# feixue94/sfd2

Measured on AMD Instinct MI355X. Metric: images/sec extract+match (1600x1200, n4096), higher is better.
Workload: dtype f16c

## Files before the change

sfd2_amd/_lib.py:

```python
import ctypes
import os

import numpy as np

_HERE = os.path.dirname(os.path.abspath(__file__))
LIB_PATH = os.path.join(_HERE, "libsfd2hip.so")


def use_library(path):
    global LIB_PATH, _lib
    if _lib is not None:
        raise RuntimeError("use_library() must be called before the library is first loaded")
    LIB_PATH = os.path.abspath(path)

FLAG_ASYNC = 1
FLAG_NO_STABILITY = 2
FLAG_IMG_NORMALISED = 4
FLAG_IMG_U8_HWC = 8
FLAG_IMG_BGR = 16
FLAG_IMG_U8_X = 32
FLAG_MATCH_OUT16 = 64
FLAG_DESC_STORE64 = 128
MATCH_HLOC, MATCH_ITLOC_NNM, MATCH_ITLOC_NNR = 0, 1, 2
DT_F32, DT_F64, DT_F16 = 0, 1, 2
# ... 197 lines not shown
                           "There is no CPU fallback.")
    lib = ctypes.CDLL(LIB_PATH)
    vp, ci, cf, i64 = ctypes.c_void_p, ctypes.c_int, ctypes.c_float, ctypes.c_int64
    pi = ctypes.POINTER(ctypes.c_int)
    lib.sfd2_version.restype = ci
    lib.sfd2_last_error.restype = ctypes.c_char_p
    lib.sfd2_ctx_create.argtypes = [ci, ctypes.POINTER(vp)]
    lib.sfd2_ctx_destroy.argtypes = [vp]
    lib.sfd2_ctx_destroy.restype = None
    lib.sfd2_get_stream.argtypes = [vp]
    lib.sfd2_get_stream.restype = vp
    lib.sfd2_load_weights.argtypes = [vp, ctypes.POINTER(Sfd2Tensor), ci]
    lib.sfd2_det.argtypes = [vp, vp, ci, ci, ci, ci, vp, vp, vp, ci, pi, pi, pi, pi]
    lib.sfd2_extract.argtypes = [vp, vp, ci, ci, ci, cf, ci, ci, vp, vp, vp, ci, i64, pi]
    lib.sfd2_extract_count.argtypes = [vp, pi]
    lib.sfd2_extract_multiscale.argtypes = [vp, vp, ci, ci, ci, vp, ci, cf, ci, ci, vp, vp, vp, ci, i64, pi]
    lib.sfd2_extract_spp.argtypes = [vp, vp, ci, ci, ci, cf, ci, vp, vp, vp, i64, pi, vp, vp]
    lib.sfd2_nms_fast.argtypes = [vp, vp, ci, ci, cf, ci, vp]
    lib.sfd2_extract_spp_levels.argtypes = [vp, vp, ci, ci, ci, ci, vp, vp, vp, cf, ci, vp, vp, vp, i64, vp]
    lib.sfd2_simple_nms.argtypes = [vp, vp, ci, ci, ci, vp]
    lib.sfd2_select_keypoints.argtypes = [vp, vp, ci, ci, cf, ci, ci, ci, vp, vp, i64, pi]
    lib.sfd2_sample_descriptors.argtypes = [vp, vp, ci, ci, ci, ci, vp, ci, vp]
    lib.sfd2_heatmap.argtypes = [vp, vp, ci, ci, vp, ci, ci, ci, ci, vp]
    lib.sfd2_debug_activation.argtypes = [vp, ctypes.c_char_p, vp, i64, pi, pi, pi]
    lib.sfd2_match.argtypes = [vp, vp, ci, vp, ci, ci, ci, ci, ci, ctypes.POINTER(MatchConf), vp, vp, ci]
    lib.sfd2_match_segments.argtypes = [vp, vp, ci, vp, ci, ci, ci, ci, ci, ci, vp, vp, ctypes.POINTER(MatchConf), vp, vp, ci]
    lib.sfd2_match_batch.argtypes = [vp, ctypes.POINTER(DescSet), ctypes.POINTER(DescSet), ci, ci,
                                     ctypes.POINTER(MatchConf), vp, vp, ci, ci]
    lib.sfd2_get_timings.argtypes = [vp, ctypes.POINTER(Timings)]
    lib.sfd2_sync.argtypes = [vp]
    lib.sfd2_set_precision.argtypes = [vp, ci]
    lib.sfd2_set_option.argtypes = [vp, ctypes.c_char_p, ci]
    lib.sfd2_get_option.argtypes = [vp, ctypes.c_char_p, pi]
    lib.sfd2_device_pci_bus_id.argtypes = [ci, ctypes.c_char_p, ci, pi]
    lib.sfd2_preprocess.argtypes = [vp, vp, ci, ci, ci, ci, ci, ci, vp]
    lib.sfd2_extract_match.argtypes = [vp, vp, ci, ci, cf, ci, ci, vp, vp, vp, ctypes.POINTER(DescSet), ci, ci,
                                       ctypes.POINTER(MatchConf), vp, vp]
    lib.sfd2_set_profiling.argtypes = [vp, ci]
    lib.sfd2_set_profile_filter.argtypes = [vp, ctypes.c_char_p]
    lib.sfd2_get_layer_timings.argtypes = [vp, ctypes.POINTER(LayerTiming), ci, pi]
    lib.sfd2_get_range_status.argtypes = [vp, ctypes.POINTER(RangeStatus), ci]
    lib.sfd2_range_tensor_name.argtypes = [ci]
    lib.sfd2_range_tensor_name.restype = ctypes.c_char_p
    lib.sfd2_calibrate_range.argtypes = [vp, vp, ci, ci, ci, ci]
    lib.sfd2_get_act_exponents.argtypes = [vp, vp, vp, ci, pi]
    lib.sfd2_get_margin_status.argtypes = [vp, vp, pi, ctypes.POINTER(ctypes.c_float)]
    lib.sfd2_get_relax_status.restype = ci
    lib.sfd2_get_relax_status.argtypes = [vp, ctypes.POINTER(ctypes.c_float), pi]
    lib.sfd2_set_act_exponents.argtypes = [vp, vp, ci]
    lib.sfd2_extract_record_async.argtypes = [vp, vp, ci]
    lib.sfd2_desc_pack.argtypes = [vp, ctypes.POINTER(DescSet), ci, vp, ci]
    lib.sfd2_jpeg_parse.argtypes = [vp, i64, ctypes.POINTER(JpegInfo)]
    lib.sfd2_jpeg_prepare.argtypes = [vp, i64, ctypes.POINTER(JpegInfo)]
    lib.sfd2_jpeg_decode.argtypes = [vp, vp, i64, ctypes.POINTER(JpegInfo), ci, vp, i64, vp, ci]
    lib.sfd2_absolute_pose_batch.argtypes = [vp, ctypes.POINTER(PoseProblem), ci, ctypes.POINTER(PoseConf), ctypes.POINTER(PoseResult), vp, ci]
    lib.sfd2_pose_refine_batch.argtypes = [vp, ctypes.POINTER(PoseProblem), ci, vp, vp, ctypes.POINTER(PoseResult), ci]
    lib.sfd2_relative_pose_batch.argtypes = [vp, ctypes.POINTER(TwoViewProblem), ci, ctypes.POINTER(TwoViewConf), ctypes.POINTER(TwoViewResult), vp, vp, ci]
    lib.sfd2_assemble_2d3d.argtypes = [vp, ctypes.POINTER(PointTable), ctypes.POINTER(AssembleJob), ci, ci, ci]
    cd = ctypes.c_double
    lib.sfd2_verify_matches_batch.argtypes = [vp, ctypes.POINTER(TriView), ci, vp, vp, vp, vp, ci, vp, cd, ci, vp, vp, ci]
    lib.sfd2_build_tracks.argtypes = [vp, i64, vp, i64, ci, vp, vp, vp, ctypes.POINTER(i64), ctypes.POINTER(i64), vp, ci]
    lib.sfd2_triangulate_tracks.argtypes = [vp, ctypes.POINTER(TriView), ci, vp, vp, ci, vp, vp, ctypes.POINTER(TriConf), vp, vp, vp, vp, vp, ci]
    lib.sfd2_pairs_retrieval.argtypes = [vp, vp, ci, vp, ci, ci, ci, ci, vp, vp, ci]
    lib.sfd2_pairs_covisibility.argtypes = [vp, vp, vp, ci, vp, vp, ci, ci, vp, vp, vp, ci]
    lib.sfd2_pairs_poses.argtypes = [vp, vp, vp, ci, ci, cd, vp, vp, vp, ci]
    lib.sfd2_covis_clusters.argtypes = [vp, vp, vp, ci, vp, vp, ci, vp, vp, ci, vp, vp, ci]
    lib.sfd2_covis_frames.argtypes = [vp, ctypes.POINTER(FramesMap), ctypes.POINTER(FramesTask), ci, vp, vp, ci, vp, vp, vp, ci]
    lib.sfd2_vlad_assign.argtypes = [vp, vp, i64, vp, ci, ci, vp, vp, ci]
    lib.sfd2_vlad_aggregate.argtypes = [vp, vp, vp, ci, vp, ci, ci, ci, vp, vp, ci]
    lib.sfd2_vlad_kmeans.argtypes = [vp, vp, i64, ci, ci, ci, vp, vp, vp, pi, ci]
    lib.sfd2_bundle_adjust.argtypes = [vp, ctypes.POINTER(TriView), ci, vp, vp, ci, vp, vp, vp, vp, ctypes.POINTER(BaConf), ctypes.POINTER(BaResult), vp, ci]
    lib.sfd2_mapper_restrict.argtypes = [vp, vp, ci, vp, vp, vp, ci, vp, vp, vp, vp, vp, ctypes.POINTER(i64), ctypes.POINTER(i64), ci]
    lib.sfd2_mapper_filter.argtypes = [vp, ctypes.POINTER(TriView), ci, vp, ci, vp, vp, vp, cd, cd, vp, vp, vp, vp, ci]
    lib.sfd2_mapper_visible.argtypes = [vp, vp, ci, vp, vp, ci, vp, vp, ci, vp, ci]
    lib.sfd2_mapper_assemble.argtypes = [vp, vp, ci, vp, vp, ci, vp, vp, vp, ci, vp, ci, i64, vp, vp, vp, vp, vp, ci]
    for name in EXPORTS:
        getattr(lib, name)
    if lib.sfd2_version() < 119:
        raise RuntimeError(f"{LIB_PATH} is version {lib.sfd2_version()}, this binding needs >= 119 (rebuild: __graft_entry__.build())")
    _lib = lib
    return lib


def check(rc):
    if rc != 0:
        raise RuntimeError("libsfd2hip: " + load().sfd2_last_error().decode("utf-8", "replace"))


def ptr(a):
    if a is None:
        return None
    if isinstance(a, int):
        return a
    if isinstance(a, np.ndarray):
        return a.ctypes.data
    return a.data_ptr()


class Context:

    def __init__(self, device=0):
        self.lib = load()
        h = ctypes.c_void_p()
        check(self.lib.sfd2_ctx_create(int(device), ctypes.byref(h)))
        self.h = h
        self.device = int(device)
        self.options = {}

    def close(self):
        if getattr(self, "h", None):
            self.lib.sfd2_ctx_destroy(self.h)
            self.h = None

    def __del__(self):
        try:
            self.close()
        except Exception:
            pass

    @property
    def stream(self):
        return self.lib.sfd2_get_stream(self.h)

    def load_weights(self, sd):
        keep, arr = [], (Sfd2Tensor * len(sd))()
        n = 0
        for name, v in sd.items():
            a = v.detach().cpu().numpy() if hasattr(v, "detach") else np.asarray(v)
            if a.dtype.kind != "f":
                continue
            a = np.ascontiguousarray(a, dtype=np.float32)
            if a.ndim > 4:
                continue
            keep.append(a)
            arr[n].name = name.encode()
            arr[n].data = a.ctypes.data
            arr[n].ndim = a.ndim
            for i, s in enumerate(a.shape):
                arr[n].shape[i] = s
            n += 1
        check(self.lib.sfd2_load_weights(self.h, arr, n))

    def timings(self):
        t = Timings()
        check(self.lib.sfd2_get_timings(self.h, ctypes.byref(t)))
        return {"ms_total": t.ms_total, "ms_backbone": t.ms_backbone, "ms_post": t.ms_post,
                "ms_match": t.ms_match, "n_candidates": t.n_candidates}

    def set_precision(self, mode):
        check(self.lib.sfd2_set_precision(self.h, {'f16': 0, 'f32': 1, 'f16x3': 2, 'f16c': 3, 'f16x3d': 2}[mode]))
        check(self.lib.sfd2_set_option(self.h, b"x3_desc16", 1 if mode == 'f16x3d' else 0))

    def set_option(self, key, value):
        check(self.lib.sfd2_set_option(self.h, key.encode(), int(value)))
        self.options.pop(key, None)
        self.options[key] = int(value)

    def get_option(self, key):
        v = ctypes.c_int(0)
        check(self.lib.sfd2_get_option(self.h, key.encode(), ctypes.byref(v)))
        return int(v.value)

    def sync(self):
        check(self.lib.sfd2_sync(self.h))

    def set_profiling(self, max_steps, kernel_filter=None):
# ... 70 lines not shown
```

sfd2_amd/build.py:

```python
import os
import subprocess

HERE = os.path.dirname(os.path.abspath(__file__))
CSRC = os.path.join(HERE, "csrc")
LIB = os.path.join(HERE, "libsfd2hip.so")
SOURCES = ["conv_kernels.hip", "conv2_kernels.hip", "conv3_kernels.hip", "conv3rf_kernels.hip", "conv2b_s2d_kernel.hip", "conv1x1_kernels.hip", "resblock_kernel.hip", "conv_f32_kernels.hip", "convc_kernels.hip", "rb23_c_kernel.hip", "sparse_da3_kernel.hip", "sparse_da0_kernel.hip", "fused_stem_kernel.hip", "fused_stem_c_kernel.hip", "post_kernels.hip", "util_kernels.hip", "nms4_kernels.hip", "match_kernels.hip", "match_mutual_kernel.hip", "api_core.hip", "api_weights.hip", "api_network.hip", "api_extract.hip", "api_match.hip", "api_graph.hip", "jpeg_parse.hip", "jpeg_kernels.hip", "api_jpeg.hip", "pose_kernels.hip", "api_pose.hip", "two_view_kernels.hip", "api_two_view.hip", "assemble_kernels.hip", "api_assemble.hip", "tri_kernels.hip", "api_triangulate.hip", "pairs_kernels.hip", "api_pairs.hip", "cluster_kernels.hip", "api_cluster.hip", "frames_kernels.hip", "api_frames.hip", "vlad_kernels.hip", "api_vlad.hip", "bundle_kernels.hip", "api_bundle.hip", "mapper_kernels.hip", "api_mapper.hip"]
_NN = ["-fno-honor-nans"]
SRC_FLAGS = {"match_mutual_kernel.hip": _NN, "conv3_kernels.hip": _NN, "conv3rf_kernels.hip": _NN, "resblock_kernel.hip": _NN, "conv2_kernels.hip": _NN,
             "fused_stem_kernel.hip": _NN, "conv_kernels.hip": _NN, "conv1x1_kernels.hip": _NN, "nms4_kernels.hip": _NN, "convc_kernels.hip": _NN, "fused_stem_c_kernel.hip": _NN, "rb23_c_kernel.hip": _NN, "sparse_da3_kernel.hip": _NN, "sparse_da0_kernel.hip": _NN, "conv2b_s2d_kernel.hip": _NN}
FLAGS = ["--offload-arch=gfx950", "-O3", "-std=c++17", "-fPIC", "-Wall", "-Wno-unused-function"] + \
    os.environ.get("SFD2_EXTRA_FLAGS", "").split()


def _newer(a, b):
    return (not os.path.exists(b)) or os.path.getmtime(a) > os.path.getmtime(b)


def _hipcc():
    return os.environ.get("HIPCC", "/opt/rocm/bin/hipcc")


def have_hipcc():
    return os.path.isfile(_hipcc()) and os.access(_hipcc(), os.X_OK)


def needs_build():
    if not os.path.exists(LIB):
        return True
    srcs = [os.path.join(CSRC, s) for s in SOURCES] + [os.path.join(CSRC, "sfd2_internal.h"), os.path.join(CSRC, "sfd2_ctx.h"), os.path.join(CSRC, "api_scratch.h"), os.path.join(CSRC, "pose_camera.h"), os.path.join(CSRC, "five_point.h"), os.path.join(CSRC, "bundle.h"), os.path.join(CSRC, "mapper.h"),
                                                      os.path.join(HERE, "..", "include", "sfd2_hip.h")]
    return any(os.path.exists(s) and os.path.getmtime(s) > os.path.getmtime(LIB) for s in srcs)


def build_lib(force=False, verbose=False, out=None, extra_flags=()):
    hipcc = _hipcc()
    objs = []
    deps = [os.path.join(CSRC, "sfd2_internal.h"), os.path.join(CSRC, "sfd2_ctx.h"), os.path.join(CSRC, "api_scratch.h"), os.path.join(CSRC, "pose_camera.h"), os.path.join(CSRC, "five_point.h"), os.path.join(CSRC, "bundle.h"), os.path.join(CSRC, "mapper.h"), os.path.join(HERE, "..", "include", "sfd2_hip.h")]
    procs = []
    lib = out or LIB
    odir = CSRC
    if out:
        odir = os.path.join(os.path.dirname(os.path.abspath(out)), "obj_" + os.path.basename(out).replace(".", "_"))
        os.makedirs(odir, exist_ok=True)
    for src in SOURCES:
        s = os.path.join(CSRC, src)
        o = os.path.join(odir, src.replace(".hip", ".o"))
        objs.append(o)
        if force or _newer(s, o) or any(_newer(d, o) for d in deps):
            cmd = [hipcc] + FLAGS + SRC_FLAGS.get(src, []) + list(extra_flags) + ["-c", s, "-o", o]
            if verbose:
                print(" ".join(cmd))
            procs.append((cmd, subprocess.Popen(cmd)))
    for cmd, p in procs:
        if p.wait() != 0:
            raise RuntimeError("hipcc failed: " + " ".join(cmd))
    if force or procs or not os.path.exists(lib) or any(_newer(o, lib) for o in objs):
        tmp = lib + ".tmp.%d" % os.getpid()
        cmd = [hipcc, "--offload-arch=gfx950", "-shared", "-fPIC", "-o", tmp] + objs
        if verbose:
            print(" ".join(cmd))
        subprocess.check_call(cmd)
        os.replace(tmp, lib)
    return lib


if __name__ == "__main__":
    print(build_lib(verbose=True))
```

sfd2_amd/csrc/api_core.hip:

```cpp
#include "sfd2_ctx.h"

static thread_local std::string g_err;
int sfd2_fail(const std::string &m)
{
    g_err = m;
    return -1;
}

std::atomic<unsigned long long> g_alloc_gen{0};

thread_local int g_sfd2_cu_limit = 0;

extern "C" int sfd2_version(void) { return 119; }
extern "C" const char *sfd2_last_error(void) { return g_err.c_str(); }

extern "C" int sfd2_ctx_create(int device, sfd2_ctx **out)
{
    if (!out) return fail("sfd2_ctx_create: out is null");
    int ndev = 0;
    hipError_t e = hipGetDeviceCount(&ndev);
    if (e != hipSuccess || ndev <= 0) return fail("sfd2_ctx_create: no HIP device available (libsfd2hip has no CPU fallback)");
    if (device < 0 || device >= ndev) return fail("sfd2_ctx_create: bad device index");
    HIPCHECK(hipSetDevice(device));
    sfd2_ctx *c = new sfd2_ctx();
// ... 18 lines not shown
    c->extract_rec.p = c->range_hist_dev.as<unsigned int>() + SFD2_RS_COUNT;
    static_assert(SFD2_RS_COUNT == SFD2_RANGE_TENSORS && AE_COUNT == SFD2_RANGE_GROUPS, "include/sfd2_hip.h and the internal tables agree");

    *out = c;
    return 0;
}

extern "C" int sfd2_device_pci_bus_id(int device, char *out, int len, int *n_devices)
{
    int ndev = 0;
    hipError_t e = hipGetDeviceCount(&ndev);
    if (e != hipSuccess || ndev <= 0) return fail("sfd2_device_pci_bus_id: no HIP device available");
    if (n_devices) *n_devices = ndev;
    if (device < 0 || device >= ndev) return fail("sfd2_device_pci_bus_id: bad device index");
    if (!out || len < 13) return fail("sfd2_device_pci_bus_id: buffer of at least 13 bytes needed");
    HIPCHECK(hipDeviceGetPCIBusId(out, len, device));
    return 0;
}

extern "C" void sfd2_ctx_destroy(sfd2_ctx *c)
{
    if (!c) return;
    (void)hipSetDevice(c->device);
    (void)hipStreamSynchronize(c->stream);
    graphs_release(c);
    for (int i = 0; i < 4; ++i) if (c->ev[i]) (void)hipEventDestroy(c->ev[i]);
    if (c->ev_jobs) (void)hipEventDestroy(c->ev_jobs);
    for (int i = 0; i < SFD2_IMG_SLOTS; ++i) {
        if (c->ev_copied[i]) (void)hipEventDestroy(c->ev_copied[i]);
        if (c->ev_img_free[i]) (void)hipEventDestroy(c->ev_img_free[i]);
    }
    if (c->copy_stream) (void)hipStreamDestroy(c->copy_stream);
    if (c->side_stream) (void)hipStreamDestroy(c->side_stream);
    if (c->ev_fork) (void)hipEventDestroy(c->ev_fork);
    if (c->ev_join) (void)hipEventDestroy(c->ev_join);
    for (hipEvent_t e : c->prof_ev) (void)hipEventDestroy(e);
    if (c->pin_jobs) (void)hipHostFree(c->pin_jobs);
    if (c->stream) (void)hipStreamDestroy(c->stream);
    delete c;
}

extern "C" void *sfd2_get_stream(sfd2_ctx *c) { return c ? (void *)c->stream : nullptr; }

extern "C" int sfd2_set_precision(sfd2_ctx *c, int mode)
{
    if (!c) return fail("sfd2_set_precision: null ctx");
    if (mode != SFD2_PREC_F16 && mode != SFD2_PREC_F32 && mode != SFD2_PREC_F16X3 && mode != SFD2_PREC_F16C)
        return fail("sfd2_set_precision: unknown mode");
    HIPCHECK(hipSetDevice(c->device));
    HIPCHECK(hipStreamSynchronize(c->stream));
    if (mode != c->precision) graphs_release(c);
    c->precision = mode;
    return sfd2_margin_selfcheck_if_pending(c);
}

extern "C" int sfd2_set_option(sfd2_ctx *c, const char *key, int value)
{
    if (!c || !key) return fail("sfd2_set_option: null argument");
    HIPCHECK(hipSetDevice(c->device));
    HIPCHECK(hipStreamSynchronize(c->stream));
    const std::string k(key);
    graphs_release(c);
    if (k == "fuse") c->fuse = value ? 1 : 0;
    else if (k == "fuse_det") c->fuse_det = value ? 1 : 0;
    else if (k == "alias") c->opt_alias = value ? 1 : 0;
    else if (k == "graphs") c->use_graphs = value ? 1 : 0;
    else if (k == "branches") c->opt_branches = value ? 1 : 0;
    else if (k == "sta_side") c->opt_sta_side = value ? 1 : 0;
    else if (k == "fuse_post") c->opt_fuse_post = value ? 1 : 0;
    else if (k == "sparse_desc") c->opt_sparse_desc = value ? 1 : 0;
    else if (k == "sparse_da3") c->opt_sparse_da3 = value ? 1 : 0;
    else if (k == "sparse_da0") c->opt_sparse_da0 = value < 0 ? 0 : (value > 2 ? 2 : value);
    else if (k == "cu_limit") c->opt_cu_limit = value < 0 ? 0 : value;
    else if (k == "auto_range") c->opt_auto_range = value ? 1 : 0;
    else if (k == "range_fallback") c->opt_range_fallback = value ? 1 : 0;
    else if (k == "x3_pp") c->opt_x3_pp = value ? 1 : 0;
    else if (k == "x3_desc16") c->opt_x3_desc16 = value ? 1 : 0;
    else if (k == "auto_margin") c->opt_auto_margin = value ? 1 : 0;
    else if (k == "fp6_filters") c->opt_fp6_filters = value ? 1 : 0;
    else if (k == "fp6_acts") c->opt_fp6_acts = value ? 1 : 0;
    else if (k == "s2d") c->opt_s2d = value ? 1 : 0;
    else if (k == "trunk_r1") c->opt_trunk_r1 = value ? 1 : 0;
    else if (k == "fuse_pb") c->opt_fuse_pb = value ? 1 : 0;
    else if (k == "generic_c") c->opt_generic_c = value ? 1 : 0;
    else if (k == "comp_rb") c->opt_comp_rb = value ? 1 : 0;
    else if (k == "no_rf_c") c->opt_no_rf_c = value ? 1 : 0;
    else if (k == "comp_heads") { c->opt_comp_heads = c->user_comp_heads = value ? 1 : 0; c->user_set_comp_heads = true; }
    else if (k == "c3b_plain") { c->user_c3b_plain = value < 0 ? -1 : (value ? 1 : 0); c->opt_c3b_plain = value > 0 ? 1 : 0; }
    else if (k == "comp_det") c->opt_comp_det = value ? 1 : 0;
    else if (k == "fuse_rb23") c->opt_fuse_rb23 = value ? 1 : 0;
    else if (k == "rb_inner") { c->opt_rb_inner = c->user_rb_inner = value < 0 ? 0 : (value > 2 ? 2 : value); c->user_set_rb_inner = true; }
    else return fail("sfd2_set_option: unknown key '" + k + "'");
    return 0;
}

extern "C" int sfd2_get_option(sfd2_ctx *c, const char *key, int *value)
{
    if (!c || !key || !value) return fail("sfd2_get_option: null argument");
    const std::string k(key);
    const struct { const char *name; int v; } tab[] = {
        {"fuse", c->fuse}, {"fuse_det", c->fuse_det}, {"alias", c->opt_alias}, {"graphs", c->use_graphs}, {"branches", c->opt_branches}, {"sta_side", c->opt_sta_side},
        {"fuse_post", c->opt_fuse_post}, {"sparse_desc", c->opt_sparse_desc}, {"sparse_da3", c->opt_sparse_da3}, {"sparse_da0", c->opt_sparse_da0}, {"cu_limit", c->opt_cu_limit},
        {"auto_range", c->opt_auto_range}, {"range_fallback", c->opt_range_fallback}, {"x3_pp", c->opt_x3_pp}, {"x3_desc16", c->opt_x3_desc16},
        {"auto_margin", c->opt_auto_margin}, {"fp6_filters", c->opt_fp6_filters}, {"fp6_acts", c->opt_fp6_acts}, {"s2d", c->opt_s2d},
        {"trunk_r1", c->opt_trunk_r1}, {"fuse_pb", c->opt_fuse_pb}, {"generic_c", c->opt_generic_c}, {"comp_rb", c->opt_comp_rb},
        {"no_rf_c", c->opt_no_rf_c}, {"comp_heads", c->opt_comp_heads}, {"c3b_plain", c->opt_c3b_plain}, {"comp_det", c->opt_comp_det},
        {"fuse_rb23", c->opt_fuse_rb23}, {"rb_inner", c->opt_rb_inner},
    };
    for (const auto &e : tab)
        if (k == e.name) { *value = e.v; return 0; }
    return fail("sfd2_get_option: unknown key '" + k + "'");
}

extern "C" int sfd2_sync(sfd2_ctx *c)
{
    if (!c) return fail("sfd2_sync: null ctx");
    HIPCHECK(hipSetDevice(c->device));
    HIPCHECK(hipStreamSynchronize(c->stream));
    return 0;
}

extern "C" int sfd2_set_profiling(sfd2_ctx *c, int max_steps)
{
    if (!c) return fail("sfd2_set_profiling: null ctx");
    HIPCHECK(hipSetDevice(c->device));
    HIPCHECK(hipStreamSynchronize(c->stream));
    if (max_steps < 0 || max_steps > 4096) return fail("sfd2_set_profiling: max_steps out of range");
    const size_t need = (size_t)max_steps * PROF_SLOTS * 2;
    while (c->prof_ev.size() < need) {
        hipEvent_t e;
        HIPCHECK(hipEventCreate(&e));
        c->prof_ev.push_back(e);
    }
    c->prof_max_steps = max_steps;
    c->prof_step = 0;
    c->prof_slot = 0;
    c->prof_used.assign(max_steps, 0);
    c->prof_row.assign((size_t)max_steps * PROF_SLOTS, 0);
    c->prof_tab.clear();
    return 0;
}

extern "C" int sfd2_set_profile_filter(sfd2_ctx *c, const char *substr)
{
    if (!c) return fail("sfd2_set_profile_filter: null ctx");
    c->prof_filter = substr ? substr : "";
    return 0;
}

extern "C" int sfd2_get_layer_timings(sfd2_ctx *c, sfd2_layer_timing *out, int cap, int *n)
{
    if (!c || !n) return fail("sfd2_get_layer_timings: null argument");
    HIPCHECK(hipSetDevice(c->device));
    HIPCHECK(hipStreamSynchronize(c->stream));
    for (int st = 0; st < c->prof_step; ++st)
        for (int sl = 0; sl < c->prof_used[st]; ++sl) {
            float ms = 0.0f;
            const size_t e = ((size_t)st * PROF_SLOTS + sl) * 2;
            const int row = c->prof_row[(size_t)st * PROF_SLOTS + sl];
            if (hipEventElapsedTime(&ms, c->prof_ev[e], c->prof_ev[e + 1]) == hipSuccess) {
                c->prof_tab[row].ms_total += ms;
                c->prof_tab[row].launches += 1;
            }
        }
    c->prof_step = 0;
    *n = (int)c->prof_tab.size();
    if (out)
        for (int i = 0; i < *n && i < cap; ++i) out[i] = c->prof_tab[i];
    return 0;
}

extern "C" int sfd2_get_timings(sfd2_ctx *c, sfd2_timings *out)
{
    if (!c || !out) return fail("sfd2_get_timings: null argument");
    *out = c->tim;
    return 0;
}

extern "C" const char *sfd2_range_tensor_name(int i) { return (i >= 0 && i < SFD2_RS_COUNT) ? kTensor[i].range : ""; }

static int fetch_range_words(sfd2_ctx *c, unsigned int *raw , bool clear)
{
    const size_t bytes = (size_t)SFD2_RS_COUNT * (SFD2_RANGE_SUB + 1) * sizeof(unsigned int);
    HIPCHECK(hipMemcpyAsync(raw, c->range_stat.p, bytes, hipMemcpyDeviceToHost, c->stream));
    if (clear) HIPCHECK(hipMemsetAsync(c->range_stat.p, 0, bytes, c->stream));
    HIPCHECK(hipStreamSynchronize(c->stream));
    return 0;
}
// ... 85 lines not shown
```

sfd2_amd/csrc/api_extract.hip:

```cpp
#include "sfd2_ctx.h"

static int release_image_slot(sfd2_ctx *c);
static int stage_image(sfd2_ctx *c, const void *x, int on_device, int H, int W, const float **dev, int u8 = 0)
{
    if (u8 == 2) {
        const float *raw = nullptr;
        if (on_device) raw = static_cast<const float *>(x);
        else if (stage_image(c, x, 0, H, W, &raw, 3)) return -1;
        HIPCHECK(c->img_u8_packed.ensure((size_t)3 * H * W + 16));
        launch_unpack_rgbx(c->stream, reinterpret_cast<const unsigned char *>(raw), c->img_u8_packed.as<unsigned char>(), (size_t)H * W);
        if (release_image_slot(c)) return -1;
        *dev = c->img_u8_packed.as<float>();
        return 0;
    }
    if (on_device) { *dev = static_cast<const float *>(x); return 0; }
    const size_t bytes = u8 == 3 ? (size_t)4 * H * W : (size_t)3 * H * W * (u8 ? 1 : sizeof(float));
    const int slot = c->img_slot = (c->img_slot + 1) % SFD2_IMG_SLOTS;
    HIPCHECK(c->img2[slot].ensure(bytes));
    HIPCHECK(hipStreamWaitEvent(c->copy_stream, c->ev_img_free[slot], 0));
    HIPCHECK(hipMemcpyAsync(c->img2[slot].p, x, bytes, hipMemcpyHostToDevice, c->copy_stream));
    HIPCHECK(hipEventRecord(c->ev_copied[slot], c->copy_stream));
    HIPCHECK(hipStreamWaitEvent(c->stream, c->ev_copied[slot], 0));
    c->img_slot_used = slot;
    *dev = c->img2[slot].as<float>();
// ... 65 lines not shown
                         int top_k, float *nms_dense, float *kpts_dev = nullptr, float *scores_dev = nullptr,
                         int Hb = 0, int Wb = 0)
{
    if (Hb <= 0) Hb = H;
    if (Wb <= 0) Wb = W;
    if (radius < 0 || radius > 4) return fail("nms radius must be in [0,4] (reference uses 4)");
    if (!(conf_th >= 0.0f)) return fail("conf_th must be >= 0 and not NaN (got " + std::to_string(conf_th) + ")");
    const int sel_cap = top_k > 0 ? std::min(top_k, c->cand_cap) : c->cand_cap;
    c->last_sel_cap = sel_cap;
    HIPCHECK(c->sel.ensure((size_t)sel_cap * 8));
    HIPCHECK(c->sorted.ensure((size_t)sel_cap * 8));
    HIPCHECK(c->kpts.ensure((size_t)sel_cap * 2 * sizeof(float)));
    HIPCHECK(c->kscores.ensure((size_t)sel_cap * sizeof(float)));
    if (!c->counters_clean) HIPCHECK(hipMemsetAsync(c->counters.p, 0, SFD2_COUNTER_BYTES, c->stream));
    c->counters_clean = false;
    bool threshold_done = false;
    {
        ProfScope ps(c, "nms_select", "nms_select_kernel", 0.0, (double)H * W * 4);
        threshold_done = launch_nms_select(c->stream, heat_dev, H, W, radius, conf_th, border, Hb, Wb, nms_dense,
                                           c->cand.as<unsigned long long>(), c->cand_cap, c->counters.as<unsigned int>(), 1, top_k);
    }
    {
        ProfScope ps(c, "topk_sort", "hist_select+compact+rank_sort", 0.0, (double)sel_cap * 24);
        c->kpts_cur = kpts_dev ? kpts_dev : c->kpts.as<float>();
        c->kscores_cur = scores_dev ? scores_dev : c->kscores.as<float>();
        launch_topk_sort(c->stream, threshold_done, c->cand.as<unsigned long long>(), c->cand_cap, top_k,
                         c->sel.as<unsigned long long>(), c->sorted.as<unsigned long long>(), sel_cap,
                         c->counters.as<unsigned int>(), c->bnd.as<unsigned long long>(), W, c->kpts_cur, c->kscores_cur);
    }
    HIPCHECK(hipGetLastError());
    return 0;
}

static int read_counts(sfd2_ctx *c, int64_t cap_out, int *n_out)
{
    unsigned int cnt[4] = {0, 0, 0, 0};
    HIPCHECK(hipMemcpyAsync(cnt, c->counters.p, sizeof(cnt), hipMemcpyDeviceToHost, c->stream));
    HIPCHECK(hipStreamSynchronize(c->stream));
    c->tim.n_candidates = cnt[0];
    if (cnt[0] > (unsigned int)c->cand_cap)
        return fail("candidate buffer overflow: " + std::to_string(cnt[0]) + " NMS survivors > capacity " +
                    std::to_string(c->cand_cap));
    int64_t n = cnt[1];
    if (n > c->last_sel_cap) n = c->last_sel_cap;
    if (cap_out >= 0 && n > cap_out) n = cap_out;
    if (n_out) *n_out = (int)n;
    return 0;
}

extern "C" int sfd2_extract(sfd2_ctx *c, const void *img, int img_on_device, int H, int W, float conf_th, int top_k,
                            int flags, float *kpts_xy, float *scores, float *desc, int out_on_device, int64_t cap_out,
                            int *n_out)
{
    if (!c || !img) return fail("sfd2_extract: null argument");
    if (!c->weights_loaded) return fail("sfd2_extract: weights not loaded");
    if (!(flags & SFD2_FLAG_NO_STABILITY) && !c->has_sta)
        return fail("sfd2_extract: the loaded state_dict has no ConvSta; pass SFD2_FLAG_NO_STABILITY (use_stability=False)");
    HIPCHECK(hipSetDevice(c->device));
    if (extract_begin(c, flags)) return -1;
    const PassPlan plan = plan_pass(c, PASS_EXTRACT, H, W, top_k, desc != nullptr);
    if (ensure_workspace(c, plan, H, W)) return -1;
    const float *img_dev = nullptr;
    const int u8 = (flags & SFD2_FLAG_IMG_U8_HWC) ? 1 : 0;
    if (u8 && (flags & SFD2_FLAG_IMG_NORMALISED)) return fail("sfd2_extract: a uint8 image cannot be pre-normalised");
    if ((flags & SFD2_FLAG_IMG_BGR) && !u8) return fail("sfd2_extract: SFD2_FLAG_IMG_BGR needs SFD2_FLAG_IMG_U8_HWC");
    if ((flags & SFD2_FLAG_IMG_U8_X) && !u8) return fail("sfd2_extract: SFD2_FLAG_IMG_U8_X needs SFD2_FLAG_IMG_U8_HWC");
    if (stage_image(c, img, img_on_device, H, W, &img_dev, u8 ? ((flags & SFD2_FLAG_IMG_U8_X) ? 2 : 1) : 0)) return -1;
    HIPCHECK(hipEventRecord(c->ev[0], c->stream));
    prof_step_begin(c);
    const int in_mode = ((flags & SFD2_FLAG_IMG_NORMALISED) ? 0 : 1) | (u8 ? 2 : 0) | ((flags & SFD2_FLAG_IMG_BGR) ? 4 : 0);
    if (run_network(c, plan, img_dev, in_mode)) return -1;
    if (release_image_slot(c)) return -1;
    HIPCHECK(hipEventRecord(c->ev[1], c->stream));
    const int HS = 8 * c->H8, WS = 8 * c->W8;
    if (plan.skip_pb) {
        ProfScope ps(c, "convPb+heads+heatmap", "pb_heads_heat_kernel", 2.0 * c->H8 * c->W8 * 65 * 256,
                     (double)c->H8 * c->W8 * 512 + (double)H * W * 4);
        launch_pb_heads_heat(c->stream, act_view(c, plan, T_PA).as<half_t>(), c->H8, c->W8, c->pb.w.as<half_t>(), c->pb.cout_pad, c->pb.scale.as<float>(),
                             c->pb.shift.as<float>(), (flags & SFD2_FLAG_NO_STABILITY) ? nullptr : c->sta.as<float>(), c->H4, c->W4,
                             H, W, c->heat.as<float>(), c->counters.as<unsigned int>(), SFD2_COUNTER_BYTES / 4);
        c->counters_clean = pb_heads_heat_clears(c->H8, c->W8, SFD2_COUNTER_BYTES / 4);
    } else if (plan.skip_head) {
        ProfScope ps(c, "heads+heatmap", "heads_heat_kernel", 0.0, (double)c->H8 * c->W8 * 65 * 4 + (double)H * W * 4);
        launch_heads_heat(c->stream, c->logits.as<float>(), 128, c->H8, c->W8,
                          (flags & SFD2_FLAG_NO_STABILITY) ? nullptr : c->sta.as<float>(), c->H4, c->W4, H, W, c->heat.as<float>());
    } else {
        ProfScope ps(c, "heatmap", "heatmap_kernel", 0.0, (double)H * W * 8);
        launch_heatmap(c->stream, c->score.as<float>(), HS, WS,
                       (flags & SFD2_FLAG_NO_STABILITY) ? nullptr : c->sta.as<float>(), c->H4, c->W4, H, W,
                       c->heat.as<float>(), nullptr);
    }
    const int sel_guess = top_k > 0 ? std::min(top_k, c->cand_cap) : c->cand_cap;
    const bool direct = out_on_device && kpts_xy && scores && cap_out >= sel_guess;
    if (run_selection(c, c->heat.as<float>(), H, W, conf_th, 4, 4, top_k, nullptr, direct ? kpts_xy : nullptr,
                      direct ? scores : nullptr)) return -1;
    const int sel_cap = c->last_sel_cap;
    int64_t ncopy = sel_cap;
    if (cap_out >= 0 && ncopy > cap_out) ncopy = cap_out;
    const bool store64 = desc && (flags & SFD2_FLAG_DESC_STORE64);
    if (store64 && cap_out < 1) return fail("sfd2_extract: SFD2_FLAG_DESC_STORE64 needs cap_out >= 1 (desc is double [128][cap_out])");
    float *desc_dst = nullptr;
    if (desc) {
        if (out_on_device && cap_out >= sel_cap && !store64) {
            desc_dst = desc;
        } else {
            HIPCHECK(c->kdesc.ensure((size_t)sel_cap * 128 * sizeof(float)));
            desc_dst = c->kdesc.as<float>();
        }
        if (plan.sparse_x3 && !plan.desc16) {
            const size_t nin = (size_t)c->H4 * c->W4 * 256;
            const int rows32 = (sel_cap * 4 + 31) / 32;
            HIPCHECK(c->da3_sparse.ensure((size_t)rows32 * 32 * 256 * sizeof(float)));
            HIPCHECK(c->db_sparse.ensure((size_t)rows32 * 32 * 128 * sizeof(float)));
            const ConvW &L3 = c->fda3;
            {
                ProfScope ps(c, "convDa.3", "sparse_da3_kernel<x3>", 2.0 * 4 * sel_cap * 256.0 * 256.0 * 9, (double)sel_cap * (16 * 1024 + 4 * 1024));
                launch_sparse_da3_x3(c->stream, c->x3_da0_planes.as<half_t>(), c->x3_da0_planes.as<half_t>() + nin, c->H4, c->W4, H, W,
                                     L3.wx3p.as<half_t>(), L3.wsl.as<half_t>(), L3.cout_pad, L3.scale.as<float>(), L3.shift.as<float>(), 0, c->kpts_cur,
                                     c->counters.as<unsigned int>() + 1, sel_cap, c->da3_sparse.as<float>(), c->zero_page.as<half_t>());
            }
            if (convf_at(c, StrictConv{}, "convDb", c->fdb, c->da3_sparse, rows32, 32, c->db_sparse, rows32, 32, 0)) return -1;
            ProfScope ps(c, "sample_desc", "sample_desc_kernel", 0.0, (double)sel_cap * 128 * 4 * 5);
            launch_sample_desc(c->stream, c->db_sparse.as<float>(), c->H4, c->W4, H, W, c->kpts_cur, c->counters.as<unsigned int>() + 1,
                               sel_cap, desc_dst, 1);
        } else if (plan.sparse_da3 || (plan.sparse_x3 && plan.desc16)) {
            HIPCHECK(c->da3_sparse.ensure((size_t)sel_cap * 4 * 256 * sizeof(half_t)));
            if (plan.sparse_da0) {
                const ConvW &L0 = c->da0;
                ProfScope ps(c, "convDa.0", "sparse_da0_kernel", 2.0 * 16 * sel_cap * (double)L0.cout * L0.cin * 9,
                             (double)sel_cap * (36 * 512 + 16 * 512) + 2.0 * L0.cout_pad * L0.cin * 9);
                launch_sparse_da0(c->stream, c->da0_in.as<half_t>(), c->H4, c->W4, H, W, L0.w.as<half_t>(), L0.scale.as<float>(), L0.shift.as<float>(), 1,
                                  c->kpts_cur, c->counters.as<unsigned int>() + 1, sel_cap, act_view(c, plan, T_DA0).as<half_t>());
            }
            {
                ProfScope ps(c, "convDa.3", "sparse_da3_kernel", 2.0 * 4 * sel_cap * 256.0 * 256.0 * 9, (double)sel_cap * (16 * 512 + 4 * 512) + 2.0 * 256 * 256 * 9);
                launch_sparse_da3(c->stream, act_view(c, plan, T_DA0).as<half_t>(), c->H4, c->W4, H, W, c->da3.w.as<half_t>(), c->da3.wsl.as<half_t>(), c->da3.cout_pad, c->da3.scale.as<float>(),
                                  c->da3.shift.as<float>(), 0, c->kpts_cur, c->counters.as<unsigned int>() + 1, sel_cap,
                                  c->da3_sparse.as<half_t>(), c->zero_page.as<half_t>());
            }
            ProfScope ps(c, "desc_head", "desc_head_kernel", 2.0 * 4 * sel_cap * 128 * 256, (double)sel_cap * (4 * 512 + 512));
            launch_desc_head(c->stream, c->da3_sparse.as<half_t>(), c->H4, c->W4, H, W, c->db.w.as<half_t>(), c->db.cout_pad, c->db.scale.as<float>(),
                             c->db.shift.as<float>(), c->kpts_cur, c->counters.as<unsigned int>() + 1, sel_cap, desc_dst, 1);
        } else if (plan.sparse_desc) {
            ProfScope ps(c, "desc_head", "desc_head_kernel", 2.0 * 4 * sel_cap * 128 * 256, (double)sel_cap * (4 * 512 + 512));
            launch_desc_head(c->stream, act_view(c, plan, T_DA).as<half_t>(), c->H4, c->W4, H, W, c->db.w.as<half_t>(), c->db.cout_pad, c->db.scale.as<float>(),
                             c->db.shift.as<float>(), c->kpts_cur, c->counters.as<unsigned int>() + 1, sel_cap, desc_dst);
        } else {
            ProfScope ps(c, "sample_desc", "sample_desc_kernel", 0.0, (double)sel_cap * 128 * 4 * 5);
            launch_sample_desc(c->stream, c->draw.as<float>(), c->H4, c->W4, H, W, c->kpts_cur,
                               c->counters.as<unsigned int>() + 1, sel_cap, desc_dst);
        }
    }
    size_t desc_bytes_fixed = 0;
    if (store64) {
        float *d64_dst = out_on_device ? desc : nullptr;
        if (!out_on_device) {
            HIPCHECK(c->kdesc64.ensure((size_t)128 * cap_out * sizeof(double)));
            d64_dst = c->kdesc64.as<float>();
        }
        ProfScope ps(c, "desc_store64", "desc_store64_kernel", 0.0, (double)sel_cap * 128 * 4 + (double)cap_out * 128 * 8);
        launch_desc_store64(c->stream, desc_dst, c->counters.as<unsigned int>() + 1, sel_cap, reinterpret_cast<double *>(d64_dst), (int)cap_out);
        desc_dst = d64_dst;
        desc_bytes_fixed = (size_t)128 * cap_out * sizeof(double);
    }
    prof_step_end(c);
    HIPCHECK(hipEventRecord(c->ev[2], c->stream));
    HIPCHECK(hipGetLastError());
    if (flags & SFD2_FLAG_ASYNC) {
        if (!direct && copy_out(c, kpts_xy, c->kpts.p, (size_t)ncopy * 2 * sizeof(float), out_on_device)) return -1;
        if (!direct && copy_out(c, scores, c->kscores.p, (size_t)ncopy * sizeof(float), out_on_device)) return -1;
        if (desc && desc_dst != desc && copy_out(c, desc, desc_dst, desc_bytes_fixed ? desc_bytes_fixed : (size_t)ncopy * 128 * sizeof(float), out_on_device)) return -1;
        if (n_out) *n_out = -1;
        return 0;
    }
    int n = 0;
    if (read_counts(c, cap_out, &n)) return -1;
    {
        const int fb = range_wants_fallback(c);
        if (fb < 0) return -1;
        if (fb) {
            FallbackScope scope(c);
            return sfd2_extract(c, img, img_on_device, H, W, conf_th, top_k, flags, kpts_xy, scores, desc, out_on_device, cap_out, n_out);
        }
    }
    if (!direct && copy_out(c, kpts_xy, c->kpts.p, (size_t)n * 2 * sizeof(float), out_on_device)) return -1;
    if (!direct && copy_out(c, scores, c->kscores.p, (size_t)n * sizeof(float), out_on_device)) return -1;
    if (desc && desc_dst != desc && copy_out(c, desc, desc_dst, desc_bytes_fixed ? desc_bytes_fixed : (size_t)n * 128 * sizeof(float), out_on_device)) return -1;
    HIPCHECK(hipStreamSynchronize(c->stream));
    float ms = 0.0f;
    if (hipEventElapsedTime(&ms, c->ev[0], c->ev[2]) == hipSuccess) c->tim.ms_total = ms;
    if (hipEventElapsedTime(&ms, c->ev[0], c->ev[1]) == hipSuccess) c->tim.ms_backbone = ms;
    if (hipEventElapsedTime(&ms, c->ev[1], c->ev[2]) == hipSuccess) c->tim.ms_post = ms;
    if (n_out) *n_out = n;
    return 0;
}

extern "C" int sfd2_preprocess(sfd2_ctx *c, const unsigned char *img_hwc, int on_device, int H, int W, int flags, int new_h,
                               int new_w, float *out_chw_dev)
{
    if (!c || !img_hwc || !out_chw_dev) return fail("sfd2_preprocess: null argument");
    if (H < 1 || W < 1 || new_h < 1 || new_w < 1) return fail("sfd2_preprocess: bad size");
    HIPCHECK(hipSetDevice(c->device));
    const float *staged = nullptr;
    if (stage_image(c, img_hwc, on_device, H, W, &staged, (flags & SFD2_FLAG_IMG_U8_X) ? 2 : 1)) return -1;
    launch_ingest_u8(c->stream, reinterpret_cast<const unsigned char *>(staged), H, W, (flags & SFD2_FLAG_IMG_BGR) ? 1 : 0, new_h,
                     new_w, out_chw_dev);
    if (release_image_slot(c)) return -1;
    HIPCHECK(hipGetLastError());
    if (!(flags & SFD2_FLAG_ASYNC)) HIPCHECK(hipStreamSynchronize(c->stream));
    return 0;
}

extern "C" int sfd2_extract_multiscale(sfd2_ctx *c, const void *img, int img_on_device, int H, int W, const double *scales,
                                       int n_scales, float conf_th, int top_k, int flags, float *kpts_xy, float *scores,
                                       float *desc, int out_on_device, int64_t cap_out, int *n_out)
{
    if (!c || !img || !scales) return fail("sfd2_extract_multiscale: null argument");
    if (n_scales < 1 || n_scales > 8) return fail("sfd2_extract_multiscale: 1..8 scales");
    if (!c->weights_loaded) return fail("sfd2_extract_multiscale: weights not loaded");
    if (!(flags & SFD2_FLAG_NO_STABILITY) && !c->has_sta)
        return fail("sfd2_extract_multiscale: the loaded state_dict has no ConvSta; pass SFD2_FLAG_NO_STABILITY");
    if (flags & SFD2_FLAG_ASYNC) return fail("sfd2_extract_multiscale: SFD2_FLAG_ASYNC is not supported");
    if (flags & SFD2_FLAG_DESC_STORE64) return fail("sfd2_extract_multiscale: SFD2_FLAG_DESC_STORE64 is not supported (single-scale sfd2_extract only)");
    if (!kpts_xy || !scores) return fail("sfd2_extract_multiscale: kpts_xy and scores are required");
    HIPCHECK(hipSetDevice(c->device));
// ... 384 lines not shown
```

sfd2_amd/csrc/api_network.hip:

```cpp
#include "sfd2_ctx.h"

static int down2(int n) { return (n - 1) / 2 + 1; }

static X3Kind x3_fast_kind(const PassPlan &p, const ConvW &L, bool has_res, int Ho, int Wo)
{
    if (!p.x3_pp || has_res || L.ks != 3 || L.cin % 64 != 0) return XK_GENERIC;
    if ((L.cout_pad == 256 || (L.cout_pad == 128 && L.stride == 2)) && conv3x3_rf_serves(3, L.stride, L.cout_pad, L.cin, Ho, Wo)) return XK_RF;
    return (L.stride == 1 && L.cout_pad % 128 == 0) ? XK_PP : XK_GENERIC;
}
static const int sl_level[] = {0 , 1, 1 , 2, 2, 2, 2, 2, 2, 2, 2, 2 , 3, 3 , 2, 2, 2};
static_assert(sizeof(sl_level) == SL_COUNT * sizeof(int), "one level per StrictLayer");
static bool on_planes(const StrictConv &s) { return s.kind == XK_PP || s.kind == XK_RF || s.kind == XK_S2D; }

#define SFD2_DA0_FRAC 0.6
PassPlan plan_pass(const sfd2_ctx *c, PassEntry entry, int H, int W, int top_k, bool desc)
{
    PassPlan p;
    const int H2 = down2(H), W2 = down2(W), H4 = down2(H2), W4 = down2(W2);
    const bool det = entry == PASS_DET, x3 = c->precision == SFD2_PREC_F16X3;
    p.f32 = x3 || c->precision == SFD2_PREC_F32;
    p.comp = c->precision == SFD2_PREC_F16C;
    p.fuse = !p.f32 && (det ? c->fuse_det : c->fuse);
    p.alias = p.fuse && !det && c->opt_alias;
    p.generic_c = p.comp && c->opt_generic_c;
    p.no_rf_c = c->opt_no_rf_c;
    p.fp6_filters = c->opt_fp6_filters;
    p.fused_stem = p.fuse && !p.generic_c;
    p.comp_rb = p.comp && c->opt_comp_rb;
    bool wrm = true, wk = true;
    for (int b = 0; b < 3; ++b) {
        wrm = wrm && c->rb1[b].wrm.p && c->rb3[b].wrm.p;
        wk = wk && c->rb1[b].wfl.p && c->rb3[b].wfl.p && c->rb2[b].wlk.p;
    }
    const char *frb = sfd2_env("SFD2_FUSED_RB");
    p.rb_fused = p.fuse && !p.comp_rb && !(frb && frb[0] == '0') && wrm;
    p.rb_inner = (p.comp_rb && !p.generic_c && wk) ? c->opt_rb_inner : 0;
    p.rb23 = p.rb_inner >= 2 && c->opt_fuse_rb23;
    if (p.comp) {
        const bool a6 = c->opt_fp6_acts && !p.generic_c && c->c2a.wc66.p && c->c3a.wc66.p && c->c3b.wc66.p;
        const bool s6 = a6 && p.fuse && c->w1b_stem_c6.p;
        const bool b6 = a6 && !p.no_rf_c && conv3x3_rf_c_serves(3, 2, c->c2b.cout_pad, c->c2b.cin, H4, W4);
        p.a2a_s2d = c->opt_s2d && p.alias && s6 && !p.no_rf_c && conv2b_s2d_serves(H2, W2, c->c2b.cin, c->c2b.cout_pad) && H4 * 2 == H2 && W4 * 2 == W2;
        static const bool c3a_plain_out = sfd2_env("SFD2_C3A_KEEP_CORR") == nullptr;
        const bool p3b = c->opt_c3b_plain && a6 && b6 && !p.generic_c;
        const bool p3a = p3b && c3a_plain_out;
        const bool tr1 = c->opt_trunk_r1 && a6 && p.rb23 && c->rb1[0].wfr.p && c->rb3[0].wf8l.p;
        p.ch = p.comp_rb && c->opt_comp_heads;
        p.chp = p.ch || (p.comp_rb && c->opt_comp_det);
        p.rec[T_CONV1A] = Rec::Unit8;
        p.rec[T_CONV1B] = s6 ? Rec::Half6 : Rec::Unit8;
        p.rec[T_CONV2A] = Rec::Unit8;
        p.rec[T_CONV2B] = b6 ? Rec::Half6 : Rec::Unit8;
        p.rec[T_CONV3A] = p3a ? Rec::None : a6 ? Rec::Half6 : Rec::Unit8;
        p.a3a_in = p3b ? Rec::None : p.rec[T_CONV3A];
        p.rec[T_CONV3B] = tr1 ? Rec::Resid8 : Rec::Unit8;
        for (int b = 0; b < 3 && p.comp_rb; ++b) {
            p.rec[T_T1_0 + b] = p.rb_inner >= 2 ? Rec::None : Rec::Unit8;
            p.rec[T_T2_0 + b] = p.rb_inner >= 1 ? Rec::None : Rec::Unit8;
            p.rec[T_OUT_0 + b] = (tr1 && (b < 2 || !p.chp)) ? Rec::Resid8 : Rec::Unit8;
        }
        p.rec[T_PA0] = p.chp ? Rec::Unit8 : Rec::None;
        p.rec[T_DA0] = p.ch ? Rec::Unit8 : Rec::None;
    }
    p.branches = c->opt_branches;
    if (entry == PASS_EXTRACT) {
        p.skip_head = c->opt_fuse_post && H % 8 == 0 && W % 8 == 0;
        p.skip_pb = p.skip_head && c->opt_fuse_pb && p.fuse && !p.branches && c->pb.cout_pad >= 96;
        const bool few = desc && top_k > 0 && (size_t)16 * top_k <= (size_t)H4 * W4;
        p.sparse_desc = c->opt_sparse_desc && p.fuse && few;
        p.sparse_da3 = p.sparse_desc && c->opt_sparse_da3 && !p.ch && !p.branches;
        p.sparse_x3 = x3 && c->opt_sparse_desc && c->opt_sparse_da3 && c->opt_x3_pp && few;
        p.sparse_da0 = p.sparse_da3 && c->opt_sparse_da0 && c->da0.w.p && c->da0.ks == 3 && c->da0.stride == 1 &&
                       sparse_da0_serves(c->da0.cin, c->da0.cout_pad, H4, W4) &&
                       (c->opt_sparse_da0 >= 2 || (double)16 * top_k <= SFD2_DA0_FRAC * (double)H4 * W4);
        p.skip_db = p.sparse_desc;
        p.skip_da3 = p.sparse_da3 || p.sparse_x3;
    }
    p.sta_early = p.alias && p.skip_pb;
    p.sta_side = c->has_sta && p.sta_early && c->opt_sta_side && !p.branches;
    if (p.alias) {
        static const int slots[T_COUNT] = {-1 , 0, 1 , 0, 1, 2, 0, 2, 0 , 1, 1, 1 ,
                                           0, 2, 0 , 1, 2 , 1 , 1 };
        for (int id = 0; id < T_COUNT; ++id) p.at[id].slot = slots[id];
        p.n_slots = p.branches ? 4 : 3;
        if (p.rb23) {
            p.at[T_T1_0 + 1].slot = 0; p.at[T_T1_0 + 2].slot = 1;
            p.at[T_OUT_0].slot = 1; p.at[T_OUT_0 + 2].slot = 0;
        }
        if (p.branches) p.at[T_DA].slot = 3;
        if (p.skip_pb) p.at[T_DA].slot = 0;
        const size_t P2 = (size_t)H2 * W2, P4 = (size_t)H4 * W4, P8 = (size_t)down2(H4) * down2(W4);
        size_t S = std::max(P2 * 64 * 2, P4 * 256 * 2);
        S = std::max(S, (P2 * 128 * 2 + 1) / 2);
        S = std::max(S, 2 * (P8 * 256 * 2 + 256));
        if (p.comp) S *= 2;
        p.slot_bytes = (S + 255) & ~(size_t)255;
        p.at[T_PA].off = (P8 * 256 * 2 * (p.comp ? 2 : 1) + 255) & ~(size_t)255;
    }
    p.x3_pp = x3 && c->opt_x3_pp;
    p.x3_fast = p.x3_pp && !det;
    if (!p.f32) return p;
    const int Hl[4] = {H, H2, H4, down2(H4)}, Wl[4] = {W, W2, W4, down2(W4)};
    for (int i = 0; i < SL_COUNT; ++i) {
        const ConvW &L = strict_layer(c, i);
        const int lo = sl_level[i] + (L.stride == 2);
        p.sl[i].kind = x3_fast_kind(p, L, i >= SL_RB3 && i < SL_RB3 + 3 , Hl[lo], Wl[lo]);
    }
    if (p.skip_da3) p.sl[SL_DA3].kind = p.sl[SL_DB].kind = XK_SKIP;
    if (!p.x3_fast) return p;
    p.x3_stem = c->w1b_stem_x3.p && c->c1a.wc.p;
    p.x3_rb = c->rb1[0].wfh.p && c->rb1[0].wfl.p && c->rb2[0].w.p && c->rb2[0].wlk.p;
    p.desc16 = p.skip_da3 && c->opt_x3_desc16 && p.x3_rb && c->da0.w.p && c->da0.scale_rawin.p && c->da3.w.p && c->db.w.p;
    if (p.x3_stem) p.sl[SL_C1B].kind = XK_SKIP;
    for (int i = SL_RB1; i < SL_RB3 + 3 && p.x3_rb; ++i) p.sl[i].kind = XK_SKIP;
    if (p.desc16) p.sl[SL_DA0].kind = XK_SKIP;
    if (c->opt_s2d && on_planes(p.sl[SL_C2B]) && on_planes(p.sl[SL_C3A]) && p.sl[SL_C2A].kind == XK_PP &&
        conv2b_s2d_serves(H2, W2, c->f2b.cin, c->f2b.cout_pad) && H4 * 2 == H2 && W4 * 2 == W2) {
        p.sl[SL_C2A].s2d_out = true, p.sl[SL_C2B].kind = XK_S2D;
    }
    X3Out have = p.x3_stem ? X3_CHAIN_A : X3_F32;
    auto route = [&](int i, bool planes_out, X3Out where = X3_CHAIN_A) {
        StrictConv &s = p.sl[i];
        s.planes_in = on_planes(s) && have != X3_F32;
        if (on_planes(s) && planes_out) s.out = (where == X3_CHAIN_A && s.planes_in && have == X3_CHAIN_A) ? X3_CHAIN_B : where;
        have = s.out;
    };
    route(SL_C2A, on_planes(p.sl[SL_C2B]));
    route(SL_C2B, on_planes(p.sl[SL_C3A]));
    route(SL_C3A, on_planes(p.sl[SL_C3B]));
    route(SL_C3B, p.x3_rb, X3_RB);
    const X3Out backbone = p.x3_rb ? X3_RB : X3_F32;
    have = backbone;
    route(SL_PA0, on_planes(p.sl[SL_PA3]));
    route(SL_PA3, false);
    have = backbone;
    if (!p.desc16) route(SL_DA0, p.skip_da3, X3_DA0);
    if (!p.skip_da3) route(SL_DA3, false);
    return p;
}

int ensure_workspace(sfd2_ctx *c, const PassPlan &p, int H, int W)
{
    if (H < 8 || W < 8) return fail("image too small (need H, W >= 8)");
    if ((long long)H * W > (1ll << 30)) return fail("image too large");
    c->H = H; c->W = W;
    c->H2 = down2(H); c->W2 = down2(W);
    c->H4 = down2(c->H2); c->W4 = down2(c->W2);
    c->H8 = down2(c->H4); c->W8 = down2(c->W4);
    const size_t P1 = (size_t)H * W, P2 = (size_t)c->H2 * c->W2, P4 = (size_t)c->H4 * c->W4, P8 = (size_t)c->H8 * c->W8;
    const size_t Pl[4] = {P1, P2, P4, P8}, hb = sizeof(half_t);
    const bool layers = !p.f32 && !p.alias;
    auto on_chip = [&](int id) { return id == T_CONV1A ? p.fused_stem : (id >= T_T1_0 && id < T_OUT_0 && p.rb_fused); };
    for (int id = 0; id < T_COUNT; ++id) {
        const size_t n = Pl[kTensor[id].level] * kTensor[id].ch;
        if (p.f32) HIPCHECK(c->act32[id].ensure(n * sizeof(float)));
        else if ((layers || id == T_CONV1A) && !on_chip(id)) HIPCHECK(c->act16[id].ensure(n * ((p.comp && id < T_PA) ? 2 * hb : hb)));
    }
    if (p.alias) HIPCHECK(c->arena.ensure(p.n_slots * p.slot_bytes));
    HIPCHECK(c->logits.ensure(P8 * 128 * sizeof(float)));
    HIPCHECK(c->draw.ensure(P4 * 128 * sizeof(float)));
    HIPCHECK(c->sta.ensure(P4 * 3 * sizeof(float)));
    HIPCHECK(c->score.ensure(P8 * 64 * sizeof(float)));
    HIPCHECK(c->heat.ensure(P1 * sizeof(float)));
    const size_t cap = cand_capacity(P1);
    c->cand_cap = (int)cap;
    HIPCHECK(c->cand.ensure(cap * 8));
    HIPCHECK(c->bnd.ensure(cap * 8));
    HIPCHECK(c->counters.ensure(SFD2_COUNTER_BYTES));
    for (ActInfo &a : c->acts) a.known = false;
    auto reg = [&](int id, const void *ptr, int is_f32, int planar, int pitch, Rec rec = Rec::None) -> ActInfo & {
        const TensorRow &t = kTensor[id];
        return c->acts[id] = ActInfo{true, ptr, is_f32, planar, t.ch, pitch, act_h(c, id), act_w(c, id), rec, (!is_f32 && t.group >= 0) ? c->act_exp[t.group] : 0};
    };
    reg(T_PB, c->logits.p, 1, 0, 128);
    reg(T_DB, c->draw.p, 1, 0, 128);
    reg(T_STA, c->sta.p, 1, 1, 0);
    if (p.f32) {
        if (p.sparse_x3 && !p.desc16 && p.sl[SL_DA0].out != X3_DA0) return fail("f16x3: the sparse descriptor head needs convDa.0 on a three-pass kernel (planes out)");
        const size_t pb = 2 * hb;
        size_t scratch = 0, chain[2] = {p.x3_stem ? std::max(P2 * 64, P4 * 256) : 0, 0}, da0 = p.desc16 ? P4 * 256 : 0;
        for (int i = 0; i < SL_COUNT; ++i) {
            const StrictConv &s = p.sl[i];
            const ConvW &L = strict_layer(c, i);
            if (!on_planes(s)) continue;
            const size_t nout = Pl[sl_level[i] + (L.stride == 2)] * L.cout_pad;
            if (!s.planes_in) scratch = std::max(scratch, Pl[sl_level[i]] * L.cin);
            if (s.out == X3_CHAIN_A || s.out == X3_CHAIN_B) chain[s.out - X3_CHAIN_A] = std::max(chain[s.out - X3_CHAIN_A], nout);
            if (s.out == X3_DA0) da0 = nout;
        }
        HIPCHECK(c->x3_planes.ensure(scratch * pb));
        for (int k = 0; k < 2; ++k) HIPCHECK(c->x3_chain[k].ensure(chain[k] * pb));
        for (int k = 0; k < 3 && p.x3_rb; ++k) HIPCHECK(c->x3_rb_planes[k].ensure(P4 * 256 * pb));
        HIPCHECK(c->x3_da0_planes.ensure(da0 * pb));
        if (ensure_strict_filters(c, p)) return -1;
    } else if (!layers) {
        if (p.sparse_da0) reg(T_DA0, act_view(c, p, T_DA0).p, 0, 0, kTensor[T_DA0].ch).absent = true;
        return 0;
    }
    for (int id = 0; id < T_COUNT; ++id) {
        if (p.f32) reg(id, c->act32[id].p, 1, 0, kTensor[id].ch).absent = p.x3_fast && id != T_OUT_0 + 2 && id != T_PA;
        else if (!on_chip(id)) reg(id, c->act16[id].p, 0, 0, kTensor[id].ch, id < T_PA0 ? p.rec[id] : Rec::None).absent = (p.rb23 && id >= T_T2_0 && id < T_OUT_0) || (p.sparse_da0 && id == T_DA0);
    }
    return 0;
}

static void conv_at(sfd2_ctx *c, const char *name, const ConvW &L, const DevPtr &in, int H, int W, const DevPtr &out,
                    int Ho, int Wo, int relu, const half_t *res = nullptr, int out_f32 = 0, const float *scale_override = nullptr)
{
    char kn[48];
    const float *scale = scale_override ? scale_override : L.scale.as<float>();
    const int bn = (L.cout_pad % 256 == 0) ? 256 : (L.cout_pad % 128 == 0 ? 128 : 64);
    snprintf(kn, sizeof(kn), "conv_igemm<%d,%d,%d%s>", L.ks, L.stride, bn, out_f32 ? ",f32" : "");
    if (!res && !out_f32 && conv3x3_pp_serves(L.ks, L.stride, L.cout_pad, L.cin)) snprintf(kn, sizeof(kn), "conv3x3_pp");
    if (!res && !out_f32 && conv3x3_rf_serves(L.ks, L.stride, L.cout_pad, L.cin, Ho, Wo)) snprintf(kn, sizeof(kn), "conv3x3_rf<%d>", L.stride);
    const double px = (double)Ho * Wo;
    const double flops = 2.0 * px * L.cout * L.cin * L.ks * L.ks;
    const double bytes = 2.0 * ((double)H * W * L.cin + (double)L.cout * L.cin * L.ks * L.ks) +
                         px * L.cout_pad * (out_f32 ? 4.0 : 2.0) + (res ? px * L.cout_pad * 2.0 : 0.0);
    static const bool no_c1 = sfd2_env("SFD2_NO_CONV1X1") != nullptr;
    if (L.wrm.p && !out_f32 && !no_c1) {
        snprintf(kn, sizeof(kn), "conv1x1_c256%s", res ? "+res" : "");
        ProfScope ps(c, name, kn, flops, bytes);
        launch_conv1x1_c256(c->cur_stream, in.as<half_t>(), Ho * Wo, L.wrm.as<half_t>(), scale, L.shift.as<float>(),
                            relu, res, reinterpret_cast<half_t *>(out.p), c->zero_page.as<half_t>());
        return;
    }
    ProfScope ps(c, name, kn, flops, bytes);
    launch_conv_igemm(c->cur_stream, in.as<half_t>(), H, W, L.cin, L.w.as<half_t>(), scale,
                      L.shift.as<float>(), L.cout_pad, L.ks, L.stride, relu, res, out.p, out_f32, Ho, Wo,
                      c->zero_page.as<half_t>());
}
static void conv(sfd2_ctx *c, const PassPlan &p, const char *name, const ConvW &L, int in, int out, int relu, int res = T_NONE, int out_f32 = 0)
{
    conv_at(c, name, L, act_view(c, p, in), act_h(c, in), act_w(c, in), act_view(c, p, out), act_h(c, out), act_w(c, out), relu,
            res != T_NONE ? act_view(c, p, res).as<half_t>() : nullptr, out_f32);
}

static unsigned int *range_slot(sfd2_ctx *c, int id)
{
    return (id >= 0 && c->range_stat.p) ? c->range_stat.as<unsigned int>() + id * SFD2_RANGE_SUB : nullptr;
}
static half_t *corr_of(const DevPtr &b, size_t px, int pitch) { return b.as<half_t>() + px * (size_t)pitch; }
struct PPFilters { const half_t *w; const float *shift; bool fp6; };
static PPFilters pp_filters(const PassPlan &p, const ConvW &L, Rec in, Rec out)
{
    if (in == Rec::Half6) return {L.wc66.as<half_t>(), L.sa66.as<float>(), true};
    if (in == Rec::Unit8 && (out == Rec::Half6 || (out == Rec::Unit8 && p.fp6_filters && L.wc6.p && L.sa6.p))) return {L.wc6.as<half_t>(), L.sa6.as<float>(), true};
    return {L.wc.as<half_t>(), L.shift.as<float>(), false};
}
static void convc(sfd2_ctx *c, const PassPlan &p, const char *name, const ConvW &L, int in_id, int out_id, int relu, int res_id = T_NONE,
                  bool s2d_out = false , const Rec *rin_override = nullptr)
{
    const DevPtr in = act_view(c, p, in_id), out = act_view(c, p, out_id), resv = res_id != T_NONE ? act_view(c, p, res_id) : DevPtr{}, *res = res_id != T_NONE ? &resv : nullptr;
    const int H = act_h(c, in_id), W = act_w(c, in_id), Ho = act_h(c, out_id), Wo = act_w(c, out_id);
    const Rec rin = rin_override ? *rin_override : p.rec[in_id], rout = p.rec[out_id];
    unsigned int *rs = range_slot(c, out_id < SFD2_RS_COUNT ? out_id : -1);
    char kn[48];
    const double px = (double)Ho * Wo;
    const double flops = 2.0 * px * L.cout * L.cin * L.ks * L.ks;
    const double bytes = (rin != Rec::None ? 4.0 : 2.0) * ((double)H * W * L.cin + (double)L.cout * L.cin * L.ks * L.ks) +
                         px * L.cout_pad * (rout != Rec::None ? 4.0 : 2.0) + (res ? px * L.cout_pad * 4.0 : 0.0);
    const half_t *in_c = rin != Rec::None ? corr_of(in, (size_t)H * W, L.cin) : nullptr;
    half_t *out_c = rout != Rec::None ? corr_of(out, (size_t)Ho * Wo, L.cout_pad) : nullptr;
    const bool pp = !res && !p.generic_c && L.ks == 3 && L.stride == 1 && L.cout_pad % 128 == 0 && L.cin % 64 == 0;
    if (pp) {
        ProfScope ps(c, name, (in_c && out_c) ? "conv3x3_pp<comp>" : (in_c ? "conv3x3_pp<comp,plain out>" : "conv3x3_pp<comp out>"), flops, bytes);
        const PPFilters f = pp_filters(p, L, rin, rout);
        if (f.w && launch_conv3x3_pp_c(c->cur_stream, in.as<half_t>(), in_c, H, W, L.cin, f.w, L.scale.as<float>(), f.shift, L.cout_pad, relu,
                                       out.as<half_t>(), out_c, Ho, Wo, c->zero_page.as<half_t>(), L.sbyte, rs, rin, rout, s2d_out, f.fp6))
            return;
        ps.cancel();
    } else if (!p.generic_c && !p.no_rf_c && in_c && out_c && !res && L.ks == 3 && L.stride == 2 && L.cout_pad == 128) {
        ProfScope ps(c, name, "conv3x3_rf<2,comp>", flops, bytes);
        if (launch_conv3x3_rf_c(c->cur_stream, in.as<half_t>(), in_c, H, W, L.cin, L.wc.as<half_t>(), L.scale.as<float>(), L.shift.as<float>(),
                                L.cout_pad, L.stride, relu, out.as<half_t>(), out_c, Ho, Wo, c->zero_page.as<half_t>(), L.sbyte, rs, rin, rout))
            return;
        ps.cancel();
    }
    const bool unit8 = (rin == Rec::None || rin == Rec::Unit8) && (rout == Rec::None || rout == Rec::Unit8) && !s2d_out;
    if (pp || !unit8) {
        c->net_error = 1;
        (void)fail(std::string(name) + ": no kernel instantiation for the corr-record formats the pass plan asks for");
        return;
    }
// ... 245 lines not shown
                                          c->zero_page.as<half_t>(), L1.sbyte, range_slot(c, t1i), x_rec, t1_rec);
                } else {
                    convc(c, p, rb_layer_name(b, 1), L1, x, t1i, 1);
                }
                if (p.rb23) {
                    ProfScope ps(c, rb_layer_name(b, 3), "rb23_c_kernel", 2.0 * P4 * 256 * 72 + 2.0 * P4 * 256.0 * 256.0,
                                 P4 * 256.0 * (10 - (x_rec == Rec::Resid8) - (o_rec == Rec::Resid8)));
                    launch_rb23_c(st, t1.as<half_t>(), H4, W4, L2.w.as<half_t>(), L2.wlk.as<half_t>(), L2.scale.as<float>(), L2.shift.as<float>(),
                                  L3.wfh.as<half_t>(), L3.wfl.as<half_t>(), L3.scale.as<float>(), L3.shift.as<float>(), xv.as<half_t>(),
                                  corr_of(xv, PP, 256), ob.as<half_t>(), corr_of(ob, PP, 256), c->zero_page.as<half_t>(),
                                  range_slot(c, t2i), range_slot(c, obi), x_rec, o_rec, L3.wf8l.as<half_t>(), L3.sbyte);
                    x = obi;
                    continue;
                }
                {
                    ProfScope ps(c, rb_layer_name(b, 2), t1p ? "gconv_c_kernel<plain>" : "gconv_c_kernel<plain out>", 2.0 * P4 * 256 * 72, P4 * 256 * (t1p ? 4 : 6));
                    launch_gconv_c(st, t1.as<half_t>(), t1p ? nullptr : corr_of(t1, PP, 256), H4, W4, L2.w.as<half_t>(),
                                   t1p ? L2.wlk.p : L2.wc.p, L2.scale.as<float>(), L2.shift.as<float>(), t2.as<half_t>(), nullptr, L2.sbyte, 0, H4,
                                   range_slot(c, t2i));
                }
                {
                    ProfScope ps(c, rb_layer_name(b, 3), "conv1x1_c256<comp,plain in>+res", 2.0 * P4 * 256.0 * 256.0, P4 * 256.0 * 10);
                    launch_conv1x1_c256_c(st, t2.as<half_t>(), nullptr, (int)PP, L3.wfh.as<half_t>(), L3.wfl.as<half_t>(), L3.scale.as<float>(),
                                          L3.shift.as<float>(), 1, xv.as<half_t>(), corr_of(xv, PP, 256), ob.as<half_t>(), corr_of(ob, PP, 256),
                                          c->zero_page.as<half_t>(), L3.sbyte, range_slot(c, obi), t2_rec, o_rec);
                }
            } else {
                convc(c, p, rb_layer_name(b, 1), c->rb1[b], x, t1i, 1);
                {
                    ProfScope ps(c, rb_layer_name(b, 2), "gconv_c_kernel", 2.0 * P4 * 256 * 72, P4 * 256 * 8);
                    launch_gconv_c(st, t1.as<half_t>(), corr_of(t1, (size_t)H4 * W4, 256), H4, W4, c->rb2[b].w.as<half_t>(),
                                   c->rb2[b].wc.p, c->rb2[b].scale.as<float>(), c->rb2[b].shift.as<float>(), t2.as<half_t>(),
                                   corr_of(t2, (size_t)H4 * W4, 256), c->rb2[b].sbyte, 0, H4, range_slot(c, t2i));
                }
                convc(c, p, rb_layer_name(b, 3), c->rb3[b], t2i, obi, 1, x);
            }
            x = obi;
        }
    } else {
    if (p.fused_stem) {
        ProfScope ps(c, "conv1a+conv1b", "fused_stem_kernel", 2.0 * P1 * 64 * 27 + 2.0 * (double)H2 * W2 * 64 * 576,
                     P1 * 12 + (double)H2 * W2 * 128);
        launch_fused_stem(st, img_dev, H, W, normalise, c->c1a.w.as<half_t>(), c->c1a.scale.as<float>(),
                          c->c1a.shift.as<float>(), c->w1b_fused.as<half_t>(), c->c1b.scale.as<float>(),
                          c->c1b.shift.as<float>(), V(T_CONV1B).as<half_t>(), H2, W2);
    } else {
        {
            ProfScope ps(c, "conv1a", "conv1a_kernel", 2.0 * P1 * 64 * 27, P1 * (12 + 128));
            launch_conv1a(st, img_dev, H, W, normalise, c->c1a.w.as<half_t>(), c->c1a.scale.as<float>(),
                          c->c1a.shift.as<float>(), V(T_CONV1A).as<half_t>());
        }
        conv(c, p, "conv1b", c->c1b, T_CONV1A, T_CONV1B, 1);
    }
    conv(c, p, "conv2a", c->c2a, T_CONV1B, T_CONV2A, 1);
    conv(c, p, "conv2b", c->c2b, T_CONV2A, T_CONV2B, 1);
    conv(c, p, "conv3a", c->c3a, T_CONV2B, T_CONV3A, 1);
    conv(c, p, "conv3b", c->c3b, T_CONV3A, T_CONV3B, 1);
    for (int b = 0; b < 3; ++b) rb_f16(b);
    }
    const bool sta_side = p.sta_side;
    if (c->has_sta && p.sta_early) {
        if (sta_side) {
            HIPCHECK(hipEventRecord(c->ev_fork, st));
            HIPCHECK(hipStreamWaitEvent(c->side_stream, c->ev_fork, 0));
            c->cur_stream = c->side_stream;
        }
        conv_sta();
        if (sta_side) {
            HIPCHECK(hipEventRecord(c->ev_join, c->side_stream));
            c->cur_stream = st;
        }
    }
    const bool fork = p.branches;
    if (fork) {
        HIPCHECK(hipEventRecord(c->ev_fork, st));
        HIPCHECK(hipStreamWaitEvent(c->side_stream, c->ev_fork, 0));
        c->cur_stream = c->side_stream;
    }
    if (p.chp) {
        convc(c, p, "convPa.0", c->pa0, x, T_PA0, 1);
        convc(c, p, "convPa.3", c->pa3, T_PA0, T_PA, 0);
    } else {
        conv(c, p, "convPa.0", c->pa0, x, T_PA0, 1);
        conv(c, p, "convPa.3", c->pa3, T_PA0, T_PA, 0);
    }
    if (!p.skip_pb) conv(c, p, "convPb", c->pb, T_PA, T_PB, 0, T_NONE, 1);
    if (!p.skip_head) {
        ProfScope ps(c, "detector_head", "detector_head_kernel", 0.0, P8 * (65 * 4 + 256));
        launch_detector_head(c->cur_stream, c->logits.as<float>(), 128, H8, W8, c->score.as<float>());
    }
    if (fork) {
        HIPCHECK(hipEventRecord(c->ev_join, c->side_stream));
        c->cur_stream = st;
    }
    if (p.ch) {
        convc(c, p, "convDa.0", c->da0, x, T_DA0, 1);
        convc(c, p, "convDa.3", c->da3, T_DA0, T_DA, 0);
    } else {
        if (p.sparse_da0) c->da0_in = V(x);
        else conv(c, p, "convDa.0", c->da0, x, T_DA0, 1);
        if (!p.skip_da3) conv(c, p, "convDa.3", c->da3, T_DA0, T_DA, 0);
    }
    if (!p.skip_db) conv(c, p, "convDb", c->db, T_DA, T_DB, 0, T_NONE, 1);
    if (c->has_sta && !p.sta_early) conv_sta();
    if (fork || sta_side) HIPCHECK(hipStreamWaitEvent(st, c->ev_join, 0));
    HIPCHECK(hipGetLastError());
    if (c->net_error) { c->net_error = 0; return -1; }
    return 0;
}
```

sfd2_amd/csrc/api_weights.hip:

```cpp
#include "sfd2_ctx.h"
#include <map>

struct TView {
    const float *d;
    std::vector<int64_t> shape;
    std::vector<int> ec;
    size_t numel() const { size_t n = 1; for (auto s : shape) n *= (size_t)s; return n; }
};
typedef std::map<std::string, TView> TMap;

static const TView *find_t(const TMap &m, const std::string &k)
{
    auto it = m.find(k);
    return it == m.end() ? nullptr : &it->second;
}

static int upload(DevBuf &b, const void *src, size_t bytes, hipStream_t st)
{
    HIPCHECK(b.ensure(bytes));
    HIPCHECK(hipMemcpyAsync(b.p, src, bytes, hipMemcpyHostToDevice, st));
    HIPCHECK(hipStreamSynchronize(st));
    return 0;
}

// ... 154 lines not shown
                        const unsigned char l8 = f32_to_e4m3(std::ldexp(v - (float)h, b0 + 11));
                        pc[plane + o] = (unsigned short)(w8 | (l8 << 8));
                    }
        if (upload(L.wc, pc.data(), pc.size() * 2, c->stream)) return -1;
        if (ks == 3 && stride == 1 && cout_pad % 128 == 0 && cin % 64 == 0) {
            std::vector<int> ec(cout_pad, 0);
            for (int pix6 = 0; pix6 < 2; ++pix6) {
            std::vector<unsigned short> p6(2 * plane, 0);
            std::memcpy(p6.data(), pc.data(), plane * 2);
            std::vector<int> sa(2 * (size_t)cout_pad, 0x7f7f7f7f);
            std::memcpy(sa.data(), sh.data(), (size_t)cout_pad * sizeof(float));
            for (int oc = 0; oc < cout; ++oc) {
                float mx = 0.0f;
                for (size_t i = 0; i < (size_t)cin * T; ++i) mx = std::max(mx, std::fabs(w->d[(size_t)oc * cin * T + i]));
                int e = (mx > 0.0f && std::isfinite(mx)) ? (int)std::ceil(std::log2(mx / 7.5f)) : 0;
                while (std::ldexp(mx, -e) > 7.5f) ++e;
                e = std::max(-40, std::min(40, e));
                ec[oc] = e;
                sa[cout_pad + oc] = ((127 - (pix6 ? 11 : SFD2_C_XL_SHIFT) + e) & 255) * 0x01010101;
            }
            for (int ch = 0; ch < nch32; ++ch)
                for (int t = 0; t < T; ++t)
                    for (int oc = 0; oc < cout; ++oc) {
                        unsigned char *row = reinterpret_cast<unsigned char *>(p6.data() + plane) + ((((size_t)ch * T + t) * cout_pad + oc) * 32) * 2;
                        for (int h = 0; h < 2; ++h) {
                            unsigned char str[24] = {0};
                            for (int p6i = 0; p6i < 32; ++p6i) {
                                const int j = 32 * h + p6i, jj = p6i >> 1;
                                const int k = pix6 ? 8 * (jj >> 2) + 4 * h + (jj & 3) : j >> 1;
                                const float v = w->d[(((size_t)oc * cin + ch * 32 + k) * ks + t / ks) * ks + t % ks];
                                const float x = (j & 1) ? std::ldexp(v - (float)(half_t)v, 11 - ec[oc]) : std::ldexp(v, -ec[oc]);
                                const unsigned int code = f32_to_e2m3(x);
                                const int bit = 6 * p6i;
                                str[bit >> 3] |= (unsigned char)(code << (bit & 7));
                                if ((bit & 7) > 2) str[(bit >> 3) + 1] |= (unsigned char)(code >> (8 - (bit & 7)));
                            }
                            std::memcpy(row + 16 * h, str, 16);
                            std::memcpy(row + 32 + 16 * h, str + 16, 8);
                        }
                    }
            if (upload(pix6 ? L.wc66 : L.wc6, p6.data(), p6.size() * 2, c->stream)) return -1;
            (pix6 ? L.h_sa66 : L.h_sa6) = sa;
            if (upload(pix6 ? L.sa66 : L.sa6, sa.data(), sa.size() * sizeof(int), c->stream)) return -1;
            }
        }
        if (ks == 1 && stride == 1 && cin == 256 && cout == 256) {
            std::vector<half_t> fh((size_t)256 * 256), fl(fh.size());
            std::vector<unsigned short> fc(fh.size());
            std::vector<unsigned char> fr(fh.size() * 2);
            for (int wv = 0; wv < 8; ++wv)
                for (int cc = 0; cc < 8; ++cc)
                    for (int l = 0; l < 64; ++l)
                        for (int e = 0; e < 16; ++e) {
                            const int row = wv * 32 + (l & 31), col = cc * 32 + (e >> 3) * 16 + (l >> 5) * 8 + (e & 7);
                            const float v = w->d[(size_t)row * 256 + col];
                            const size_t o = (((size_t)wv * 8 + cc) * 64 + l) * 16 + e;
                            fh[o] = (half_t)v;
                            fl[o] = (half_t)((v - (float)(half_t)v) * 2048.0f);
                            fc[o] = (unsigned short)(f32_to_e4m3(std::ldexp(v, b0)) | (f32_to_e4m3(std::ldexp(v - (float)(half_t)v, b0 + 11)) << 8));
                            fr[(o - e) * 2 + e] = f32_to_e4m3(std::ldexp(v, b0));
                            fr[(o - e) * 2 + 16 + e] = f32_to_e4m3(std::ldexp(v - (float)(half_t)v, b0 + 11));
                        }
            if (upload(L.wfh, fh.data(), fh.size() * 2, c->stream)) return -1;
            if (upload(L.wfl, fl.data(), fl.size() * 2, c->stream)) return -1;
            if (upload(L.wfc, fc.data(), fc.size() * 2, c->stream)) return -1;
            if (upload(L.wfr, fr.data(), fr.size(), c->stream)) return -1;
            {
                std::vector<unsigned char> f8((size_t)8 * 4 * 64 * 32);
                for (int wv = 0; wv < 8; ++wv)
                    for (int j = 0; j < 4; ++j)
                        for (int l = 0; l < 64; ++l)
                            for (int n = 0; n < 32; ++n) {
                                const int row = wv * 32 + (l & 31), col = 16 * (4 * j + (n >> 3)) + 8 * (l >> 5) + (n & 7);
                                const float v = w->d[(size_t)row * 256 + col];
                                f8[(((size_t)wv * 4 + j) * 64 + l) * 32 + n] = f32_to_e4m3(std::ldexp(v - (float)(half_t)v, b0 + 11));
                            }
                if (upload(L.wf8l, f8.data(), f8.size(), c->stream)) return -1;
            }
        }
    }
    return 0;
}

static int pack_conv1a(sfd2_ctx *c, const TMap &m)
{
    const TView *w = find_t(m, "conv1a.0.weight");
    if (!w) return fail("missing tensor: conv1a.0.weight");
    if (w->shape.size() != 4 || w->shape[0] != 64 || w->shape[1] != 3 || w->shape[2] != 3 || w->shape[3] != 3)
        return fail("bad shape for conv1a.0.weight");
    ConvW &L = c->c1a;
    L.cin = 3; L.cout = 64; L.cout_pad = 64; L.ks = 3; L.stride = 1;
    std::vector<half_t> pk((size_t)2 * 3 * 64 * 8, (half_t)0.0f);
    for (int ct = 0; ct < 2; ++ct)
        for (int ky = 0; ky < 3; ++ky)
            for (int lane = 0; lane < 64; ++lane)
                for (int j = 0; j < 8; ++j) {
                    const int oc = ct * 32 + (lane & 31), g = lane >> 5;
                    const int kx = 2 * g + (j >> 2), ch = j & 3;
                    float v = 0.0f;
                    if (kx < 3 && ch < 3) v = w->d[(((size_t)oc * 3 + ch) * 3 + ky) * 3 + kx];
                    pk[(((size_t)ct * 3 + ky) * 64 + lane) * 8 + j] = (half_t)v;
                }
    std::vector<float> sc, sh;
    if (fold_scale_shift(m, "conv1a.0", "conv1a.1", 64, 64, sc, sh)) return -1;
    if (upload(L.w, pk.data(), pk.size() * sizeof(half_t), c->stream)) return -1;
    if (set_scale_shift(c, L, sc, sh)) return -1;
    {
        std::vector<half_t> pc(2 * pk.size(), (half_t)0.0f);
        for (int ct = 0; ct < 2; ++ct)
            for (int ky = 0; ky < 3; ++ky)
                for (int lane = 0; lane < 64; ++lane)
                    for (int j = 0; j < 8; ++j) {
                        const int oc = ct * 32 + (lane & 31), g = lane >> 5;
                        const int kx = 2 * g + (j >> 2), ch = j & 3;
                        float v = 0.0f;
                        if (kx < 3 && ch < 3) v = w->d[(((size_t)oc * 3 + ch) * 3 + ky) * 3 + kx];
                        const size_t o = (((size_t)ct * 3 + ky) * 64 + lane) * 8 + j;
                        pc[o] = (half_t)v;
                        pc[pk.size() + o] = (half_t)(v - (float)pc[o]);
                    }
        if (upload(L.wc, pc.data(), pc.size() * sizeof(half_t), c->stream)) return -1;
    }
    return 0;
}

static int pack_gconv(sfd2_ctx *c, const TMap &m, ConvW &L, const std::string &conv, const std::string &bn)
{
    const TView *w = find_t(m, conv + ".weight");
    if (!w) return fail("missing tensor: " + conv + ".weight");
    if (w->shape.size() != 4 || w->shape[0] != 256 || w->shape[1] != 8 || w->shape[2] != 3 || w->shape[3] != 3)
        return fail("bad shape for " + conv + ".weight (expected [256,8,3,3], groups=32)");
    L.cin = 256; L.cout = 256; L.cout_pad = 256; L.ks = 3; L.stride = 1;
    std::vector<half_t> pk((size_t)16 * 5 * 64 * 8, (half_t)0.0f), pl(pk.size(), (half_t)0.0f);
    for (int pair = 0; pair < 16; ++pair)
        for (int s = 0; s < 5; ++s)
            for (int lane = 0; lane < 64; ++lane)
                for (int j = 0; j < 8; ++j) {
                    const int i = lane & 15, g = lane >> 4;
                    const int tap = 2 * s + (g >> 1);
                    const int oc = pair * 16 + i;
                    float v = 0.0f;
                    if (tap <= 8 && (i >> 3) == (g & 1)) v = w->d[(((size_t)oc * 8 + j) * 3 + tap / 3) * 3 + tap % 3];
                    pk[(((size_t)pair * 5 + s) * 64 + lane) * 8 + j] = (half_t)v;
                    pl[(((size_t)pair * 5 + s) * 64 + lane) * 8 + j] = (half_t)((v - (float)(half_t)v) * 2048.0f);
                }
    if (upload(L.wlk, pl.data(), pl.size() * sizeof(half_t), c->stream)) return -1;
    std::vector<float> sc, sh;
    if (fold_scale_shift(m, conv, bn, 256, 256, sc, sh)) return -1;
    if (upload(L.w, pk.data(), pk.size() * sizeof(half_t), c->stream)) return -1;
    if (set_scale_shift(c, L, sc, sh)) return -1;
    std::vector<half_t> cp((size_t)256 * 9 * 8);
    for (int oc = 0; oc < 256; ++oc)
        for (int tap = 0; tap < 9; ++tap)
            for (int j = 0; j < 8; ++j)
                cp[((size_t)oc * 9 + tap) * 8 + j] = (half_t)w->d[(((size_t)oc * 8 + j) * 3 + tap / 3) * 3 + tap % 3];
    if (upload(L.wgc, cp.data(), cp.size() * sizeof(half_t), c->stream)) return -1;
    {
        const int b0 = corr_b0(w->d, w->numel());
        L.sbyte = 127 - SFD2_C_XL_SHIFT - b0;
        std::vector<unsigned short> pc((size_t)16 * 3 * 64 * 16, 0);
        for (int pair = 0; pair < 16; ++pair)
            for (int mm = 0; mm < 3; ++mm)
                for (int lane = 0; lane < 64; ++lane)
                    for (int ch = 0; ch < 16; ++ch) {
                        const int i = lane & 15, tap = 4 * mm + (lane >> 4);
                        const int oc = pair * 16 + i;
// ... 141 lines not shown
            for (int oc = 0; oc < 64; ++oc)
                for (int ic = 0; ic < 64; ++ic) pk[((size_t)t * 64 + oc) * 64 + ic] = (half_t)w->d[((size_t)oc * 64 + ic) * 9 + t];
        if (upload(c->w1b_fused, pk.data(), pk.size() * sizeof(half_t), c->stream)) return -1;
    }
    {
        const TView *w = find_t(m, "conv1b.0.weight");
        const int b0 = 127 - SFD2_C_XL_SHIFT - c->c1b.sbyte;
        std::vector<unsigned short> pk((size_t)2 * 18 * 64 * 32, 0);
        for (int cth = 0; cth < 2; ++cth)
            for (int u = 0; u < 18; ++u)
                for (int lane = 0; lane < 64; ++lane)
                    for (int kk = 0; kk < 2; ++kk)
                        for (int j = 0; j < 8; ++j) {
                            const int oc = cth * 32 + (lane & 31), ic = (u & 1) * 32 + kk * 16 + (lane >> 5) * 8 + j, tap = u >> 1;
                            const float v = w->d[((size_t)oc * 64 + ic) * 9 + tap];
                            const half_t h = (half_t)v;
                            unsigned short hb;
                            std::memcpy(&hb, &h, 2);
                            const size_t base = ((size_t)(cth * 18 + u) * 64 + lane) * 32;
                            pk[base + kk * 8 + j] = hb;
                            pk[base + 16 + kk * 8 + j] = (unsigned short)(f32_to_e4m3(std::ldexp(v, b0)) | (f32_to_e4m3(std::ldexp(v - (float)h, b0 + 11)) << 8));
                        }
        if (upload(c->w1b_stem_c, pk.data(), pk.size() * 2, c->stream)) return -1;
        {
            std::vector<unsigned short> p6 = pk;
            for (int cth = 0; cth < 2; ++cth)
                for (int lane = 0; lane < 64; ++lane) {
                    const int oc = cth * 32 + (lane & 31), h = lane >> 5;
                    float mx = 0.0f;
                    for (int i = 0; i < 64 * 9; ++i) mx = std::max(mx, std::fabs(w->d[(size_t)oc * 576 + i]));
                    int ec = (mx > 0.0f && std::isfinite(mx)) ? (int)std::ceil(std::log2(mx / 7.5f)) : 0;
                    while (std::ldexp(mx, -ec) > 7.5f) ++ec;
                    ec = std::max(-40, std::min(40, ec));
                    for (int u = 0; u < 18; ++u) {
                        unsigned char str[32] = {0};
                        for (int p = 0; p < 32; ++p) {
                            const int j = p >> 1, ic = (u & 1) * 32 + 8 * (j >> 2) + 4 * h + (j & 3), tap = u >> 1;
                            const float v = w->d[((size_t)oc * 64 + ic) * 9 + tap];
                            const float x = (p & 1) ? std::ldexp(v - (float)(half_t)v, 11 - ec) : std::ldexp(v, -ec);
                            const unsigned int code = f32_to_e2m3(x);
                            const int bit = 6 * p;
                            str[bit >> 3] |= (unsigned char)(code << (bit & 7));
                            if ((bit & 7) > 2) str[(bit >> 3) + 1] |= (unsigned char)(code >> (8 - (bit & 7)));
                        }
                        const unsigned int sb = ((unsigned int)(127 - 11 + ec) & 255u) * 0x01010101u;
                        std::memcpy(str + 24, &sb, 4);
                        std::memcpy(reinterpret_cast<unsigned char *>(p6.data()) + (((size_t)(cth * 18 + u) * 64 + lane) * 32 + 16) * 2, str, 32);
                    }
                }
            if (upload(c->w1b_stem_c6, p6.data(), p6.size() * 2, c->stream)) return -1;
        }
        for (int cth = 0; cth < 2; ++cth)
            for (int u = 0; u < 18; ++u)
                for (int lane = 0; lane < 64; ++lane)
                    for (int kk = 0; kk < 2; ++kk)
                        for (int j = 0; j < 8; ++j) {
                            const int oc = cth * 32 + (lane & 31), ic = (u & 1) * 32 + kk * 16 + (lane >> 5) * 8 + j, tap = u >> 1;
                            const float v = w->d[((size_t)oc * 64 + ic) * 9 + tap];
                            const half_t l = (half_t)((v - (float)(half_t)v) * 2048.0f);
                            unsigned short lb;
                            std::memcpy(&lb, &l, 2);
                            pk[((size_t)(cth * 18 + u) * 64 + lane) * 32 + 16 + kk * 8 + j] = lb;
                        }
        if (upload(c->w1b_stem_x3, pk.data(), pk.size() * 2, c->stream)) return -1;
    }
    if (pack_igemm(c, m, c->c2a, "conv2a.0", "conv2a.1", 64, 128, 3, 1)) return -1;
    if (pack_igemm(c, m, c->c2b, "conv2b.0", "bn2b.0", 128, 128, 3, 2)) return -1;
    if (pack_igemm(c, m, c->c3a, "conv3a.0", "conv3a.1", 128, 256, 3, 1)) return -1;
    if (pack_igemm(c, m, c->c3b, "conv3b.0", "bn3b.0", 256, 256, 3, 1)) return -1;
    for (int b = 0; b < 3; ++b) {
        const std::string p = "conv4." + std::to_string(b) + ".";
        if (pack_igemm(c, m, c->rb1[b], p + "conv1", p + "bn1", 256, 256, 1, 1)) return -1;
        if (pack_gconv(c, m, c->rb2[b], p + "conv2", p + "bn2")) return -1;
        if (pack_igemm(c, m, c->rb3[b], p + "conv3", p + "bn3", 256, 256, 1, 1)) return -1;
    }
    if (pack_igemm(c, m, c->pa0, "convPa.0", "convPa.1", 256, 256, 3, 2)) return -1;
    if (pack_igemm(c, m, c->pa3, "convPa.3", "", 256, 256, 3, 1)) return -1;
    if (pack_igemm(c, m, c->da0, "convDa.0", "convDa.1", 256, 256, 3, 1)) return -1;
    if (pack_igemm(c, m, c->da3, "convDa.3", "", 256, 256, 3, 1)) return -1;
    HIPCHECK(c->da3.wsl.ensure((size_t)(256 / 32) * 9 * c->da3.cout_pad * 32 * sizeof(half_t)));
    launch_sparse_da3_repack(c->stream, c->da3.w.as<half_t>(), c->da3.wsl.as<half_t>(), c->da3.cout_pad, 256);
    if (pack_igemm(c, m, c->pb, "convPb", "", 256, 65, 1, 1)) return -1;
    if (pack_igemm(c, m, c->db, "convDb", "", 256, 128, 1, 1)) return -1;
    const TView *sw = find_t(m, "ConvSta.weight"), *sb = find_t(m, "ConvSta.bias");
    c->has_sta = false;
    if (sw || sb) {
        if (!sw || !sb) return fail("missing tensor: ConvSta.{weight,bias} (only one of the two is present)");
        if (sw->numel() != 3 * 256 || sb->numel() != 3) return fail("bad shape for ConvSta");
        c->h_sta_w.assign(sw->d, sw->d + 3 * 256);
        if (upload(c->sta_w, sw->d, 3 * 256 * sizeof(float), c->stream)) return -1;
        if (upload(c->sta_b, sb->d, 3 * sizeof(float), c->stream)) return -1;
        c->has_sta = true;
    }
    if (pack_all_f32(c, m)) return -1;
    for (int g = 0; g < AE_COUNT; ++g) { c->act_exp[g] = 0; c->act_max[g] = 0.0f; }
    c->weights_loaded = true;
    if (apply_act_exponents(c)) { c->weights_loaded = false; return -1; }
    c->margin_done = false;
    c->margin_pending = false;
    c->margin_choice = -1;
    for (float &e : c->margin_err) e = -1.0f;
    c->relax_err = -1.0f;
    c->opt_c3b_plain = c->user_c3b_plain == 1 ? 1 : 0;
    if (c->opt_auto_range && calibrate_on_probe(c)) { c->weights_loaded = false; return -1; }
    return 0;
}

int apply_act_exponents(sfd2_ctx *c)
{
    struct Row { ConvW *L; int e_in, e_out; };
    const int *e = c->act_exp;
    std::vector<Row> rows = {
        {&c->c1a, -1, AE_CONV1A}, {&c->c1b, AE_CONV1A, AE_CONV1B}, {&c->c2a, AE_CONV1B, AE_CONV2A}, {&c->c2b, AE_CONV2A, AE_CONV2B},
        {&c->c3a, AE_CONV2B, AE_CONV3A}, {&c->c3b, AE_CONV3A, AE_TRUNK}, {&c->pa0, AE_TRUNK, AE_PA0}, {&c->pa3, AE_PA0, -1},
        {&c->da0, AE_TRUNK, AE_DA0}, {&c->da3, AE_DA0, -1}};
    for (int b = 0; b < 3; ++b) {
        rows.push_back({&c->rb1[b], AE_TRUNK, AE_T1_0 + b});
        rows.push_back({&c->rb2[b], AE_T1_0 + b, AE_T2_0 + b});
        rows.push_back({&c->rb3[b], AE_T2_0 + b, AE_TRUNK});
    }
    std::vector<float> sc, sh;
    for (const Row &r : rows) {
        ConvW &L = *r.L;
        if (L.h_scale.empty()) continue;
        const int ei = r.e_in >= 0 ? e[r.e_in] : 0, eo = r.e_out >= 0 ? e[r.e_out] : 0;
        sc = L.h_scale; sh = L.h_shift;
        for (float &v : sc) v = std::ldexp(v, eo - ei);
        for (float &v : sh) v = std::ldexp(v, eo);
        if (upload(L.scale, sc.data(), sc.size() * sizeof(float), c->stream)) return -1;
        if (upload(L.shift, sh.data(), sh.size() * sizeof(float), c->stream)) return -1;
        if (!L.h_sa6.empty() && L.sa6.p) {
            std::vector<int> sa = L.h_sa6;
            std::memcpy(sa.data(), sh.data(), std::min(sh.size(), sa.size() / 2) * sizeof(float));
            if (upload(L.sa6, sa.data(), sa.size() * sizeof(int), c->stream)) return -1;
        }
        if (!L.h_sa66.empty() && L.sa66.p) {
            std::vector<int> sa = L.h_sa66;
            std::memcpy(sa.data(), sh.data(), std::min(sh.size(), sa.size() / 2) * sizeof(float));
            if (upload(L.sa66, sa.data(), sa.size() * sizeof(int), c->stream)) return -1;
        }
    }
    if (!c->da0.h_scale.empty()) {
        sc = c->da0.h_scale;
        for (float &v : sc) v = std::ldexp(v, e[AE_DA0]);
        if (upload(c->da0.scale_rawin, sc.data(), sc.size() * sizeof(float), c->stream)) return -1;
    }
    if (c->has_sta && !c->h_sta_w.empty()) {
        std::vector<float> w = c->h_sta_w;
        for (float &v : w) v = std::ldexp(v, -e[AE_TRUNK]);
        if (upload(c->sta_w16, w.data(), w.size() * sizeof(float), c->stream)) return -1;
    }
    graphs_release(c);
    return reset_range_records(c);
}

#define SFD2_RANGE_TARGET 16.0f
static int calibrate_impl(sfd2_ctx *c, const float *img, int on_device, int H, int W, int flags)
{
    if (!c->weights_loaded) return fail("sfd2_calibrate_range: weights not loaded");
    HIPCHECK(hipSetDevice(c->device));
    const int prec = c->precision, prof_max = c->prof_max_steps;
    c->precision = SFD2_PREC_F32;
    c->prof_max_steps = 0;
    const int rc = sfd2_det(c, img, on_device, H, W, flags, nullptr, nullptr, nullptr, 0, nullptr, nullptr, nullptr, nullptr);
    c->precision = prec;
    c->prof_max_steps = prof_max;
    if (rc) return -1;
    HIPCHECK(c->range_scratch.ensure(AE_COUNT * sizeof(unsigned int)));
    HIPCHECK(hipMemsetAsync(c->range_scratch.p, 0, AE_COUNT * sizeof(unsigned int), c->stream));
    for (int id = 0; id < SFD2_RS_COUNT; ++id)
        launch_absmax_f32(c->stream, c->act32[id].as<float>(), (size_t)kTensor[id].ch * act_h(c, id) * act_w(c, id), c->range_scratch.as<unsigned int>() + kTensor[id].group);
    HIPCHECK(hipGetLastError());
    float mx[AE_COUNT];
    HIPCHECK(hipMemcpyAsync(mx, c->range_scratch.p, sizeof(mx), hipMemcpyDeviceToHost, c->stream));
    HIPCHECK(hipStreamSynchronize(c->stream));
    for (int g = 0; g < AE_COUNT; ++g) {
        c->act_max[g] = mx[g];
        int e = 0;
        if (mx[g] > 0.0f && std::isfinite(mx[g])) e = (int)std::lround(std::log2(SFD2_RANGE_TARGET / mx[g]));
        c->act_exp[g] = std::max(-60, std::min(60, e));
    }
    return apply_act_exponents(c);
}

extern "C" int sfd2_calibrate_range(sfd2_ctx *c, const float *img, int img_on_device, int H, int W, int flags)
{
    if (!c || !img) return fail("sfd2_calibrate_range: null argument");
    return calibrate_impl(c, img, img_on_device, H, W, flags);
}

extern "C" int sfd2_get_act_exponents(sfd2_ctx *c, int32_t *exps, float *maxima, int cap, int *n)
{
    if (!c || !n) return fail("sfd2_get_act_exponents: null argument");
    *n = AE_COUNT;
    for (int g = 0; g < AE_COUNT && g < cap; ++g) {
        if (exps) exps[g] = c->act_exp[g];
        if (maxima) maxima[g] = c->act_max[g];
    }
// ... 146 lines not shown
```

sfd2_amd/csrc/conv_kernels.hip:

```cpp
#include "sfd2_internal.h"
#include <stdlib.h>

#define TW 32
#define TH 4
#define CC 32
#define PIXP 40
#define NT 256

__device__ __forceinline__ int xcd_swizzle(int bid, int nblk)
{
    const int q = nblk >> 3, r = nblk & 7, xcd = bid & 7, local = bid >> 3;
    const int base = xcd < r ? xcd * (q + 1) : r * (q + 1) + (xcd - r) * q;
    return base + local;
}

__device__ __forceinline__ h4_t cvt4(float a, float b, float c, float d)
{
    h4_t r;
    r[0] = (half_t)a; r[1] = (half_t)b; r[2] = (half_t)c; r[3] = (half_t)d;
    return r;
}

template <int KS, int STRIDE, int BN, bool OUT_F32, bool HAS_RES>
__global__ __launch_bounds__(NT, (STRIDE == 1 ? 2 : 1))
// ... 146 lines not shown
                }
#pragma unroll
                for (int q = 0; q < 4; ++q) {
                    const float4 sc = *reinterpret_cast<const float4 *>(SS + cl + 8 * q);
                    const float4 sh = *reinterpret_cast<const float4 *>(SS + BN + cl + 8 * q);
                    float v0 = acc[ct][pr][4 * q + 0] * sc.x + sh.x;
                    float v1 = acc[ct][pr][4 * q + 1] * sc.y + sh.y;
                    float v2 = acc[ct][pr][4 * q + 2] * sc.z + sh.z;
                    float v3 = acc[ct][pr][4 * q + 3] * sc.w + sh.w;
                    if (HAS_RES) {
                        v0 += (float)rq[q][0]; v1 += (float)rq[q][1]; v2 += (float)rq[q][2]; v3 += (float)rq[q][3];
                    }
                    if (relu) {
                        v0 = fmaxf(v0, 0.0f); v1 = fmaxf(v1, 0.0f); v2 = fmaxf(v2, 0.0f); v3 = fmaxf(v3, 0.0f);
                    }
                    const size_t o = pix * CoutP + n0 + cl + 8 * q;
                    if (OUT_F32) *reinterpret_cast<float4 *>(reinterpret_cast<float *>(outv) + o) = make_float4(v0, v1, v2, v3);
                    else *reinterpret_cast<h4_t *>(reinterpret_cast<half_t *>(outv) + o) = cvt4(v0, v1, v2, v3);
                }
            }
        }
    }
}

template <int KS, int STRIDE, int BN, bool OUT_F32, bool HAS_RES>
static void launch_igemm_t(hipStream_t st, const half_t *in, int H, int W, int Cin, const half_t *wpk,
                           const float *scale, const float *shift, int CoutP, int relu, const half_t *res,
                           void *out, int Ho, int Wo)
{
    constexpr int PH = (TH - 1) * STRIDE + KS, PW = (TW - 1) * STRIDE + KS;
    constexpr size_t lds = (size_t)(2 * PH * PW + 2 * BN) * PIXP * sizeof(half_t) + (size_t)2 * BN * sizeof(float);
    static bool attr_done = false;
    auto kern = conv_igemm_kernel<KS, STRIDE, BN, OUT_F32, HAS_RES>;
    if (!attr_done) {
        (void)hipFuncSetAttribute(reinterpret_cast<const void *>(kern), hipFuncAttributeMaxDynamicSharedMemorySize, (int)lds);
        attr_done = true;
    }
    const int tiles_x = (Wo + TW - 1) / TW, tiles_y = (Ho + TH - 1) / TH;
    const int grid = tiles_x * tiles_y * (CoutP / BN);
    hipLaunchKernelGGL(kern, dim3(grid), dim3(NT), lds, st, in, H, W, Cin, wpk, scale, shift, CoutP, relu, res, out,
                       Ho, Wo, tiles_x);
}

bool launch_conv_igemm2(hipStream_t st, const half_t *in, int H, int W, int Cin, const half_t *wpk,
                        const float *scale, const float *shift, int CoutP, int ks, int stride, int relu,
                        const half_t *residual, void *out, int out_f32, int Ho, int Wo, const half_t *zero_page);
int conv_igemm2_chunk(int ks, int stride, int CoutP, int Cin);

int conv_igemm_chunk(int ks, int stride, int CoutP, int Cin)
{
    static const bool force_v1 = sfd2_env("SFD2_CONV_V1") != nullptr;
    if (!force_v1) {
        const int c = conv_igemm2_chunk(ks, stride, CoutP, Cin);
        if (c) return c;
    }
    return 32;
}

void launch_conv_igemm(hipStream_t st, const half_t *in, int H, int W, int Cin, const half_t *wpk,
                       const float *scale, const float *shift, int CoutP, int ks, int stride, int relu,
                       const half_t *residual, void *out, int out_f32, int Ho, int Wo, const half_t *zero_page)
{
    if (sfd2_env("SFD2_CONV_V1") == nullptr && zero_page &&
        launch_conv_igemm2(st, in, H, W, Cin, wpk, scale, shift, CoutP, ks, stride, relu, residual, out, out_f32, Ho, Wo, zero_page))
        return;
#define SFD2_IGEMM(KS_, ST_, BN_, F32_)                                                                               \
    do {                                                                                                              \
        if (residual) launch_igemm_t<KS_, ST_, BN_, F32_, true>(st, in, H, W, Cin, wpk, scale, shift, CoutP, relu, residual, out, Ho, Wo); \
        else launch_igemm_t<KS_, ST_, BN_, F32_, false>(st, in, H, W, Cin, wpk, scale, shift, CoutP, relu, residual, out, Ho, Wo);         \
    } while (0)
    const int bn = (CoutP % 256 == 0) ? 256 : (CoutP % 128 == 0 ? 128 : 64);
    if (ks == 3 && stride == 1 && !out_f32) {
        if (bn == 256) SFD2_IGEMM(3, 1, 256, false);
        else if (bn == 128) SFD2_IGEMM(3, 1, 128, false);
        else SFD2_IGEMM(3, 1, 64, false);
    } else if (ks == 3 && stride == 2 && !out_f32) {
        if (bn == 256) SFD2_IGEMM(3, 2, 256, false);
        else if (bn == 128) SFD2_IGEMM(3, 2, 128, false);
        else SFD2_IGEMM(3, 2, 64, false);
    } else if (ks == 1 && stride == 1 && !out_f32) {
        if (bn == 256) SFD2_IGEMM(1, 1, 256, false);
        else if (bn == 128) SFD2_IGEMM(1, 1, 128, false);
        else SFD2_IGEMM(1, 1, 64, false);
    } else if (ks == 1 && stride == 1 && out_f32) {
        if (bn == 256) SFD2_IGEMM(1, 1, 256, true);
        else if (bn == 128) SFD2_IGEMM(1, 1, 128, true);
        else SFD2_IGEMM(1, 1, 64, true);
    } else {
        abort();
    }
#undef SFD2_IGEMM
}

#define C1_TH 8
#define C1_PH 10
#define C1_PW 36
__global__ __launch_bounds__(NT)
void conv1a_kernel(const float *__restrict__ img, int H, int W, int normalise,
                   const half_t *__restrict__ wpk, const float *__restrict__ scale,
                   const float *__restrict__ shift, half_t *__restrict__ out, int tiles_x)
{
    __shared__ __attribute__((aligned(16))) half_t Xs[C1_PH * C1_PW * 4];
    const int tid = threadIdx.x, lane = tid & 63, wave = tid >> 6;
    const int swz = xcd_swizzle(blockIdx.x, gridDim.x);
    const int tx = swz % tiles_x, ty = swz / tiles_x;
    const int oy0 = ty * C1_TH, ox0 = tx * TW;
    const size_t plane = (size_t)H * W;

    for (int p = tid; p < C1_PH * C1_PW; p += NT) {
        const int py = p / C1_PW, px = p - py * C1_PW;
        const int iy = oy0 - 1 + py, ix = ox0 - 1 + px;
        float r = 0.0f, g = 0.0f, b = 0.0f;
        if (iy >= 0 && iy < H && ix >= 0 && ix < W) {
            const size_t o = (size_t)iy * W + ix;
            if (normalise & 2) {
                const unsigned char *u = reinterpret_cast<const unsigned char *>(img) + o * 3;
                const int sw = (normalise & 4) ? 2 : 0;
                r = __fdiv_rn((float)u[sw], 255.0f); g = __fdiv_rn((float)u[1], 255.0f); b = __fdiv_rn((float)u[2 - sw], 255.0f);
            } else {
                r = img[o]; g = img[plane + o]; b = img[2 * plane + o];
            }
            if (normalise & 1) {
                r = __fdiv_rn(__fsub_rn(r, 0.485f), 0.229f);
                g = __fdiv_rn(__fsub_rn(g, 0.456f), 0.224f);
                b = __fdiv_rn(__fsub_rn(b, 0.406f), 0.225f);
            }
        }
        *reinterpret_cast<h4_t *>(Xs + p * 4) = cvt4(r, g, b, 0.0f);
    }

    h8_t a[2][3];
#pragma unroll
    for (int ct = 0; ct < 2; ++ct)
#pragma unroll
        for (int ky = 0; ky < 3; ++ky)
            a[ct][ky] = *reinterpret_cast<const h8_t *>(wpk + ((size_t)(ct * 3 + ky) * 64 + lane) * 8);
    __syncthreads();

    f32x16_t acc[2][2];
#pragma unroll
    for (int i = 0; i < 2; ++i)
#pragma unroll
        for (int j = 0; j < 2; ++j)
#pragma unroll
            for (int r = 0; r < 16; ++r) acc[i][j][r] = 0.0f;

    const int lrow = lane & 31, lg = lane >> 5;
#pragma unroll
    for (int ky = 0; ky < 3; ++ky)
#pragma unroll
        for (int pr = 0; pr < 2; ++pr) {
            const int q = (wave * 2 + pr + ky) * C1_PW + lrow + 2 * lg;
            const h4_t lo = *reinterpret_cast<const h4_t *>(Xs + q * 4);
            const h4_t hi = *reinterpret_cast<const h4_t *>(Xs + (q + 1) * 4);
            h8_t b;
            b[0] = lo[0]; b[1] = lo[1]; b[2] = lo[2]; b[3] = lo[3];
            b[4] = hi[0]; b[5] = hi[1]; b[6] = hi[2]; b[7] = hi[3];
#pragma unroll
            for (int ct = 0; ct < 2; ++ct)
                acc[ct][pr] = __builtin_amdgcn_mfma_f32_32x32x16_f16(a[ct][ky], b, acc[ct][pr], 0, 0, 0);
        }

#pragma unroll
    for (int pr = 0; pr < 2; ++pr) {
        const int oy = oy0 + wave * 2 + pr, ox = ox0 + lrow;
        if (oy < H && ox < W) {
// ... 165 lines not shown
```

sfd2_amd/csrc/post_kernels.hip:

```cpp
#include "sfd2_internal.h"
#include <math.h>
#include <stdlib.h>

#define NT 256

__device__ __forceinline__ float wave_sum(float v)
{
#pragma unroll
    for (int m = 32; m >= 1; m >>= 1) v += __shfl_xor(v, m);
    return v;
}

__global__ __launch_bounds__(NT)
void detector_head_kernel(const float *__restrict__ logits, int pitch, int hc, int wc, float *__restrict__ score)
{
    const int lane = threadIdx.x & 63;
    const int cell = blockIdx.x * (NT / 64) + (threadIdx.x >> 6);
    if (cell >= hc * wc) return;
    const int y = cell / wc, x = cell - y * wc;
    const float *p = logits + (size_t)cell * pitch;
    const float e = expf(p[lane]);
    const float ed = expf(p[64]);
    const float den = (wave_sum(e) + ed) + 0.00001f;
    score[(size_t)(8 * y + (lane >> 3)) * (8 * wc) + 8 * x + (lane & 7)] = e / den;
}

void launch_detector_head(hipStream_t st, const float *logits, int pitch, int hc, int wc, float *score)
{
    const int cells = hc * wc;
    hipLaunchKernelGGL(detector_head_kernel, dim3((cells + 3) / 4), dim3(NT), 0, st, logits, pitch, hc, wc, score);
}

struct LinCoef { int i0, i1; float l0, l1; };
__device__ __forceinline__ LinCoef lin_coef(int dst, int in_size, int out_size, float scale)
{
    LinCoef c;
    if (in_size == out_size) { c.i0 = dst; c.i1 = dst; c.l0 = 1.0f; c.l1 = 0.0f; return c; }
    float src = __fmaf_rn(scale, (float)dst + 0.5f, -0.5f);
    if (src < 0.0f) src = 0.0f;
    int a = (int)floorf(src);
    if (a > in_size - 1) a = in_size - 1;
    float lam = __fsub_rn(src, (float)a);
    lam = fminf(fmaxf(lam, 0.0f), 1.0f);
    c.i0 = a;
    c.i1 = (a + 1 < in_size) ? a + 1 : in_size - 1;
    c.l1 = lam;
    c.l0 = __fsub_rn(1.0f, lam);
    return c;
}
__device__ __forceinline__ float bilerp(const float *__restrict__ p, int w, const LinCoef &cy, const LinCoef &cx)
{
    const float v00 = p[(size_t)cy.i0 * w + cx.i0], v01 = p[(size_t)cy.i0 * w + cx.i1];
    const float v10 = p[(size_t)cy.i1 * w + cx.i0], v11 = p[(size_t)cy.i1 * w + cx.i1];
    const float top = __fmaf_rn(v00, cx.l0, __fmul_rn(v01, cx.l1));
    const float bot = __fmaf_rn(v10, cx.l0, __fmul_rn(v11, cx.l1));
    return __fmaf_rn(top, cy.l0, __fmul_rn(bot, cy.l1));
}

__global__ __launch_bounds__(NT)
void heatmap_kernel(const float *__restrict__ score, int hs, int ws, float sc_y, float sc_x,
                    const float *__restrict__ sta, int hc, int wc, float st_y, float st_x,
                    int H, int W, float *__restrict__ heat, float *__restrict__ stab_out)
{
    const int x = blockIdx.x * 64 + (threadIdx.x & 63);
    const int y = blockIdx.y * 4 + (threadIdx.x >> 6);
    if (x >= W || y >= H) return;
    float s;
    if (hs == H && ws == W) {
        s = score[(size_t)y * ws + x];
    } else {
        const LinCoef cy = lin_coef(y, hs, H, sc_y), cx = lin_coef(x, ws, W, sc_x);
        s = bilerp(score, ws, cy, cx);
    }
    float stab = 1.0f;
    if (sta) {
        const LinCoef cy = lin_coef(y, hc, H, st_y), cx = lin_coef(x, wc, W, st_x);
        const size_t plane = (size_t)hc * wc;
        const float v0 = bilerp(sta, wc, cy, cx);
        const float v1 = bilerp(sta + plane, wc, cy, cx);
        const float v2 = bilerp(sta + 2 * plane, wc, cy, cx);
        int best = 0;
        float bv = v0;
        if (v1 > bv) { bv = v1; best = 1; }
        if (v2 > bv) { bv = v2; best = 2; }
        stab = best == 0 ? 0.1f : (best == 1 ? 0.5f : 1.0f);
        if (stab_out) stab_out[(size_t)y * W + x] = stab;
    }
    if (heat) heat[(size_t)y * W + x] = __fmul_rn(s, stab);
}

void launch_heatmap(hipStream_t st, const float *score, int hs, int ws, const float *sta, int hc, int wc,
                    int H, int W, float *heat, float *stab_out)
{
    const float sc_y = (float)hs / (float)H, sc_x = (float)ws / (float)W;
    const float st_y = hc > 0 ? (float)hc / (float)H : 1.0f, st_x = wc > 0 ? (float)wc / (float)W : 1.0f;
    hipLaunchKernelGGL(heatmap_kernel, dim3((W + 63) / 64, (H + 3) / 4), dim3(NT), 0, st, score, hs, ws, sc_y, sc_x,
                       sta, hc, wc, st_y, st_x, H, W, heat, stab_out);
}

__global__ __launch_bounds__(NT)
void heads_heat_kernel(const float *__restrict__ logits, int pitch, int hc8, int wc8, const float *__restrict__ sta, int hc, int wc,
                       float st_y, float st_x, int H, int W, float *__restrict__ heat)
{
    const int lane = threadIdx.x & 63;
    const int cell = blockIdx.x * (NT / 64) + (threadIdx.x >> 6);
    if (cell >= hc8 * wc8) return;
    const int cy = cell / wc8, cx = cell - cy * wc8;
    const float *p = logits + (size_t)cell * pitch;
    const float e = expf(p[lane]);
    const float ed = expf(p[64]);
    const float den = (wave_sum(e) + ed) + 0.00001f;
    const float s = e / den;
    const int y = 8 * cy + (lane >> 3), x = 8 * cx + (lane & 7);
    float stab = 1.0f;
    if (sta) {
        const LinCoef ly = lin_coef(y, hc, H, st_y), lx = lin_coef(x, wc, W, st_x);
        const size_t plane = (size_t)hc * wc;
        const float v0 = bilerp(sta, wc, ly, lx);
        const float v1 = bilerp(sta + plane, wc, ly, lx);
        const float v2 = bilerp(sta + 2 * plane, wc, ly, lx);
        int best = 0;
        float bv = v0;
        if (v1 > bv) { bv = v1; best = 1; }
        if (v2 > bv) { bv = v2; best = 2; }
        stab = best == 0 ? 0.1f : (best == 1 ? 0.5f : 1.0f);
    }
    heat[(size_t)y * W + x] = __fmul_rn(s, stab);
}

void launch_heads_heat(hipStream_t st, const float *logits, int pitch, int hc8, int wc8, const float *sta, int hc, int wc,
                       int H, int W, float *heat)
{
    const float st_y = hc > 0 ? (float)hc / (float)H : 1.0f, st_x = wc > 0 ? (float)wc / (float)W : 1.0f;
    const int cells = hc8 * wc8;
    hipLaunchKernelGGL(heads_heat_kernel, dim3((cells + 3) / 4), dim3(NT), 0, st, logits, pitch, hc8, wc8, sta, hc, wc, st_y, st_x, H, W, heat);
}

#define PH_CELLS 32
#define PH_XREC 528
#define PH_OREC 100
__global__ __launch_bounds__(NT)
void pb_heads_heat_kernel(const half_t *__restrict__ fmap , int hc8, int wc8,
                          const half_t *__restrict__ wpk , int CoutP, const float *__restrict__ scale,
                          const float *__restrict__ shift, const float *__restrict__ sta, int hc, int wc, float st_y, float st_x,
                          int H, int W, float *__restrict__ heat, unsigned int *__restrict__ zero_words, int n_zero)
{
    if (zero_words && (int)(blockIdx.x * blockDim.x + threadIdx.x) < n_zero) zero_words[blockIdx.x * blockDim.x + threadIdx.x] = 0u;
    __shared__ __attribute__((aligned(16))) unsigned char X[PH_CELLS * PH_XREC];
    __shared__ __attribute__((aligned(16))) float O[PH_CELLS * PH_OREC];
    const int tid = threadIdx.x, lane = tid & 63, wave = tid >> 6;
    const int lrow = lane & 31, lhi = lane >> 5;
    const int ncell = hc8 * wc8, c0cell = blockIdx.x * PH_CELLS;

    h8_t a[16];
    if (wave < 3) {
#pragma unroll
        for (int kk = 0; kk < 16; ++kk)
            a[kk] = *reinterpret_cast<const h8_t *>(wpk + ((size_t)(kk >> 1) * CoutP + wave * 32 + lrow) * 32 + (kk & 1) * 16 + lhi * 8);
    }
    for (int rec = wave * 2 + lhi; rec < PH_CELLS; rec += 8) {
        const int cell = c0cell + rec;
        uint4 v = make_uint4(0, 0, 0, 0);
        if (cell < ncell) v = *reinterpret_cast<const uint4 *>(fmap + (size_t)cell * 256 + lrow * 8);
        *reinterpret_cast<uint4 *>(X + rec * PH_XREC + lrow * 16) = v;
    }
    __syncthreads();
    if (wave < 3) {
        f32x16_t acc;
#pragma unroll
        for (int r = 0; r < 16; ++r) acc[r] = 0.0f;
#pragma unroll
        for (int kk = 0; kk < 16; ++kk) {
            const h8_t b = *reinterpret_cast<const h8_t *>(X + lrow * PH_XREC + kk * 32 + lhi * 16);
            acc = __builtin_amdgcn_mfma_f32_32x32x16_f16(a[kk], b, acc, 0, 0, 0);
        }
#pragma unroll
        for (int q = 0; q < 4; ++q) {
            const int c0 = wave * 32 + 8 * q + 4 * lhi;
            const float4 sc = *reinterpret_cast<const float4 *>(scale + c0);
            const float4 sh = *reinterpret_cast<const float4 *>(shift + c0);
            *reinterpret_cast<float4 *>(O + lrow * PH_OREC + c0) =
                make_float4(acc[4 * q + 0] * sc.x + sh.x, acc[4 * q + 1] * sc.y + sh.y, acc[4 * q + 2] * sc.z + sh.z, acc[4 * q + 3] * sc.w + sh.w);
        }
    }
    __syncthreads();
#pragma unroll 4
    for (int jj = 0; jj < PH_CELLS / (NT / 64); ++jj) {
        const int j = wave + jj * (NT / 64);
        const bool live = c0cell + j < ncell;
        const int cell = live ? c0cell + j : ncell - 1;
        const int cy = cell / wc8, cx = cell - cy * wc8;
        const float *p = O + j * PH_OREC;
        const float e = expf(p[lane]);
        const float ed = expf(p[64]);
        const float den = (wave_sum(e) + ed) + 0.00001f;
        const float s = e / den;
        const int y = 8 * cy + (lane >> 3), x = 8 * cx + (lane & 7);
        float stab = 1.0f;
        if (sta) {
            const LinCoef ly = lin_coef(y, hc, H, st_y), lx = lin_coef(x, wc, W, st_x);
            const size_t plane = (size_t)hc * wc;
            const float v0 = bilerp(sta, wc, ly, lx);
            const float v1 = bilerp(sta + plane, wc, ly, lx);
            const float v2 = bilerp(sta + 2 * plane, wc, ly, lx);
            int best = 0;
            float bv = v0;
            if (v1 > bv) { bv = v1; best = 1; }
            if (v2 > bv) { bv = v2; best = 2; }
            stab = best == 0 ? 0.1f : (best == 1 ? 0.5f : 1.0f);
        }
        if (live) heat[(size_t)y * W + x] = __fmul_rn(s, stab);
    }
}

void launch_pb_heads_heat(hipStream_t st, const half_t *fmap, int hc8, int wc8, const half_t *wpk, int CoutP, const float *scale,
                          const float *shift, const float *sta, int hc, int wc, int H, int W, float *heat, unsigned int *zero_words,
                          int n_zero)
{
    const float st_y = hc > 0 ? (float)hc / (float)H : 1.0f, st_x = wc > 0 ? (float)wc / (float)W : 1.0f;
// ... 714 lines not shown
```

sfd2_amd/csrc/sfd2_ctx.h:

```cpp
#pragma once
#include "../../include/sfd2_hip.h"
#include "sfd2_internal.h"

#include <algorithm>
#include <atomic>
#include <cstdlib>
#include <cmath>
#include <cstdio>
#include <cstring>
#include <string>
#include <vector>

int sfd2_fail(const std::string &m);
#define fail sfd2_fail
struct PoseCam;
bool sfd2_pose_cam(int model, const double *params, PoseCam &c, std::string &why);
#define HIPCHECK(expr)                                                                           \
    do {                                                                                          \
        hipError_t e_ = (expr);                                                                   \
        if (e_ != hipSuccess)                                                                     \
            return fail(std::string(#expr) + ": " + hipGetErrorString(e_) + " @" + std::to_string(__LINE__)); \
    } while (0)

extern std::atomic<unsigned long long> g_alloc_gen;
// ... 94 lines not shown
    template <typename T> T *as() const { return reinterpret_cast<T *>(p); }
};
inline hipError_t grow(ScratchBuf &b, size_t bytes)
{
    if (bytes <= b.cap) return hipSuccess;
    if (b.p) (void)hipFree(b.p);
    b.p = nullptr;
    b.cap = 0;
    hipError_t e = hipMalloc(&b.p, bytes);
    if (e == hipSuccess) b.cap = bytes;
    return e;
}
struct JpegScratch {
    ScratchBuf in[2];
    hipEvent_t ev_copied[2] = {}, ev_free[2] = {};
    int slot = 0;
    ScratchBuf lanes, pre, coef, planes;
    ScratchBuf words;
    ~JpegScratch()
    {
        for (int i = 0; i < 2; ++i) {
            if (ev_copied[i]) (void)hipEventDestroy(ev_copied[i]);
            if (ev_free[i]) (void)hipEventDestroy(ev_free[i]);
        }
    }
};

struct sfd2_ctx {
    int device = 0;
    hipStream_t stream = nullptr;
    hipEvent_t ev[4] = {nullptr, nullptr, nullptr, nullptr};
    hipEvent_t ev_jobs = nullptr;
    hipStream_t copy_stream = nullptr;
#define SFD2_IMG_SLOTS 4
    hipEvent_t ev_copied[SFD2_IMG_SLOTS] = {}, ev_img_free[SFD2_IMG_SLOTS] = {};
    DevBuf img2[SFD2_IMG_SLOTS];
    int img_slot = 0, img_slot_used = -1;
    void *pin_jobs = nullptr;
    size_t pin_cap = 0;
    bool weights_loaded = false;
    bool counters_clean = false;
    bool has_sta = false;
    int opt_alias = 1;
    int act_exp[AE_COUNT] = {};
    float act_max[AE_COUNT] = {};
    int opt_range_fallback = 1;
    int range_fallbacks = 0;
    int in_fallback = 0;
    int prof_step_entry = 0;
    float range_hist[SFD2_RS_COUNT] = {};
    int opt_auto_range = 1;
    std::vector<float> h_sta_w;
    int opt_cu_limit = 0;
    int fuse_det = 0;
    int use_graphs = 0;
    DevBuf x3_chain[2];
    DevBuf x3_rb_planes[3];
    int opt_fuse_post = 1;
    int opt_sparse_desc = 1;
    DevBuf da3_sparse;
    int opt_fp6_acts = 1;
    int net_error = 0;
    int opt_trunk_r1 = 1;
    int opt_s2d = 1;
    int opt_fp6_filters = 0;
    int opt_x3_pp = 1;
    int opt_auto_margin = 1;
    float margin_err[4] = {-1.0f, -1.0f, -1.0f, -1.0f};
    int margin_choice = -1;
    int opt_c3b_plain = 0;
    int user_c3b_plain = -1;
    bool margin_done = false, margin_pending = false;
    float relax_err = -1.0f;
    bool user_set_rb_inner = false, user_set_comp_heads = false;
    int user_rb_inner = 2, user_comp_heads = 0;
    int opt_x3_desc16 = 0;
    DevBuf x3_planes;
    DevBuf x3_da0_planes;
    DevBuf db_sparse;
    int opt_sparse_da3 = 1;
    int opt_sparse_da0 = 1;
    DevPtr da0_in;
    int opt_fuse_pb = 1;
    int opt_comp_rb = 1;
    int opt_rb_inner = 2;
    int opt_fuse_rb23 = 1;
    int opt_comp_det = 0;
    int opt_comp_heads = 0;
    int opt_no_rf_c = 0;
    int opt_generic_c = 0;
    int opt_branches = 0;
    int opt_sta_side = 0;
    hipStream_t side_stream = nullptr;
    hipStream_t cur_stream = nullptr;
    hipEvent_t ev_fork = nullptr, ev_join = nullptr;
    struct GraphEntry *graphs = nullptr;
    int n_graphs = 0;
    unsigned long long graph_clock = 0;
    ConvW c1a, c1b, c2a, c2b, c3a, c3b, rb1[3], rb2[3], rb3[3], pa0, pa3, da0, da3, pb, db;
    DevBuf sta_w16;
    DevPtr range_stat;
    DevPtr range_hist_dev;
    DevPtr extract_rec;
    DevBuf range_scratch;
    DevBuf sta_w, sta_b, zero_page, w1b_fused;
    DevBuf w1b_stem_c6;
    DevBuf w1b_stem_c;
    DevBuf w1b_stem_x3;
    int fuse = 1;
    int precision = SFD2_PREC_F16;
    ConvW f1a, f1b, f2a, f2b, f3a, f3b, frb1[3], frb2[3], frb3[3], fpa0, fpa3, fda0, fda3, fpb, fdb;
    DevBuf act32[T_COUNT];
    int H = 0, W = 0, H2 = 0, W2 = 0, H4 = 0, W4 = 0, H8 = 0, W8 = 0;
    DevBuf img, act16[T_COUNT];
    DevBuf logits , draw , sta , score , heat ;
    DevBuf stab , desc_nchw, tmp_f32;
    DevBuf cand, bnd, sel, sorted, counters, kpts, kscores, kdesc;
    DevBuf kdesc64;
    DevBuf g_keys, g_state0, g_state1, g_kept;
    int cand_cap = 0;
    int last_sel_cap = 0;
    float *kpts_cur = nullptr, *kscores_cur = nullptr;
    DevBuf arena;
    DevBuf img_u8_packed;
    JpegScratch jpeg;
    ScratchBuf asm_in, asm_ws, asm_out;
    ScratchBuf pose_in, pose_ws, pose_out;
    ScratchBuf tv_in, tv_ws, tv_out;
    ScratchBuf tri_in, tri_ws;
    ScratchBuf pairs_in, pairs_ws;
    ScratchBuf vlad_in, vlad_ws;
    ScratchBuf ba_in, ba_ws;
    ScratchBuf map_in, map_ws;
    DevBuf img_scaled, ms_kp, ms_sc, ms_de, ms_keys, ms_sorted, ms_cnt;
    unsigned int ms_cand_seen[8] = {};
    int ms_cand_cap[8] = {};
    DevBuf m_stage, m_hi0, m_lo0, m_hi1, m_lo1, m_part_f, m_part_i, m_red, m_jobs, m_fins, m_out_m, m_out_s, m_rkeys;
    sfd2_timings tim = {};
    ActInfo acts[T_ALL] = {};
    int prof_max_steps = 0, prof_step = 0, prof_slot = 0;
    std::vector<hipEvent_t> prof_ev;
    std::vector<sfd2_layer_timing> prof_tab;
    std::vector<int> prof_used;
    std::vector<int> prof_row;
    std::string prof_filter;
};

void graphs_release(sfd2_ctx *c);
#define PROF_SLOTS 48
struct ProfScope {
    sfd2_ctx *c; int slot;
    ProfScope(sfd2_ctx *c_, const char *name, const char *kernel, double flops, double bytes) : c(c_), slot(-1)
    {
        if (c->prof_max_steps <= 0 || c->prof_step >= c->prof_max_steps || c->prof_slot >= PROF_SLOTS) return;
        if (!c->prof_filter.empty() && strstr(kernel, c->prof_filter.c_str()) == nullptr) return;
        slot = c->prof_slot++;
        int row = -1;
        for (size_t i = 0; i < c->prof_tab.size(); ++i)
            if (strncmp(c->prof_tab[i].name, name, sizeof(c->prof_tab[i].name) - 1) == 0) { row = (int)i; break; }
        if (row < 0) {
            c->prof_tab.push_back(sfd2_layer_timing{});
            row = (int)c->prof_tab.size() - 1;
            snprintf(c->prof_tab[row].name, sizeof(c->prof_tab[row].name), "%s", name);
            snprintf(c->prof_tab[row].kernel, sizeof(c->prof_tab[row].kernel), "%s", kernel);
        }
        c->prof_tab[row].flops = flops;
        c->prof_tab[row].bytes = bytes;
        c->prof_row[(size_t)c->prof_step * PROF_SLOTS + slot] = row;
        (void)hipEventRecord(c->prof_ev[((size_t)c->prof_step * PROF_SLOTS + slot) * 2], c->cur_stream);
    }
    void cancel()
    {
        if (slot >= 0 && slot == c->prof_slot - 1) c->prof_slot--;
        slot = -1;
    }
    ~ProfScope()
    {
        if (slot >= 0) (void)hipEventRecord(c->prof_ev[((size_t)c->prof_step * PROF_SLOTS + slot) * 2 + 1], c->cur_stream);
    }
};
static inline void prof_step_begin(sfd2_ctx *c) { c->prof_slot = 0; }
static inline void prof_step_end(sfd2_ctx *c)
{
    if (c->prof_max_steps > 0 && c->prof_step < c->prof_max_steps) {
        c->prof_used[c->prof_step] = c->prof_slot;
        c->prof_step++;
    }
}

int apply_act_exponents(sfd2_ctx *c);
int read_range_status(sfd2_ctx *c, sfd2_range_status *out, int reset);
int range_wants_fallback(sfd2_ctx *c);
int range_fold_before_sync_extract(sfd2_ctx *c);
int sfd2_margin_selfcheck_if_pending(sfd2_ctx *c);
int reset_range_records(sfd2_ctx *c);
struct FallbackScope {
    sfd2_ctx *c; int prec;
    explicit FallbackScope(sfd2_ctx *c_) : c(c_), prec(c_->precision)
    {
        c->precision = SFD2_PREC_F16X3; c->in_fallback = 1; c->range_fallbacks++;
        if (c->prof_step > c->prof_step_entry) c->prof_step = c->prof_step_entry;
    }
    ~FallbackScope() { c->precision = prec; c->in_fallback = 0; }
};
enum PassEntry { PASS_DET , PASS_DENSE , PASS_EXTRACT  };
enum StrictLayer { SL_C1B, SL_C2A, SL_C2B, SL_C3A, SL_C3B, SL_RB1, SL_RB3 = SL_RB1 + 3, SL_PA0 = SL_RB3 + 3, SL_PA3, SL_PB, SL_DA0, SL_DA3, SL_DB, SL_COUNT };
template <class Ctx> auto &strict_layer(Ctx *c, int i)
{
    decltype(&c->f1b) t[] = {&c->f1b, &c->f2a, &c->f2b, &c->f3a, &c->f3b, &c->frb1[0], &c->frb1[1], &c->frb1[2], &c->frb3[0], &c->frb3[1], &c->frb3[2],
                             &c->fpa0, &c->fpa3, &c->fpb, &c->fda0, &c->fda3, &c->fdb};
    static_assert(sizeof(t) == SL_COUNT * sizeof(t[0]), "one entry per StrictLayer");
    return *t[i];
}
enum X3Kind { XK_GENERIC, XK_PP, XK_RF, XK_S2D, XK_SKIP };
enum X3Out { X3_F32, X3_CHAIN_A, X3_CHAIN_B, X3_RB, X3_DA0 };
struct StrictConv { X3Kind kind = XK_GENERIC; bool planes_in = false; X3Out out = X3_F32; bool s2d_out = false; };
struct X3Pair { half_t *hi = nullptr, *lo = nullptr; };
struct PassPlan {
    bool f32 = false, comp = false;
    bool fuse = false, alias = false;
    bool fused_stem = false, rb_fused = false;
    bool comp_rb = false;
    int rb_inner = 0;
    bool rb23 = false, generic_c = false, no_rf_c = false, fp6_filters = false;
    Rec rec[T_COUNT] = {};
    Rec a3a_in = Rec::None;
    bool a2a_s2d = false;
    bool ch = false, chp = false;
    bool branches = false, sta_early = false, sta_side = false;
    bool skip_head = false, skip_pb = false, skip_db = false, skip_da3 = false;
    bool sparse_desc = false, sparse_da3 = false, sparse_x3 = false;
    bool sparse_da0 = false;
    struct { int slot = -1; size_t off = 0; } at[T_COUNT];
    int n_slots = 0;
    size_t slot_bytes = 0;
    bool x3_pp = false, x3_fast = false;
    bool x3_stem = false, x3_rb = false;
    bool desc16 = false;
    StrictConv sl[SL_COUNT];
};
PassPlan plan_pass(const sfd2_ctx *c, PassEntry entry, int H, int W, int top_k = 0, bool desc = false);
int ensure_workspace(sfd2_ctx *c, const PassPlan &p, int H, int W);
int run_network(sfd2_ctx *c, const PassPlan &p, const float *img_dev, int normalise);
inline DevPtr act_view(const sfd2_ctx *c, const PassPlan &p, int id)
{
    if (id >= T_COUNT) return id == T_PB ? c->logits : id == T_DB ? c->draw : c->sta;
    if (p.f32) return (id == T_DA0 && p.desc16) ? c->x3_da0_planes : c->act32[id];
    if (!p.alias || p.at[id].slot < 0) return c->act16[id];
    DevPtr v;
    v.p = c->arena.as<char>() + (size_t)p.at[id].slot * p.slot_bytes + p.at[id].off;
    return v;
}
inline int act_h(const sfd2_ctx *c, int id) { const int h[4] = {c->H, c->H2, c->H4, c->H8}; return h[kTensor[id].level]; }
inline int act_w(const sfd2_ctx *c, int id) { const int w[4] = {c->W, c->W2, c->W4, c->W8}; return w[kTensor[id].level]; }
inline size_t cand_capacity(size_t P1) { return std::min(std::max<size_t>(65536, P1 / 8), P1); }
int convf_at(sfd2_ctx *c, const StrictConv &s, const char *name, const ConvW &L, const DevPtr &in, int H, int W, const DevPtr &out, int Ho, int Wo,
             int relu, const float *res = nullptr, X3Pair *planes = nullptr);
int ensure_strict_filters(sfd2_ctx *c, const PassPlan &p);
int copy_out(sfd2_ctx *c, void *dst, const void *src_dev, size_t bytes, int dst_on_device);
```

sfd2_amd/csrc/sfd2_internal.h:

```cpp
#pragma once
#include <hip/hip_runtime.h>
#include <hip/hip_fp16.h>
#include <stdint.h>

#ifdef SFD2_EXPERIMENTS
#include <stdlib.h>
static inline const char *sfd2_env(const char *name) { return getenv(name); }
#else
static inline const char *sfd2_env(const char *) { return nullptr; }
#endif

extern thread_local int g_sfd2_cu_limit;
static inline int sfd2_slots(int cus) { return (g_sfd2_cu_limit > 0 && g_sfd2_cu_limit < cus) ? g_sfd2_cu_limit : cus; }

#define SFD2_BARRIER_DRAIN() asm volatile("s_waitcnt vmcnt(0) lgkmcnt(0)\n\ts_barrier" ::: "memory")

typedef _Float16 half_t;
typedef _Float16 h8_t __attribute__((ext_vector_type(8)));
typedef _Float16 h4_t __attribute__((ext_vector_type(4)));
typedef float f32x16_t __attribute__((ext_vector_type(16)));

#ifdef __HIPCC__
__device__ __forceinline__ float4 sfd2_lds_f4(const float *p)
{
// ... 217 lines not shown
    int e8 = (int)(mb >> 23) - 4 + ((mb & 0x7fffffu) > 0x600000u ? 1 : 0);
    e8 = e8 < 1 ? 1 : e8;
    const float scale = __uint_as_float((unsigned int)e8 << 23);
    asm volatile("v_cvt_scalef32_2xpk16_bf6_f32 %0, %1, %2, %3" : "=&v"(d) : "v"(l), "v"(v), "v"(scale));
#else
    int e8 = (int)(mb >> 23) - 2 + ((mb & 0x7fffffu) > 0x700000u ? 1 : 0);
    e8 = e8 < 1 ? 1 : e8;
    const float scale = __uint_as_float((unsigned int)e8 << 23);
    asm volatile("v_cvt_scalef32_2xpk16_fp6_f32 %0, %1, %2, %3" : "=&v"(d) : "v"(l), "v"(v), "v"(scale));
#endif
    rec0 = make_uint4((unsigned)d[0], (unsigned)d[1], (unsigned)d[2], (unsigned)d[3]);
    rec1 = make_uint4((unsigned)d[4], (unsigned)d[5], (unsigned)e8 * 0x01010101u, 0u);
}
__device__ __forceinline__ float sfd2_corr_lo(unsigned d, int ch )
{
    return (ch ? __builtin_amdgcn_cvt_f32_fp8((int)d, 2) : __builtin_amdgcn_cvt_f32_fp8((int)d, 0)) * (1.0f / (float)(1 << SFD2_C_XL_SHIFT));
}
#endif


void launch_conv1a(hipStream_t st, const float *img_chw, int H, int W, int normalise,
                   const half_t *wpk , const float *scale, const float *shift,
                   half_t *out );

void launch_fused_stem(hipStream_t st, const float *img, int H, int W, int normalise, const half_t *w1, const float *sc1,
                       const float *sh1, const half_t *w2, const float *sc2, const float *sh2, half_t *out, int H2, int W2);

bool conv3x3_pp_serves(int ks, int stride, int CoutP, int Cin);
bool launch_conv3x3_rf_x3(hipStream_t st, const half_t *in_hi, const half_t *in_lo, int H, int W, int Cin, const half_t *wpl,
                          const float *scale, const float *shift, int CoutP, int stride, int relu, half_t *out_hi, half_t *out_lo,
                          float *out_f32, int Ho, int Wo, const half_t *zero_page);
bool conv3x3_rf_serves(int ks, int stride, int CoutP, int Cin, int Ho, int Wo);
void launch_conv_igemm(hipStream_t st, const half_t *in, int H, int W, int Cin,
                       const half_t *wpk, const float *scale, const float *shift, int Cout_pad,
                       int ks, int stride, int relu, const half_t *residual,
                       void *out, int out_f32, int Ho, int Wo, const half_t *zero_page );

int conv_igemm_chunk(int ks, int stride, int Cout_pad, int Cin);

void launch_gconv3x3_g8(hipStream_t st, const half_t *in, int H, int W, const half_t *wpk,
                        const float *scale, const float *shift, half_t *out);

void launch_convsta(hipStream_t st, const half_t *in, int npix, const float *w , const float *b,
                    float *out );

enum class Rec {
    None,
    Unit8,
    Half6,
    Resid8,
};
void launch_convc_igemm(hipStream_t st, const half_t *in, const half_t *in_c, int H, int W, int Cin, const half_t *wpk,
                        const float *scale, const float *shift, int Cout_pad, int ks, int stride, int relu,
                        const half_t *res, const half_t *res_c, half_t *out, half_t *out_c, int Ho, int Wo, int sbyte, unsigned int *range = nullptr);
bool launch_conv3x3_pp_c(hipStream_t st, const half_t *in, const half_t *in_c, int H, int W, int Cin, const half_t *wpk,
                         const float *scale, const float *shift, int CoutP, int relu, half_t *out, half_t *out_c,
                         int Ho, int Wo, const half_t *zero_page, int sbyte,
                         unsigned int *range ,
                         Rec rin, Rec rout, bool s2d_out, bool fp6_w);
bool conv3x3_rf_c_serves(int ks, int stride, int CoutP, int Cin, int Ho, int Wo);
bool conv2b_s2d_serves(int H2, int W2, int Cin, int CoutP);
void launch_conv2b_s2d(hipStream_t st, const half_t *in_s2d, const half_t *in_c_s2d, int H4, int W4, const half_t *wpk, const float *scale,
                       const float *shift, int relu, half_t *out, half_t *out_c, const half_t *zero_page, int sbyte, unsigned int *range, Rec rout );
void launch_conv2b_s2d_x3(hipStream_t st, const half_t *in_hi_s2d, const half_t *in_lo_s2d, int H4, int W4, const half_t *wpk ,
                          const float *scale, const float *shift, int relu, half_t *out_hi, half_t *out_lo, const half_t *zero_page);
bool launch_conv3x3_rf_c(hipStream_t st, const half_t *in, const half_t *in_c, int H, int W, int Cin, const half_t *wpk,
                         const float *scale, const float *shift, int CoutP, int stride, int relu, half_t *out, half_t *out_c,
                         int Ho, int Wo, const half_t *zero_page, int sbyte, unsigned int *range, Rec rin , Rec rout );
bool launch_conv_igemm2_c(hipStream_t st, const half_t *in, const half_t *in_c, int H, int W, int Cin, const half_t *wpk,
                          const float *scale, const float *shift, int CoutP, int ks, int stride, int relu,
                          const half_t *res, const half_t *res_c, half_t *out, half_t *out_c, int Ho, int Wo,
                          const half_t *zero_page, int sbyte, unsigned int *range = nullptr);
void launch_fused_stem_c(hipStream_t st, const float *img, int H, int W, int normalise, const half_t *w1, const float *sc1,
                         const float *sh1, const void *w2, const float *sc2, const float *sh2, half_t *out, half_t *out_c,
                         int H2, int W2, int sbyte, unsigned int *range_base = nullptr ,
                         Rec rout = Rec::Unit8 );
void launch_conv1x1_c256_c(hipStream_t st, const half_t *in, const half_t *in_c, int npix, const half_t *w_frag,
                           const half_t *wc_frag, const float *scale, const float *shift, int relu, const half_t *res,
                           const half_t *res_c, half_t *out, half_t *out_c, const half_t *zero_page, int sbyte, unsigned int *range,
                           Rec rin , Rec rout );
bool sparse_da0_serves(int cin, int CoutP, int hc, int wc);
void launch_sparse_da0(hipStream_t st, const half_t *in, int hc, int wc, int nh, int nw, const half_t *wpk, const float *scale, const float *shift,
                       int relu, const float *kpts, const unsigned int *count, int n_max, half_t *out);
void launch_sparse_da3(hipStream_t st, const half_t *fmap, int hc, int wc, int nh, int nw, const half_t *wpk, const half_t *wsl, int CoutP,
                       const float *scale, const float *shift, int relu, const float *kpts, const unsigned int *count, int n_max,
                       half_t *out, const half_t *zero_page);
void launch_sparse_da3_repack(hipStream_t st, const half_t *w, half_t *dst, int CoutP, int cin);
void launch_sparse_da3_x3(hipStream_t st, const half_t *fmap_hi, const half_t *fmap_lo, int hc, int wc, int nh, int nw, const half_t *wpk, const half_t *wsl,
                          int CoutP, const float *scale, const float *shift, int relu, const float *kpts, const unsigned int *count,
                          int n_max, float *out, const half_t *zero_page);
void launch_rb23_c(hipStream_t st, const half_t *t1, int H, int W, const half_t *w2h, const half_t *w2l, const float *sc2,
                   const float *sh2, const half_t *w3h, const half_t *w3l, const float *sc3, const float *sh3,
                   const half_t *res, const half_t *res_c, half_t *out, half_t *out_c, const half_t *zero_page,
                   unsigned int *range_t2, unsigned int *range_out, Rec rres, Rec rout ,
                   const half_t *w3l8, int sbyte3 );
void launch_conv1x1_c256_x3(hipStream_t st, const half_t *in, const half_t *in_lo, int npix, const half_t *w, const half_t *wl,
                            const float *scale, const float *shift, int relu, const void *res, const half_t *res_lo, float *out, half_t *out_hi,
                            half_t *out_lo, const half_t *zero_page);
void launch_conv1a_c(hipStream_t st, const float *img, int H, int W, int normalise, const half_t *wpk ,
                     const float *scale, const float *shift, half_t *out, half_t *out_c, unsigned int *range = nullptr);
void launch_gconv_c(hipStream_t st, const half_t *in, const half_t *in_c, int H, int W, const half_t *wpk ,
                    const void *wck , const float *scale, const float *shift, half_t *out, half_t *out_c, int sbyte,
                    int row0, int row1 , unsigned int *range = nullptr);
void launch_nhwc_hc_to_nchw_f(hipStream_t st, const half_t *in, const half_t *in_c, int npix, int pitch, int c, float *out, Rec rec );

void launch_conv_igemm_f32(hipStream_t st, const float *in, int H, int W, int Cin, const float *wpk,
                           const float *scale, const float *shift, int Cout_pad, int ks, int stride, int relu,
                           const float *residual, float *out, int Ho, int Wo);
void launch_x3_split(hipStream_t st, const float *w, size_t n_floats, void *out);
void launch_x3_split_planes(hipStream_t st, const float *in, size_t n_floats, void *hi_out, void *lo_out);
void launch_conv3x3_pp_x3(hipStream_t st, const half_t *in, const half_t *in_lo, int H, int W, int Cin, const half_t *wpk,
                          const float *scale, const float *shift, int CoutP, int relu, half_t *out_hi, half_t *out_lo, float *out_f32,
                          int Ho, int Wo, const half_t *zero_page, int s2d = 0 );
void launch_gconv_x3_pack(hipStream_t st, const float *w , void *out );
void launch_gconv_x3(hipStream_t st, const float *in, int H, int W, const void *wpk, const float *scale, const float *shift, float *out);
void launch_conv_igemm_x3(hipStream_t st, const float *in, int H, int W, int Cin, const float *wpk,
                           const float *scale, const float *shift, int Cout_pad, int ks, int stride, int relu,
                           const float *residual, float *out, int Ho, int Wo);
void launch_conv1a_f32(hipStream_t st, const float *img_chw, int H, int W, int normalise, const float *w ,
                       const float *scale, const float *shift, float *out );
void launch_gconv_f32(hipStream_t st, const float *in, int H, int W, const float *w , const float *scale,
                      const float *shift, float *out);
void launch_convsta_f32(hipStream_t st, const float *in, int npix, const float *w, const float *b, float *out);

void launch_detector_head(hipStream_t st, const float *logits, int pitch, int hc, int wc, float *score);
void launch_heatmap(hipStream_t st, const float *score, int hs, int ws, const float *sta, int hc, int wc,
                    int H, int W, float *heat, float *stab_out );
bool launch_nms_select(hipStream_t st, const float *heat, int H, int W, int radius, float conf_th, int border, int Hb, int Wb,
                       float *nms_dense , unsigned long long *cand_keys, int cand_cap,
                       unsigned int *counters , int fuse_threshold = 0, int top_k = 0);
void launch_heads_heat(hipStream_t st, const float *logits, int pitch, int hc8, int wc8, const float *sta, int hc, int wc,
                       int H, int W, float *heat);
void launch_topk_sort(hipStream_t st, bool threshold_done, const unsigned long long *cand, int cand_cap, int top_k,
                      unsigned long long *sel, unsigned long long *sorted, int sel_cap, unsigned int *counters,
                      unsigned long long *bnd, int W, float *kpts, float *scores);
#define SFD2_HIST_BINS 4096
#define SFD2_COUNTER_BYTES (64 + SFD2_HIST_BINS * 4)
__device__ __forceinline__ unsigned int key_bin(unsigned long long key)
{
    const int b = (int)((unsigned int)(key >> 47) & 0xFFFFu) - ((127 - 12) << 8);
    return (unsigned int)(b < 0 ? 0 : (b > SFD2_HIST_BINS - 1 ? SFD2_HIST_BINS - 1 : b));
}

__device__ __forceinline__ unsigned int sfd2_ld_agent(const unsigned int *p)
{
    return __hip_atomic_load(p, __ATOMIC_RELAXED, __HIP_MEMORY_SCOPE_AGENT);
}

template <bool COHERENT>
__device__ __forceinline__ void sfd2_select_threshold(int cand_cap, int top_k, unsigned int *__restrict__ counters, unsigned int *wsum)
{
    static_assert(SFD2_HIST_BINS == 4096, "one uint4 of bins per thread");
    const unsigned int *hist = counters + 16;
    unsigned int n = COHERENT ? sfd2_ld_agent(counters) : counters[0];
    if (n > (unsigned int)cand_cap) n = cand_cap;
    const unsigned int k = (top_k <= 0 || (unsigned int)top_k > n) ? n : (unsigned int)top_k;
    if (k == n) {
        if (threadIdx.x == 0) { counters[1] = n; counters[2] = 0; counters[3] = 0; counters[4] = 0; counters[5] = 0; counters[6] = 1; }
        return;
    }
    const int t = threadIdx.x, lane = t & 63, wave = t >> 6;
    uint4 hv;
    if (COHERENT) hv = make_uint4(sfd2_ld_agent(hist + 4 * t), sfd2_ld_agent(hist + 4 * t + 1), sfd2_ld_agent(hist + 4 * t + 2), sfd2_ld_agent(hist + 4 * t + 3));
    else hv = reinterpret_cast<const uint4 *>(hist)[t];
    const unsigned int sum = hv.x + hv.y + hv.z + hv.w;
    unsigned int suf = sum;
#pragma unroll
    for (int d = 1; d < 64; d <<= 1) {
        const unsigned int o = __shfl_down(suf, d);
        if (lane + d < 64) suf += o;
    }
    if (lane == 0) wsum[wave] = suf;
    __syncthreads();
    unsigned int higher = 0;
    for (int w = wave + 1; w < 16; ++w) higher += wsum[w];
    const unsigned int above_incl = higher + suf;
    unsigned int above = above_incl - sum;
    if (above < k && above_incl >= k) {
        const unsigned int b[4] = {hv.x, hv.y, hv.z, hv.w};
#pragma unroll
        for (int j = 3; j >= 0; --j) {
            if (above < k && above + b[j] >= k) {
                counters[1] = k; counters[2] = 0; counters[3] = 0;
                counters[4] = 4 * t + j;
                counters[5] = k - above;
                counters[6] = 0;
            }
            above += b[j];
        }
    }
}

void launch_nms4_select(hipStream_t st, const float *heat, int H, int W, float conf_th, int border, int Hb, int Wb, float *nms_dense,
                        unsigned long long *cand, int cand_cap, unsigned int *counters, unsigned int *hist, int fuse_threshold, int top_k);
void launch_greedy_init(hipStream_t st, const float *heat, int n, float conf_th, unsigned long long *keys, unsigned char *state);
void launch_greedy_iter(hipStream_t st, const unsigned long long *keys, const unsigned char *sin, unsigned char *sout,
                        int H, int W, int dist, unsigned int *undecided);
void launch_greedy_final(hipStream_t st, const float *heat, const unsigned char *state, int n, float *kept);
void launch_keys_to_kpts(hipStream_t st, const unsigned long long *sorted_keys, const unsigned int *counters,
                         int W, float *kpts_xy, float *scores, int cap);
void launch_sample_desc(hipStream_t st, const float *desc_nhwc, int hc, int wc, int nh, int nw,
                        const float *kpts_xy, const unsigned int *count , int n_max,
                        float *out, int compact = 0);
void launch_pb_heads_heat(hipStream_t st, const half_t *fmap, int hc8, int wc8, const half_t *wpk, int CoutP, const float *scale,
                          const float *shift, const float *sta, int hc, int wc, int H, int W, float *heat,
                          unsigned int *zero_words , int n_zero);
bool pb_heads_heat_clears(int hc8, int wc8, int n_zero);
void launch_desc_store64(hipStream_t st, const float *in , const unsigned int *count, int n_max, double *out , int pitch);
void launch_desc_head(hipStream_t st, const half_t *fmap, int hc, int wc, int nh, int nw, const half_t *wpk, int CoutP,
                      const float *scale, const float *shift, const float *kpts, const unsigned int *count, int n_max, float *out, int compact = 0);
void launch_desc_normalise_nchw(hipStream_t st, const float *desc_nhwc, int npix, float *out_nchw);
void launch_nhwc_h_to_nchw_f(hipStream_t st, const half_t *in, int npix, int c_pitch, int c, float *out);
void launch_nhwc_f_to_nchw_f(hipStream_t st, const float *in, int npix, int c_pitch, int c, float *out);
void launch_nchw_f_to_nhwc_f(hipStream_t st, const float *in, int npix, int c, float *out);

// ... 260 lines not shown
```

Before: 714.3.

## Fold 3x3 conv and following 1x1 conv into one 3x3 conv for heads

After: 719.7 (median of 6 runs). Within noise of the previous version (+0.8%).

```diff
diff --git a/sfd2_amd/_lib.py b/sfd2_amd/_lib.py
--- a/sfd2_amd/_lib.py
+++ b/sfd2_amd/_lib.py
@@ -303,6 +303,23 @@
     return lib
 
 
+def fold_conv_pair(w3, b3, w1, b1):
+    lib = load()
+    fn = lib.sfd2_fold_conv_pair
+    vp, ci = ctypes.c_void_p, ctypes.c_int
+    fn.argtypes = [vp, vp, vp, vp, ci, ci, ci, vp, vp]
+    w3 = np.ascontiguousarray(w3, dtype=np.float32)
+    mid, cin = w3.shape[0], w3.shape[1]
+    w1 = np.ascontiguousarray(w1, dtype=np.float32).reshape(-1, mid)
+    cout = w1.shape[0]
+    b3 = None if b3 is None else np.ascontiguousarray(b3, dtype=np.float32)
+    b1 = None if b1 is None else np.ascontiguousarray(b1, dtype=np.float32)
+    w = np.empty((cout, cin, 3, 3), np.float64)
+    b = np.empty((cout,), np.float64)
+    check(fn(ptr(w3), ptr(b3), ptr(w1), ptr(b1), cin, mid, cout, ptr(w), ptr(b)))
+    return w, b
+
+
 def check(rc):
     if rc != 0:
         raise RuntimeError("libsfd2hip: " + load().sfd2_last_error().decode("utf-8", "replace"))
diff --git a/sfd2_amd/build.py b/sfd2_amd/build.py
--- a/sfd2_amd/build.py
+++ b/sfd2_amd/build.py
@@ -4,10 +4,10 @@
 HERE = os.path.dirname(os.path.abspath(__file__))
 CSRC = os.path.join(HERE, "csrc")
 LIB = os.path.join(HERE, "libsfd2hip.so")
-SOURCES = ["conv_kernels.hip", "conv2_kernels.hip", "conv3_kernels.hip", "conv3rf_kernels.hip", "conv2b_s2d_kernel.hip", "conv1x1_kernels.hip", "resblock_kernel.hip", "conv_f32_kernels.hip", "convc_kernels.hip", "rb23_c_kernel.hip", "sparse_da3_kernel.hip", "sparse_da0_kernel.hip", "fused_stem_kernel.hip", "fused_stem_c_kernel.hip", "post_kernels.hip", "util_kernels.hip", "nms4_kernels.hip", "match_kernels.hip", "match_mutual_kernel.hip", "api_core.hip", "api_weights.hip", "api_network.hip", "api_extract.hip", "api_match.hip", "api_graph.hip", "jpeg_parse.hip", "jpeg_kernels.hip", "api_jpeg.hip", "pose_kernels.hip", "api_pose.hip", "two_view_kernels.hip", "api_two_view.hip", "assemble_kernels.hip", "api_assemble.hip", "tri_kernels.hip", "api_triangulate.hip", "pairs_kernels.hip", "api_pairs.hip", "cluster_kernels.hip", "api_cluster.hip", "frames_kernels.hip", "api_frames.hip", "vlad_kernels.hip", "api_vlad.hip", "bundle_kernels.hip", "api_bundle.hip", "mapper_kernels.hip", "api_mapper.hip"]
+SOURCES = ["conv_kernels.hip", "conv2_kernels.hip", "conv3_kernels.hip", "conv3rf_kernels.hip", "conv2b_s2d_kernel.hip", "conv1x1_kernels.hip", "resblock_kernel.hip", "conv_f32_kernels.hip", "convc_kernels.hip", "rb23_c_kernel.hip", "sparse_da3_kernel.hip", "sparse_da0_kernel.hip", "fold_pab_kernel.hip", "fold_dab_kernel.hip", "fused_stem_kernel.hip", "fused_stem_c_kernel.hip", "post_kernels.hip", "util_kernels.hip", "nms4_kernels.hip", "match_kernels.hip", "match_mutual_kernel.hip", "api_core.hip", "api_weights.hip", "api_network.hip", "api_extract.hip", "api_match.hip", "api_graph.hip", "jpeg_parse.hip", "jpeg_kernels.hip", "api_jpeg.hip", "pose_kernels.hip", "api_pose.hip", "two_view_kernels.hip", "api_two_view.hip", "assemble_kernels.hip", "api_assemble.hip", "tri_kernels.hip", "api_triangulate.hip", "pairs_kernels.hip", "api_pairs.hip", "cluster_kernels.hip", "api_cluster.hip", "frames_kernels.hip", "api_frames.hip", "vlad_kernels.hip", "api_vlad.hip", "bundle_kernels.hip", "api_bundle.hip", "mapper_kernels.hip", "api_mapper.hip"]
 _NN = ["-fno-honor-nans"]
 SRC_FLAGS = {"match_mutual_kernel.hip": _NN, "conv3_kernels.hip": _NN, "conv3rf_kernels.hip": _NN, "resblock_kernel.hip": _NN, "conv2_kernels.hip": _NN,
-             "fused_stem_kernel.hip": _NN, "conv_kernels.hip": _NN, "conv1x1_kernels.hip": _NN, "nms4_kernels.hip": _NN, "convc_kernels.hip": _NN, "fused_stem_c_kernel.hip": _NN, "rb23_c_kernel.hip": _NN, "sparse_da3_kernel.hip": _NN, "sparse_da0_kernel.hip": _NN, "conv2b_s2d_kernel.hip": _NN}
+             "fused_stem_kernel.hip": _NN, "conv_kernels.hip": _NN, "conv1x1_kernels.hip": _NN, "nms4_kernels.hip": _NN, "convc_kernels.hip": _NN, "fused_stem_c_kernel.hip": _NN, "rb23_c_kernel.hip": _NN, "sparse_da3_kernel.hip": _NN, "sparse_da0_kernel.hip": _NN, "fold_pab_kernel.hip": _NN, "fold_dab_kernel.hip": _NN, "conv2b_s2d_kernel.hip": _NN}
 FLAGS = ["--offload-arch=gfx950", "-O3", "-std=c++17", "-fPIC", "-Wall", "-Wno-unused-function"] + \
     os.environ.get("SFD2_EXTRA_FLAGS", "").split()
 
diff --git a/sfd2_amd/csrc/api_core.hip b/sfd2_amd/csrc/api_core.hip
--- a/sfd2_amd/csrc/api_core.hip
+++ b/sfd2_amd/csrc/api_core.hip
@@ -124,6 +124,8 @@
     else if (k == "s2d") c->opt_s2d = value ? 1 : 0;
     else if (k == "trunk_r1") c->opt_trunk_r1 = value ? 1 : 0;
     else if (k == "fuse_pb") c->opt_fuse_pb = value ? 1 : 0;
+    else if (k == "fold_pab") c->opt_fold_pab = value ? 1 : 0;
+    else if (k == "fold_dab") c->opt_fold_dab = value ? 1 : 0;
     else if (k == "generic_c") c->opt_generic_c = value ? 1 : 0;
     else if (k == "comp_rb") c->opt_comp_rb = value ? 1 : 0;
     else if (k == "no_rf_c") c->opt_no_rf_c = value ? 1 : 0;
@@ -145,7 +147,7 @@
         {"fuse_post", c->opt_fuse_post}, {"sparse_desc", c->opt_sparse_desc}, {"sparse_da3", c->opt_sparse_da3}, {"sparse_da0", c->opt_sparse_da0}, {"cu_limit", c->opt_cu_limit},
         {"auto_range", c->opt_auto_range}, {"range_fallback", c->opt_range_fallback}, {"x3_pp", c->opt_x3_pp}, {"x3_desc16", c->opt_x3_desc16},
         {"auto_margin", c->opt_auto_margin}, {"fp6_filters", c->opt_fp6_filters}, {"fp6_acts", c->opt_fp6_acts}, {"s2d", c->opt_s2d},
-        {"trunk_r1", c->opt_trunk_r1}, {"fuse_pb", c->opt_fuse_pb}, {"generic_c", c->opt_generic_c}, {"comp_rb", c->opt_comp_rb},
+        {"trunk_r1", c->opt_trunk_r1}, {"fuse_pb", c->opt_fuse_pb}, {"fold_pab", c->opt_fold_pab}, {"fold_dab", c->opt_fold_dab}, {"generic_c", c->opt_generic_c}, {"comp_rb", c->opt_comp_rb},
         {"no_rf_c", c->opt_no_rf_c}, {"comp_heads", c->opt_comp_heads}, {"c3b_plain", c->opt_c3b_plain}, {"comp_det", c->opt_comp_det},
         {"fuse_rb23", c->opt_fuse_rb23}, {"rb_inner", c->opt_rb_inner},
     };
diff --git a/sfd2_amd/csrc/api_extract.hip b/sfd2_amd/csrc/api_extract.hip
--- a/sfd2_amd/csrc/api_extract.hip
+++ b/sfd2_amd/csrc/api_extract.hip
@@ -171,8 +171,11 @@
         c->counters_clean = pb_heads_heat_clears(c->H8, c->W8, SFD2_COUNTER_BYTES / 4);
     } else if (plan.skip_head) {
         ProfScope ps(c, "heads+heatmap", "heads_heat_kernel", 0.0, (double)c->H8 * c->W8 * 65 * 4 + (double)H * W * 4);
+        const bool clr = plan.fold_pab && heads_heat_clears(c->H8, c->W8, SFD2_COUNTER_BYTES / 4);
         launch_heads_heat(c->stream, c->logits.as<float>(), 128, c->H8, c->W8,
-                          (flags & SFD2_FLAG_NO_STABILITY) ? nullptr : c->sta.as<float>(), c->H4, c->W4, H, W, c->heat.as<float>());
+                          (flags & SFD2_FLAG_NO_STABILITY) ? nullptr : c->sta.as<float>(), c->H4, c->W4, H, W, c->heat.as<float>(),
+                          clr ? c->counters.as<unsigned int>() : nullptr, clr ? SFD2_COUNTER_BYTES / 4 : 0);
+        c->counters_clean = clr;
     } else {
         ProfScope ps(c, "heatmap", "heatmap_kernel", 0.0, (double)H * W * 8);
         launch_heatmap(c->stream, c->score.as<float>(), HS, WS,
@@ -221,6 +224,16 @@
                 launch_sparse_da0(c->stream, c->da0_in.as<half_t>(), c->H4, c->W4, H, W, L0.w.as<half_t>(), L0.scale.as<float>(), L0.shift.as<float>(), 1,
                                   c->kpts_cur, c->counters.as<unsigned int>() + 1, sel_cap, act_view(c, plan, T_DA0).as<half_t>());
             }
+            if (plan.fold_dab) {
+                const ConvW &L = c->dab;
+                {
+                    ProfScope ps(c, "convDa.3", "desc_fold_kernel", 2.0 * 4 * sel_cap * (double)L.cout * L.cin * 9, (double)sel_cap * (16 * 512 + 4 * 512) + 2.0 * L.cout_pad * L.cin * 9);
+                    launch_desc_fold(c->stream, act_view(c, plan, T_DA0).as<half_t>(), c->H4, c->W4, H, W, L.wsl.as<half_t>(), L.scale.as<float>(), L.shift.as<float>(),
+                                     c->kpts_cur, c->counters.as<unsigned int>() + 1, sel_cap, c->da3_sparse.as<float>(), c->zero_page.as<half_t>());
+                }
+                ProfScope ps(c, "desc_head", "sample_desc_kernel", 0.0, (double)sel_cap * (4 * 512 + 512));
+                launch_sample_desc(c->stream, c->da3_sparse.as<float>(), c->H4, c->W4, H, W, c->kpts_cur, c->counters.as<unsigned int>() + 1, sel_cap, desc_dst, 1);
+            } else {
             {
                 ProfScope ps(c, "convDa.3", "sparse_da3_kernel", 2.0 * 4 * sel_cap * 256.0 * 256.0 * 9, (double)sel_cap * (16 * 512 + 4 * 512) + 2.0 * 256 * 256 * 9);
                 launch_sparse_da3(c->stream, act_view(c, plan, T_DA0).as<half_t>(), c->H4, c->W4, H, W, c->da3.w.as<half_t>(), c->da3.wsl.as<half_t>(), c->da3.cout_pad, c->da3.scale.as<float>(),
@@ -230,6 +243,10 @@
             ProfScope ps(c, "desc_head", "desc_head_kernel", 2.0 * 4 * sel_cap * 128 * 256, (double)sel_cap * (4 * 512 + 512));
             launch_desc_head(c->stream, c->da3_sparse.as<half_t>(), c->H4, c->W4, H, W, c->db.w.as<half_t>(), c->db.cout_pad, c->db.scale.as<float>(),
                              c->db.shift.as<float>(), c->kpts_cur, c->counters.as<unsigned int>() + 1, sel_cap, desc_dst, 1);
+            }
+        } else if (plan.fold_dab) {
+            ProfScope ps(c, "desc_head", "sample_desc_kernel", 0.0, (double)sel_cap * 128 * 4 * 5);
+            launch_sample_desc(c->stream, c->draw.as<float>(), c->H4, c->W4, H, W, c->kpts_cur, c->counters.as<unsigned int>() + 1, sel_cap, desc_dst);
         } else if (plan.sparse_desc) {
             ProfScope ps(c, "desc_head", "desc_head_kernel", 2.0 * 4 * sel_cap * 128 * 256, (double)sel_cap * (4 * 512 + 512));
             launch_desc_head(c->stream, act_view(c, plan, T_DA).as<half_t>(), c->H4, c->W4, H, W, c->db.w.as<half_t>(), c->db.cout_pad, c->db.scale.as<float>(),
diff --git a/sfd2_amd/csrc/api_network.hip b/sfd2_amd/csrc/api_network.hip
--- a/sfd2_amd/csrc/api_network.hip
+++ b/sfd2_amd/csrc/api_network.hip
@@ -63,9 +63,11 @@
         p.rec[T_DA0] = p.ch ? Rec::Unit8 : Rec::None;
     }
     p.branches = c->opt_branches;
+    p.fold_pab = c->opt_fold_pab && !det && !p.f32 && !p.chp && c->pab.w.p && c->pab.cin == c->pa0.cout_pad &&
+                 det_fold_serves(c->pab.cin, down2(H4), down2(W4));
     if (entry == PASS_EXTRACT) {
         p.skip_head = c->opt_fuse_post && H % 8 == 0 && W % 8 == 0;
-        p.skip_pb = p.skip_head && c->opt_fuse_pb && p.fuse && !p.branches && c->pb.cout_pad >= 96;
+        p.skip_pb = p.skip_head && c->opt_fuse_pb && p.fuse && !p.branches && c->pb.cout_pad >= 96 && !p.fold_pab;
         const bool few = desc && top_k > 0 && (size_t)16 * top_k <= (size_t)H4 * W4;
         p.sparse_desc = c->opt_sparse_desc && p.fuse && few;
         p.sparse_da3 = p.sparse_desc && c->opt_sparse_da3 && !p.ch && !p.branches;
@@ -73,10 +75,11 @@
         p.sparse_da0 = p.sparse_da3 && c->opt_sparse_da0 && c->da0.w.p && c->da0.ks == 3 && c->da0.stride == 1 &&
                        sparse_da0_serves(c->da0.cin, c->da0.cout_pad, H4, W4) &&
                        (c->opt_sparse_da0 >= 2 || (double)16 * top_k <= SFD2_DA0_FRAC * (double)H4 * W4);
-        p.skip_db = p.sparse_desc;
+        p.fold_dab = c->opt_fold_dab && few && !p.f32 && !p.chp && !p.branches && c->dab.w.p && c->dab.wsl.p && c->dab.cin == c->da0.cout_pad;
+        p.skip_db = p.sparse_desc || p.fold_dab;
         p.skip_da3 = p.sparse_da3 || p.sparse_x3;
     }
-    p.sta_early = p.alias && p.skip_pb;
+    p.sta_early = p.alias && (p.skip_pb || (p.fold_pab && entry == PASS_EXTRACT && !p.branches));
     p.sta_side = c->has_sta && p.sta_early && c->opt_sta_side && !p.branches;
     if (p.alias) {
         static const int slots[T_COUNT] = {-1 , 0, 1 , 0, 1, 2, 0, 2, 0 , 1, 1, 1 ,
@@ -195,11 +198,12 @@
         if (ensure_strict_filters(c, p)) return -1;
     } else if (!layers) {
         if (p.sparse_da0) reg(T_DA0, act_view(c, p, T_DA0).p, 0, 0, kTensor[T_DA0].ch).absent = true;
+        if (p.fold_dab) reg(T_DA, act_view(c, p, T_DA).p, 0, 0, kTensor[T_DA].ch).absent = true;
         return 0;
     }
     for (int id = 0; id < T_COUNT; ++id) {
         if (p.f32) reg(id, c->act32[id].p, 1, 0, kTensor[id].ch).absent = p.x3_fast && id != T_OUT_0 + 2 && id != T_PA;
-        else if (!on_chip(id)) reg(id, c->act16[id].p, 0, 0, kTensor[id].ch, id < T_PA0 ? p.rec[id] : Rec::None).absent = (p.rb23 && id >= T_T2_0 && id < T_OUT_0) || (p.sparse_da0 && id == T_DA0);
+        else if (!on_chip(id)) reg(id, c->act16[id].p, 0, 0, kTensor[id].ch, id < T_PA0 ? p.rec[id] : Rec::None).absent = (p.rb23 && id >= T_T2_0 && id < T_OUT_0) || (p.sparse_da0 && id == T_DA0) || (p.fold_pab && id == T_PA) || (p.fold_dab && id == T_DA);
     }
     return 0;
 }
@@ -611,9 +615,15 @@
         convc(c, p, "convPa.3", c->pa3, T_PA0, T_PA, 0);
     } else {
         conv(c, p, "convPa.0", c->pa0, x, T_PA0, 1);
+        if (p.fold_pab) {
+            const ConvW &L = c->pab;
+            ProfScope ps(c, "convPa.3", "det_fold_kernel", 2.0 * P8 * L.cout * L.cin * 9, 2.0 * (P8 * L.cin + (double)L.cout * L.cin * 9) + P8 * 72 * 4.0);
+            launch_det_fold(c->cur_stream, V(T_PA0).as<half_t>(), H8, W8, L.cin, L.w.as<half_t>(), L.scale.as<float>(), L.shift.as<float>(), L.cout,
+                            c->logits.as<float>(), 128);
+        } else
         conv(c, p, "convPa.3", c->pa3, T_PA0, T_PA, 0);
     }
-    if (!p.skip_pb) conv(c, p, "convPb", c->pb, T_PA, T_PB, 0, T_NONE, 1);
+    if (!p.skip_pb && !p.fold_pab) conv(c, p, "convPb", c->pb, T_PA, T_PB, 0, T_NONE, 1);
     if (!p.skip_head) {
         ProfScope ps(c, "detector_head", "detector_head_kernel", 0.0, P8 * (65 * 4 + 256));
         launch_detector_head(c->cur_stream, c->logits.as<float>(), 128, H8, W8, c->score.as<float>());
@@ -628,7 +638,8 @@
     } else {
         if (p.sparse_da0) c->da0_in = V(x);
         else conv(c, p, "convDa.0", c->da0, x, T_DA0, 1);
-        if (!p.skip_da3) conv(c, p, "convDa.3", c->da3, T_DA0, T_DA, 0);
+        if (!p.skip_da3 && p.fold_dab) conv(c, p, "convDa.3", c->dab, T_DA0, T_DB, 0, T_NONE, 1);
+        else if (!p.skip_da3) conv(c, p, "convDa.3", c->da3, T_DA0, T_DA, 0);
     }
     if (!p.skip_db) conv(c, p, "convDb", c->db, T_DA, T_DB, 0, T_NONE, 1);
     if (c->has_sta && !p.sta_early) conv_sta();
diff --git a/sfd2_amd/csrc/api_weights.hip b/sfd2_amd/csrc/api_weights.hip
--- a/sfd2_amd/csrc/api_weights.hip
+++ b/sfd2_amd/csrc/api_weights.hip
@@ -260,6 +260,64 @@
     return 0;
 }
 
+extern "C" int sfd2_fold_conv_pair(const float *w3, const float *b3, const float *w1, const float *b1, int cin, int mid, int cout,
+                                   double *w_out, double *b_out)
+{
+    if (!w3 || !w1 || !w_out || !b_out || cin <= 0 || mid <= 0 || cout <= 0) return fail("sfd2_fold_conv_pair: bad argument");
+    const size_t per = (size_t)cin * 9;
+    for (int o = 0; o < cout; ++o) {
+        double *wo = w_out + (size_t)o * per;
+        for (size_t i = 0; i < per; ++i) wo[i] = 0.0;
+        double b = b1 ? (double)b1[o] : 0.0;
+        for (int mm = 0; mm < mid; ++mm) {
+            const double a = (double)w1[(size_t)o * mid + mm];
+            const float *wm = w3 + (size_t)mm * per;
+            for (size_t i = 0; i < per; ++i) wo[i] += a * (double)wm[i];
+            if (b3) b += a * (double)b3[mm];
+        }
+        b_out[o] = b;
+    }
+    return 0;
+}
+
+static int pack_folded_pair(sfd2_ctx *c, const TMap &m, ConvW &L, const std::string &conv3, const std::string &conv1, int cin, int mid,
+                            int cout, int cout_pad)
+{
+    const TView *w3 = find_t(m, conv3 + ".weight"), *w1 = find_t(m, conv1 + ".weight");
+    const TView *b3 = find_t(m, conv3 + ".bias"), *b1 = find_t(m, conv1 + ".bias");
+    if (!w3 || !w1) return fail("missing tensor: " + conv3 + " / " + conv1 + ".weight");
+    if (w3->numel() != (size_t)mid * cin * 9 || w1->numel() != (size_t)cout * mid || (b3 && (int)b3->numel() != mid) ||
+        (b1 && (int)b1->numel() != cout) || cout > cout_pad || cin % 32 != 0)
+        return fail("bad shape for the folded pair " + conv3 + " + " + conv1);
+    const size_t per = (size_t)cin * 9;
+    std::vector<float> f3(w3->d, w3->d + w3->numel()), f1(w1->d, w1->d + w1->numel());
+    for (int mm = 0; mm < mid && !w3->ec.empty(); ++mm)
+        for (size_t i = 0; i < per; ++i) f3[mm * per + i] = std::ldexp(f3[mm * per + i], w3->ec[mm]);
+    for (int o = 0; o < cout && !w1->ec.empty(); ++o)
+        for (int mm = 0; mm < mid; ++mm) f1[(size_t)o * mid + mm] = std::ldexp(f1[(size_t)o * mid + mm], w1->ec[o]);
+    std::vector<double> wf((size_t)cout * per), bf(cout);
+    if (sfd2_fold_conv_pair(f3.data(), b3 ? b3->d : nullptr, f1.data(), b1 ? b1->d : nullptr, cin, mid, cout, wf.data(), bf.data())) return -1;
+    L.cin = cin; L.cout = cout; L.cout_pad = cout_pad; L.ks = 3; L.stride = 1;
+    std::vector<half_t> pk((size_t)(cin / 32) * 9 * cout_pad * 32, (half_t)0.0f);
+    std::vector<float> sc(cout_pad, 1.0f), sh(cout_pad, 0.0f);
+    for (int o = 0; o < cout; ++o) {
+        double mx = 0.0;
+        for (size_t i = 0; i < per; ++i) mx = std::max(mx, std::fabs(wf[o * per + i]));
+        int e = 0;
+        if (mx > 0.0 && std::isfinite(mx)) {
+            (void)std::frexp(mx, &e);
+            e = std::max(-100, std::min(100, e - 1));
+        }
+        sc[o] = std::ldexp(1.0f, e);
+        sh[o] = (float)bf[o];
+        for (int ci = 0; ci < cin; ++ci)
+            for (int t = 0; t < 9; ++t)
+                pk[(((size_t)(ci / 32) * 9 + t) * cout_pad + o) * 32 + ci % 32] = (half_t)(float)std::ldexp(wf[o * per + (size_t)ci * 9 + t], -e);
+    }
+    if (upload(L.w, pk.data(), pk.size() * sizeof(half_t), c->stream)) return -1;
+    return set_scale_shift(c, L, sc, sh);
+}
+
 static int pack_conv1a(sfd2_ctx *c, const TMap &m)
 {
     const TView *w = find_t(m, "conv1a.0.weight");
@@ -567,6 +625,10 @@
     launch_sparse_da3_repack(c->stream, c->da3.w.as<half_t>(), c->da3.wsl.as<half_t>(), c->da3.cout_pad, 256);
     if (pack_igemm(c, m, c->pb, "convPb", "", 256, 65, 1, 1)) return -1;
     if (pack_igemm(c, m, c->db, "convDb", "", 256, 128, 1, 1)) return -1;
+    if (pack_folded_pair(c, m, c->pab, "convPa.3", "convPb", 256, 256, 65, det_fold_cout_pad())) return -1;
+    if (pack_folded_pair(c, m, c->dab, "convDa.3", "convDb", 256, 256, 128, desc_fold_cout_pad())) return -1;
+    HIPCHECK(c->dab.wsl.ensure((size_t)(256 / 32) * 9 * c->dab.cout_pad * 32 * sizeof(half_t)));
+    launch_sparse_da3_repack(c->stream, c->dab.w.as<half_t>(), c->dab.wsl.as<half_t>(), c->dab.cout_pad, 256);
     const TView *sw = find_t(m, "ConvSta.weight"), *sb = find_t(m, "ConvSta.bias");
     c->has_sta = false;
     if (sw || sb) {
@@ -598,7 +660,7 @@
     std::vector<Row> rows = {
         {&c->c1a, -1, AE_CONV1A}, {&c->c1b, AE_CONV1A, AE_CONV1B}, {&c->c2a, AE_CONV1B, AE_CONV2A}, {&c->c2b, AE_CONV2A, AE_CONV2B},
         {&c->c3a, AE_CONV2B, AE_CONV3A}, {&c->c3b, AE_CONV3A, AE_TRUNK}, {&c->pa0, AE_TRUNK, AE_PA0}, {&c->pa3, AE_PA0, -1},
-        {&c->da0, AE_TRUNK, AE_DA0}, {&c->da3, AE_DA0, -1}};
+        {&c->da0, AE_TRUNK, AE_DA0}, {&c->da3, AE_DA0, -1}, {&c->pab, AE_PA0, -1}, {&c->dab, AE_DA0, -1}};
     for (int b = 0; b < 3; ++b) {
         rows.push_back({&c->rb1[b], AE_TRUNK, AE_T1_0 + b});
         rows.push_back({&c->rb2[b], AE_T1_0 + b, AE_T2_0 + b});
diff --git a/sfd2_amd/csrc/conv_kernels.hip b/sfd2_amd/csrc/conv_kernels.hip
--- a/sfd2_amd/csrc/conv_kernels.hip
+++ b/sfd2_amd/csrc/conv_kernels.hip
@@ -252,6 +252,8 @@
         if (bn == 256) SFD2_IGEMM(1, 1, 256, false);
         else if (bn == 128) SFD2_IGEMM(1, 1, 128, false);
         else SFD2_IGEMM(1, 1, 64, false);
+    } else if (ks == 3 && stride == 1 && out_f32 && bn == 128) {
+        SFD2_IGEMM(3, 1, 128, true);
     } else if (ks == 1 && stride == 1 && out_f32) {
         if (bn == 256) SFD2_IGEMM(1, 1, 256, true);
         else if (bn == 128) SFD2_IGEMM(1, 1, 128, true);
diff --git a/sfd2_amd/csrc/fold_dab_kernel.hip b/sfd2_amd/csrc/fold_dab_kernel.hip
--- /dev/null
+++ b/sfd2_amd/csrc/fold_dab_kernel.hip
@@ -0,0 +1,124 @@
+#include "sfd2_internal.h"
+
+#define FD_KP 16
+#define FD_NT 256
+#define FD_C 128
+#define FD_RING 4
+
+typedef __attribute__((address_space(3))) void fd_lds_t;
+typedef const __attribute__((address_space(1))) void fd_gbl_t;
+
+__global__ __launch_bounds__(FD_NT, 2)
+void desc_fold_kernel(const half_t *__restrict__ fmap , int hc, int wc, float half_w, float half_h,
+                      const half_t *__restrict__ wsl ,
+                      const float *__restrict__ scale, const float *__restrict__ shift,
+                      const float *__restrict__ kpts, const unsigned int *__restrict__ count, int n_max,
+                      float *__restrict__ out , const half_t *__restrict__ zero_page)
+{
+    __shared__ __attribute__((aligned(16))) unsigned char X[FD_KP * 16 * 128];
+    __shared__ int geo[2 * FD_KP];
+    const int tid = threadIdx.x, lane = tid & 63;
+    const int wave = __builtin_amdgcn_readfirstlane(tid >> 6);
+    const int lrow = lane & 31, lhi = lane >> 5;
+    int n = n_max;
+    const int k0 = blockIdx.x * FD_KP;
+    float kpx = 0.0f, kpy = 0.0f;
+    if (tid < FD_KP) {
+        const int kp = k0 + tid < n_max ? k0 + tid : n_max - 1;
+        kpx = kpts[2 * kp];
+        kpy = kpts[2 * kp + 1];
+    }
+    const int n0 = wave * 32;
+#define FD_LOAD_A(dst_, c_, tap_)                                                                                          \
+    _Pragma("unroll") for (int k16 = 0; k16 < 4; ++k16)                                                                   \
+        dst_[k16] = *reinterpret_cast<const h8_t *>(wsl + ((size_t)(((c_)*2 + (k16 >> 1)) * 9 + (tap_)) * FD_C + n0) * 32 + (k16 & 1) * 512 + lane * 8);
+    constexpr int DIST = FD_RING - 1;
+    h8_t an[FD_RING][4];
+#pragma unroll
+    for (int i = 0; i < DIST; ++i) { FD_LOAD_A(an[i], 0, i) }
+    if (count) { const unsigned int c = *count; if ((unsigned int)n > c) n = (int)c; }
+    if (k0 >= n) return;
+
+    if (tid < FD_KP) {
+        int x0, y0;
+        if (k0 + tid >= n) kpx = kpy = 0.0f;
+        sd_corner(kpx, kpy, half_w, half_h, hc, wc, x0, y0);
+        geo[2 * tid] = x0;
+        geo[2 * tid + 1] = y0;
+    }
+    __syncthreads();
+
+    f32x16_t acc[2];
+#pragma unroll
+    for (int t = 0; t < 2; ++t)
+#pragma unroll
+        for (int r = 0; r < 16; ++r) acc[t][r] = 0.0f;
+
+    int recb[2];
+#pragma unroll
+    for (int t = 0; t < 2; ++t) recb[t] = (t * 8 + (lrow >> 2)) * 16 + ((lrow >> 1) & 1) * 4 + (lrow & 1);
+    const int kcode = (lrow >> 2) & 3;
+
+#pragma unroll
+    for (int c = 0; c < 4; ++c) {
+        if (c) __syncthreads();
+#pragma unroll
+        for (int i = 0; i < 8; ++i) {
+            const int j = wave + 4 * i;
+            const int kpl = j >> 1, ppix = (j & 1) * 8 + (lane >> 3), slot = lane & 7;
+            const int x0 = geo[2 * kpl], y0 = geo[2 * kpl + 1];
+            const int iy = y0 - 1 + (ppix >> 2), ix = x0 - 1 + (ppix & 3);
+            const int part = slot ^ (ppix & 7) ^ (kpl & 3);
+            const bool ok = iy >= 0 && iy < hc && ix >= 0 && ix < wc;
+            const half_t *src = ok ? fmap + ((size_t)iy * wc + ix) * 256 + c * 64 + part * 8 : zero_page + slot * 8;
+            __builtin_amdgcn_global_load_lds((fd_gbl_t *)src, (fd_lds_t *)(X + j * 1024), 16, 0, 0);
+        }
+        asm volatile("s_waitcnt vmcnt(0)" ::: "memory");
+        __syncthreads();
+#pragma unroll
+        for (int tap = 0; tap < 9; ++tap) {
+            const int ky = tap / 3, kx = tap - ky * 3;
+            h8_t a[4];
+#pragma unroll
+            for (int k16 = 0; k16 < 4; ++k16) a[k16] = an[(c * 9 + tap) % FD_RING][k16];
+            const int gn = c * 9 + tap + DIST < 36 ? c * 9 + tap + DIST : 35;
+            FD_LOAD_A(an[(c * 9 + tap + DIST) % FD_RING], gn / 9, gn % 9)
+            __builtin_amdgcn_sched_barrier(0);
+#pragma unroll
+            for (int t = 0; t < 2; ++t) {
+                const int rec = recb[t] + ky * 4 + kx;
+#pragma unroll
+                for (int k16 = 0; k16 < 4; ++k16) {
+                    const h8_t b = *reinterpret_cast<const h8_t *>(X + rec * 128 + (((k16 * 2 + lhi) ^ (rec & 7) ^ kcode) << 4));
+                    acc[t] = __builtin_amdgcn_mfma_f32_32x32x16_f16(a[k16], b, acc[t], 0, 0, 0);
+                }
+            }
+        }
+    }
+#undef FD_LOAD_A
+
+#pragma unroll
+    for (int t = 0; t < 2; ++t) {
+        const int kp = k0 + t * 8 + (lrow >> 2);
+        if (kp >= n) continue;
+        const size_t oo = ((size_t)kp * 4 + (lrow & 3)) * FD_C + n0 + 4 * lhi;
+#pragma unroll
+        for (int q = 0; q < 4; ++q) {
+            const float4 sc = *reinterpret_cast<const float4 *>(scale + n0 + 8 * q + 4 * lhi);
+            const float4 sh = *reinterpret_cast<const float4 *>(shift + n0 + 8 * q + 4 * lhi);
+            const float v0 = acc[t][4 * q + 0] * sc.x + sh.x, v1 = acc[t][4 * q + 1] * sc.y + sh.y;
+            const float v2 = acc[t][4 * q + 2] * sc.z + sh.z, v3 = acc[t][4 * q + 3] * sc.w + sh.w;
+            *reinterpret_cast<float4 *>(out + oo + 8 * q) = make_float4(v0, v1, v2, v3);
+        }
+    }
+}
+
+int desc_fold_cout_pad() { return FD_C; }
+
+void launch_desc_fold(hipStream_t st, const half_t *fmap, int hc, int wc, int nh, int nw, const half_t *wsl, const float *scale, const float *shift,
+                      const float *kpts, const unsigned int *count, int n_max, float *out, const half_t *zero_page)
+{
+    if (n_max <= 0) return;
+    hipLaunchKernelGGL(desc_fold_kernel, dim3((n_max + FD_KP - 1) / FD_KP), dim3(FD_NT), 0, st, fmap, hc, wc, (float)nw / 2.0f, (float)nh / 2.0f,
+                       wsl, scale, shift, kpts, count, n_max, out, zero_page);
+}
diff --git a/sfd2_amd/csrc/fold_pab_kernel.hip b/sfd2_amd/csrc/fold_pab_kernel.hip
--- /dev/null
+++ b/sfd2_amd/csrc/fold_pab_kernel.hip
@@ -0,0 +1,223 @@
+#include "sfd2_internal.h"
+
+#define FP_TH 8
+#define FP_TW 16
+#define FP_CC 32
+#define FP_NW 3
+#define FP_COUT (FP_NW * 32)
+#define FP_P 32
+#define FP_PH (FP_TH + 2)
+#define FP_PWU (FP_TW + 2)
+#define FP_NPIECE (FP_PH * FP_P / 16)
+#define FP_PPW ((FP_NPIECE + FP_NW - 1) / FP_NW)
+#define FP_XBYTES (FP_NPIECE * 1024)
+#define FP_DF (2 * FP_P)
+
+typedef __attribute__((address_space(3))) void fp_lds_t;
+
+__device__ __forceinline__ int fp_xcd_swizzle(int bid, int nblk)
+{
+    const int q = nblk >> 3, r = nblk & 7, xcd = bid & 7, local = bid >> 3;
+    const int base = xcd < r ? xcd * (q + 1) : r * (q + 1) + (xcd - r) * q;
+    return base + local;
+}
+
+__device__ __forceinline__ void fp_copy_piece(const half_t *base, int nbytes, unsigned char *dst, int voff, int soff)
+{
+    const auto rs = __builtin_amdgcn_make_buffer_rsrc(const_cast<half_t *>(base), 0, nbytes, 0x00020000);
+    __builtin_amdgcn_raw_ptr_buffer_load_lds(rs, (fp_lds_t *)dst, 16, voff, soff, 0, 0);
+}
+
+__global__ __launch_bounds__(FP_NW * 64)
+void det_fold_kernel(const half_t *__restrict__ in, int H, int W, int Cin, const half_t *__restrict__ wpk, const float *__restrict__ scale,
+                     const float *__restrict__ shift, float *__restrict__ out, int pitch, int cstore, int tiles_x, int n_tiles)
+{
+    extern __shared__ __attribute__((aligned(16))) unsigned char smem[];
+    unsigned char *Xs = smem;
+
+    const int tid = threadIdx.x, lane = tid & 63;
+    const int wave = __builtin_amdgcn_readfirstlane(tid >> 6);
+    const int lhi = lane >> 5, l32 = lane & 31, ly = l32 >> 4, lx = l32 & 15;
+    const int n0 = wave * 32;
+
+    const int NCH = Cin / FP_CC;
+    const int NU = NCH * 9;
+    const int n_my = (n_tiles - (int)blockIdx.x + (int)gridDim.x - 1) / (int)gridDim.x;
+    if (n_my <= 0) return;
+    const int TC = n_my * NCH;
+
+    const int in_bytes = (int)((size_t)H * W * Cin * sizeof(half_t));
+    int xoff[FP_PPW];
+    int xoff_seq = -1;
+#define FP_SETUP_X(seq_)                                                                               \
+    {                                                                                                  \
+        const int swz_ = fp_xcd_swizzle((int)blockIdx.x + (seq_) * (int)gridDim.x, n_tiles);           \
+        const int tx_ = swz_ % tiles_x, ty_ = swz_ / tiles_x;                                          \
+        const int poy0_ = ty_ * FP_TH, pox0_ = tx_ * FP_TW;                                            \
+        _Pragma("unroll") for (int i = 0; i < FP_PPW; ++i) {                                           \
+            int piece = wave + FP_NW * i;                                                              \
+            if (piece >= FP_NPIECE) piece = FP_NPIECE - 1;                                             \
+            const int q = piece * 16 + (lane >> 2);                                                    \
+            const int slot = (lane & 3) ^ ((q >> 2) & 3);                                              \
+            const int row = q / FP_P, ir = q - row * FP_P;                                             \
+            int off = (int)0x80000000;                                                                 \
+            if (row < FP_PH && ir < FP_PWU) {                                                          \
+                const int iy = poy0_ - 1 + row, ix = pox0_ - 1 + ir;                                   \
+                if (iy >= 0 && iy < H && ix >= 0 && ix < W) off = ((iy * W + ix) * Cin + slot * 8) * (int)sizeof(half_t); \
+            }                                                                                          \
+            xoff[i] = off;                                                                             \
+        }                                                                                              \
+        xoff_seq = (seq_);                                                                             \
+    }
+#define FP_ISSUE_X1(chunk_, buf_, i_)                                                                  \
+    do {                                                                                               \
+        const int pc_ = (wave + FP_NW * (i_) < FP_NPIECE) ? wave + FP_NW * (i_) : FP_NPIECE - 1;       \
+        fp_copy_piece(in, in_bytes, Xs + (buf_)*FP_XBYTES + pc_ * 1024, xoff[i_], (chunk_)*FP_CC * (int)sizeof(half_t)); \
+    } while (0)
+#define FP_ISSUE_X(chunk_, buf_) \
+    _Pragma("unroll") for (int i_ = 0; i_ < FP_PPW; ++i_) FP_ISSUE_X1(chunk_, buf_, i_);
+
+    const int aoff = (n0 + l32) * FP_CC + lhi * 8;
+#define FP_LOAD_A(u_, dst_)                                                                            \
+    do {                                                                                               \
+        int ao_ = aoff;                                                                                \
+        asm volatile("" : "+v"(ao_));                                                                  \
+        const half_t *ap_ = wpk + (size_t)(u_)*FP_COUT * FP_CC + ao_;                                  \
+        dst_[0] = *reinterpret_cast<const h8_t *>(ap_);                                                \
+        dst_[1] = *reinterpret_cast<const h8_t *>(ap_ + 16);                                           \
+    } while (0)
+
+    const int qb = ly * FP_P + lx;
+#define FP_READ_B(xs_, t_, kk_, dst_)                                                                  \
+    do {                                                                                               \
+        const int to_ = ((t_) / 3) * FP_P + (t_) % 3;                                                  \
+        int q_ = qb;                                                                                   \
+        asm volatile("" : "+v"(q_));                                                                   \
+        q_ += to_;                                                                                     \
+        const unsigned char *bp_ = (xs_) + q_ * 64 + (((((kk_)*2 + lhi)) ^ ((q_ >> 2) & 3)) << 4);    \
+        _Pragma("unroll") for (int f_ = 0; f_ < 4; ++f_)                                               \
+            dst_[f_] = *reinterpret_cast<const h8_t *>(bp_ + f_ * (FP_DF * 64));                       \
+    } while (0)
+
+    f32x16_t acc[4];
+#pragma unroll
+    for (int f = 0; f < 4; ++f)
+#pragma unroll
+        for (int r = 0; r < 16; ++r) acc[f][r] = 0.0f;
+    h8_t fa[9][2], fb[3][4];
+
+    float4 sc[4], sh[4];
+#pragma unroll
+    for (int q = 0; q < 4; ++q) {
+        sc[q] = *reinterpret_cast<const float4 *>(scale + n0 + 4 * lhi + 8 * q);
+        sh[q] = *reinterpret_cast<const float4 *>(shift + n0 + 4 * lhi + 8 * q);
+    }
+
+    FP_SETUP_X(0)
+    FP_ISSUE_X(0, 0)
+    FP_ISSUE_X(1, 1)
+#pragma unroll
+    for (int u = 0; u < 9; ++u) FP_LOAD_A(u, fa[u]);
+    SFD2_BARRIER_DRAIN();
+    FP_READ_B(Xs, 0, 0, fb[0]);
+    FP_READ_B(Xs, 0, 1, fb[1]);
+
+    int bc = 0;
+    int c = 0, seq = 0, C = 0;
+    auto chunk = [&]() {
+        const int bn = bc == 2 ? 0 : bc + 1, bnn = bn == 2 ? 0 : bn + 1;
+        const unsigned char *xs = Xs + bc * FP_XBYTES;
+        const unsigned char *xn = Xs + bn * FP_XBYTES;
+        const int Cx = C + 2 < TC ? C + 2 : TC - 1;
+        const int seq_x = Cx / NCH, cx = Cx - seq_x * NCH;
+        if (seq_x != xoff_seq) FP_SETUP_X(seq_x)
+#pragma unroll
+        for (int t = 0; t < 9; ++t) {
+            if (t < FP_PPW) FP_ISSUE_X1(cx, bnn, t);
+            if (t == 8) {
+                static_assert(2 * (10 - FP_PPW) + 16 + FP_PPW == 29, "chunk-boundary wait count");
+                asm volatile("s_waitcnt vmcnt(29) lgkmcnt(0)\n\ts_barrier" ::: "memory");
+                __builtin_amdgcn_sched_barrier(0);
+            }
+#pragma unroll
+            for (int kk = 0; kk < 2; ++kk) {
+                const int h = 2 * t + kk;
+                if (h + 2 < 18) FP_READ_B(xs, (h + 2) / 2, (h + 2) % 2, fb[(h + 2) % 3]);
+                else FP_READ_B(xn, (h + 2 - 18) / 2, (h + 2) % 2, fb[(h + 2) % 3]);
+                __builtin_amdgcn_sched_barrier(0);
+#pragma unroll
+                for (int f = 0; f < 4; ++f)
+                    acc[f] = __builtin_amdgcn_mfma_f32_32x32x16_f16(fa[t][kk], fb[h % 3][f], acc[f], 0, 0, 0);
+                __builtin_amdgcn_sched_barrier(0);
+            }
+            int ua = c * 9 + t + 9;
+            if (ua >= NU) ua -= NU;
+            FP_LOAD_A(ua, fa[t]);
+            __builtin_amdgcn_sched_barrier(0);
+        }
+        bc = bn;
+        ++C;
+    };
+    auto epilogue = [&]() {
+        const int swz_ = fp_xcd_swizzle((int)blockIdx.x + seq * (int)gridDim.x, n_tiles);
+        const int tx_ = swz_ % tiles_x, ty_ = swz_ / tiles_x;
+        const int oy0 = ty_ * FP_TH, ox0 = tx_ * FP_TW;
+#pragma unroll
+        for (int f = 0; f < 4; ++f) {
+            const int oy = oy0 + 2 * f + ly, ox = ox0 + lx;
+            const bool inb = oy < H && ox < W;
+            const size_t pix = (size_t)(inb ? oy : 0) * W + (inb ? ox : 0);
+#pragma unroll
+            for (int q = 0; q < 4; ++q) {
+                const float v0 = acc[f][4 * q + 0] * sc[q].x + sh[q].x;
+                const float v1 = acc[f][4 * q + 1] * sc[q].y + sh[q].y;
+                const float v2 = acc[f][4 * q + 2] * sc[q].z + sh[q].z;
+                const float v3 = acc[f][4 * q + 3] * sc[q].w + sh[q].w;
+                if (inb && n0 + 8 * q < cstore)
+                    *reinterpret_cast<float4 *>(out + pix * pitch + n0 + 8 * q + 4 * lhi) = make_float4(v0, v1, v2, v3);
+            }
+#pragma unroll
+            for (int r = 0; r < 16; ++r) acc[f][r] = 0.0f;
+        }
+        c = 0;
+        ++seq;
+    };
+    while (C < TC) {
+        chunk();
+        if (++c == NCH) epilogue();
+    }
+#undef FP_ISSUE_X
+#undef FP_ISSUE_X1
+#undef FP_LOAD_A
+#undef FP_READ_B
+#undef FP_SETUP_X
+}
+
+bool det_fold_serves(int cin, int H, int W)
+{
+    return cin >= 64 && cin % 64 == 0 && (long long)(H + 2) * (W + 2) * cin * (long long)sizeof(half_t) < (1ll << 31);
+}
+
+int det_fold_cout_pad() { return FP_COUT; }
+
+void launch_det_fold(hipStream_t st, const half_t *in, int H, int W, int Cin, const half_t *wpk, const float *scale, const float *shift,
+                     int cout, float *out, int pitch)
+{
+    constexpr size_t lds = (size_t)3 * FP_XBYTES;
+    static bool attr_done = false;
+    static int slots = 256;
+    if (!attr_done) {
+        (void)hipFuncSetAttribute(reinterpret_cast<const void *>(det_fold_kernel), hipFuncAttributeMaxDynamicSharedMemorySize, (int)lds);
+        int dev = 0, cus = 0;
+        if (hipGetDevice(&dev) == hipSuccess && hipDeviceGetAttribute(&cus, hipDeviceAttributeMultiprocessorCount, dev) == hipSuccess && cus > 0)
+            slots = cus;
+        attr_done = true;
+    }
+    const int tiles_x = (W + FP_TW - 1) / FP_TW, tiles_y = (H + FP_TH - 1) / FP_TH;
+    const int n_tiles = tiles_x * tiles_y;
+    const int grid = n_tiles < sfd2_slots(slots) ? n_tiles : sfd2_slots(slots);
+    int cstore = (cout + 7) / 8 * 8;
+    if (cstore > FP_COUT) cstore = FP_COUT;
+    if (cstore > pitch) cstore = pitch / 8 * 8;
+    hipLaunchKernelGGL(det_fold_kernel, dim3(grid), dim3(FP_NW * 64), lds, st, in, H, W, Cin, wpk, scale, shift, out, pitch, cstore, tiles_x, n_tiles);
+}
diff --git a/sfd2_amd/csrc/post_kernels.hip b/sfd2_amd/csrc/post_kernels.hip
--- a/sfd2_amd/csrc/post_kernels.hip
+++ b/sfd2_amd/csrc/post_kernels.hip
@@ -100,8 +100,9 @@
 
 __global__ __launch_bounds__(NT)
 void heads_heat_kernel(const float *__restrict__ logits, int pitch, int hc8, int wc8, const float *__restrict__ sta, int hc, int wc,
-                       float st_y, float st_x, int H, int W, float *__restrict__ heat)
-{
+                       float st_y, float st_x, int H, int W, float *__restrict__ heat, unsigned int *__restrict__ zero, int n_zero)
+{
+    if (zero && (int)(blockIdx.x * NT + threadIdx.x) < n_zero) zero[blockIdx.x * NT + threadIdx.x] = 0u;
     const int lane = threadIdx.x & 63;
     const int cell = blockIdx.x * (NT / 64) + (threadIdx.x >> 6);
     if (cell >= hc8 * wc8) return;
@@ -129,12 +130,14 @@
 }
 
 void launch_heads_heat(hipStream_t st, const float *logits, int pitch, int hc8, int wc8, const float *sta, int hc, int wc,
-                       int H, int W, float *heat)
+                       int H, int W, float *heat, unsigned int *zero, int n_zero)
 {
     const float st_y = hc > 0 ? (float)hc / (float)H : 1.0f, st_x = wc > 0 ? (float)wc / (float)W : 1.0f;
     const int cells = hc8 * wc8;
-    hipLaunchKernelGGL(heads_heat_kernel, dim3((cells + 3) / 4), dim3(NT), 0, st, logits, pitch, hc8, wc8, sta, hc, wc, st_y, st_x, H, W, heat);
-}
+    if (!heads_heat_clears(hc8, wc8, n_zero)) zero = nullptr;
+    hipLaunchKernelGGL(heads_heat_kernel, dim3((cells + 3) / 4), dim3(NT), 0, st, logits, pitch, hc8, wc8, sta, hc, wc, st_y, st_x, H, W, heat, zero, n_zero);
+}
+bool heads_heat_clears(int hc8, int wc8, int n_zero) { return n_zero > 0 && ((hc8 * wc8 + 3) / 4) * NT >= n_zero; }
 
 #define PH_CELLS 32
 #define PH_XREC 528
diff --git a/sfd2_amd/csrc/sfd2_ctx.h b/sfd2_amd/csrc/sfd2_ctx.h
--- a/sfd2_amd/csrc/sfd2_ctx.h
+++ b/sfd2_amd/csrc/sfd2_ctx.h
@@ -200,6 +200,10 @@
     int opt_sparse_da0 = 1;
     DevPtr da0_in;
     int opt_fuse_pb = 1;
+    int opt_fold_pab = 0;
+    ConvW pab;
+    int opt_fold_dab = 1;
+    ConvW dab;
     int opt_comp_rb = 1;
     int opt_rb_inner = 2;
     int opt_fuse_rb23 = 1;
@@ -349,6 +353,8 @@
     bool skip_head = false, skip_pb = false, skip_db = false, skip_da3 = false;
     bool sparse_desc = false, sparse_da3 = false, sparse_x3 = false;
     bool sparse_da0 = false;
+    bool fold_dab = false;
+    bool fold_pab = false;
     struct { int slot = -1; size_t off = 0; } at[T_COUNT];
     int n_slots = 0;
     size_t slot_bytes = 0;
diff --git a/sfd2_amd/csrc/sfd2_internal.h b/sfd2_amd/csrc/sfd2_internal.h
--- a/sfd2_amd/csrc/sfd2_internal.h
+++ b/sfd2_amd/csrc/sfd2_internal.h
@@ -323,6 +323,13 @@
 bool sparse_da0_serves(int cin, int CoutP, int hc, int wc);
 void launch_sparse_da0(hipStream_t st, const half_t *in, int hc, int wc, int nh, int nw, const half_t *wpk, const float *scale, const float *shift,
                        int relu, const float *kpts, const unsigned int *count, int n_max, half_t *out);
+bool det_fold_serves(int cin, int H, int W);
+int det_fold_cout_pad();
+void launch_det_fold(hipStream_t st, const half_t *in, int H, int W, int Cin, const half_t *wpk, const float *scale, const float *shift,
+                     int cout, float *out, int pitch);
+int desc_fold_cout_pad();
+void launch_desc_fold(hipStream_t st, const half_t *fmap, int hc, int wc, int nh, int nw, const half_t *wsl, const float *scale, const float *shift,
+                      const float *kpts, const unsigned int *count, int n_max, float *out, const half_t *zero_page);
 void launch_sparse_da3(hipStream_t st, const half_t *fmap, int hc, int wc, int nh, int nw, const half_t *wpk, const half_t *wsl, int CoutP,
                        const float *scale, const float *shift, int relu, const float *kpts, const unsigned int *count, int n_max,
                        half_t *out, const half_t *zero_page);
@@ -371,7 +378,8 @@
                        float *nms_dense , unsigned long long *cand_keys, int cand_cap,
                        unsigned int *counters , int fuse_threshold = 0, int top_k = 0);
 void launch_heads_heat(hipStream_t st, const float *logits, int pitch, int hc8, int wc8, const float *sta, int hc, int wc,
-                       int H, int W, float *heat);
+                       int H, int W, float *heat, unsigned int *zero = nullptr, int n_zero = 0);
+bool heads_heat_clears(int hc8, int wc8, int n_zero);
 void launch_topk_sort(hipStream_t st, bool threshold_done, const unsigned long long *cand, int cand_cap, int top_k,
                       unsigned long long *sel, unsigned long long *sorted, int sel_cap, unsigned int *counters,
                       unsigned long long *bnd, int W, float *kpts, float *scores);
```
